# klindsay28/Newton-Krylov_OOC

Hardware: AMD Instinct MI355X
Metric: GMRES JVPs/sec, py_driver_2d iage (value = value_frozen: products on frozen years, the default; value_reference_semantic: the reference's product, two free-running years, same solver, same run) (higher is better)
Workload: dtype f64

## Files before the change

### newton-krylov_ooc_amd/csrc/nk2d_api.hip

```cpp
#include "nk2d_common.h"
#include "nk2d_build_id.h"

#include <algorithm>
#include <cmath>
#include <cstring>
#include <new>

namespace {

template <typename T>
int dev_alloc(nk2d_ctx* c, T** p, size_t n) {
    NK2D_CHECK(c, hipMalloc((void**)p, sizeof(T) * std::max<size_t>(n, 1)));
    NK2D_CHECK(c, hipMemsetAsync(*p, 0, sizeof(T) * std::max<size_t>(n, 1), nk2d_s(c)));
    return 0;
}

int ensure_stage(nk2d_ctx* c, size_t n) {
    if (n <= c->stage_elems) return 0;
    NK2D_CHECK(c, hipStreamSynchronize(nk2d_s(c)));
    if (c->STAGE) NK2D_CHECK(c, hipFree(c->STAGE));
    if (c->hSTAGE) NK2D_CHECK(c, hipHostFree(c->hSTAGE));
    c->STAGE = c->hSTAGE = nullptr;
    c->stage_elems = 0;
    NK2D_CHECK(c, hipMalloc((void**)&c->STAGE, sizeof(double) * n));
    NK2D_CHECK(c, hipHostMalloc((void**)&c->hSTAGE, sizeof(double) * n));
    c->stage_elems = n;
    return 0;
}

int stage_in(nk2d_ctx* c, const double* host, size_t n) {
    NK2D_TRY(ensure_stage(c, n));
    NK2D_CHECK(c, hipStreamSynchronize(nk2d_s(c)));
    std::memcpy(c->hSTAGE, host, sizeof(double) * n);
    NK2D_CHECK(c, hipMemcpyAsync(c->STAGE, c->hSTAGE, sizeof(double) * n, hipMemcpyHostToDevice, nk2d_s(c)));
    return 0;
}

int stage_out(nk2d_ctx* c, double* host, size_t n) {
    NK2D_CHECK(c, hipMemcpyAsync(c->hSTAGE, c->STAGE, sizeof(double) * n, hipMemcpyDeviceToHost, nk2d_s(c)));
    NK2D_CHECK(c, hipStreamSynchronize(nk2d_s(c)));
    std::memcpy(host, c->hSTAGE, sizeof(double) * n);
    return 0;
}

}

struct nk2d_download {
    double* dev = nullptr;
    double* host = nullptr;
    hipEvent_t done = nullptr;
    size_t n = 0;
};
struct nk2d_download_pool {
    std::mutex m;
    std::vector<nk2d_download*> all, idle;
};

namespace {

void download_pool_free(nk2d_ctx* c) {
    if (!c->dl_pool) return;
    for (nk2d_download* t : c->dl_pool->all) {
        (void)hipEventSynchronize(t->done);
        (void)hipEventDestroy(t->done);
        (void)hipFree(t->dev);
        (void)hipHostFree(t->host);
        delete t;
    }
    delete c->dl_pool;
    c->dl_pool = nullptr;
}

int upload_plane(nk2d_ctx* c, const double* host, int nrows, int ncols, double* dst, double fill = 0.0) {
    const size_t n = (size_t)nrows * ncols;
    NK2D_TRY(stage_in(c, host, n));
    NK2D_TRY(nk2d_k_pack_plane(c, c->STAGE, nrows, ncols, dst, fill));
    NK2D_CHECK(c, hipStreamSynchronize(nk2d_s(c)));
    return 0;
}

void build_front(nk2d_ctx* c, const std::vector<double>& dzr, const std::vector<double>& dyr) {
    const int nz = c->nz, ny = c->ny;
    const double* v = c->d.vvel;
    const double* w = c->d.wvel;
    const double* kh = c->d.hmix_coeff;
    std::vector<std::pair<double, double>> pts;
    pts.reserve((size_t)nz * ny);
    for (int k = 0; k < nz; ++k)
        for (int j = 0; j < ny; ++j) {
            const double a_up = (k > 0) ? (-0.5 * w[(size_t)k * ny + j]) * dzr[k] : 0.0;
            const double a_dn = (k < nz - 1) ? (0.5 * w[(size_t)(k + 1) * ny + j]) * dzr[k] : 0.0;
            const double a_s = (j > 0) ? (0.5 * v[(size_t)k * (ny + 1) + j]) * dyr[j] : 0.0;
            const double a_n = (j < ny - 1) ? (-0.5 * v[(size_t)k * (ny + 1) + j + 1]) * dyr[j] : 0.0;
            const double h_s = (j > 0) ? kh[(size_t)k * (ny - 1) + j - 1] * dyr[j] : 0.0;
            const double h_n = (j < ny - 1) ? kh[(size_t)k * (ny - 1) + j] * dyr[j] : 0.0;
            const double s = std::fabs(a_s + h_s) + std::fabs(a_n + h_n);
            const double q = (h_s + h_n) - (a_s + a_n) - 2.0 * (a_up + a_dn);
            if (c->kind == 1) {
                const double* ph = c->d.phos_params;
                const double upr_max = ph[1] * c->d.light_lim[(size_t)k * ny + j] / ph[0];
                const double sink_out = (k < nz - 1) ? ph[5] * dzr[k] : 0.0, sink_in = (k > 0) ? ph[5] * dzr[k] : 0.0;
                pts.emplace_back(q, s + ph[3] + ph[4]);
                pts.emplace_back(q + ph[3], s + ph[2] * upr_max);
                pts.emplace_back(q + ph[4] + sink_out - sink_in, s + (1.0 - ph[2]) * upr_max);
            } else if (s > 0.0) {
                pts.emplace_back(q, s);
            }
        }
    c->rho_c0 = 1.0e-10;
    c->rho_dlog = 1.0 / 64.0;
    const int ntab = 64 * 15;
    c->rho_tab.assign(ntab, 0.0);
    for (int k = 0; k < ntab; ++k) {
        const double shift = c->rho_c0 * std::pow(10.0, k * c->rho_dlog);
        double rho = 0.0;
        for (const auto& p : pts) {
            const double den = shift + p.first;
            const double r = (den > 0.0) ? p.second / den : 1.0e30;
            if (r > rho) rho = r;
        }
        c->rho_tab[k] = rho;
    }
}

}

extern "C" const char* nk2d_version(void) { return "nk2d 0.1 (gfx950)"; }

extern "C" const char* nk2d_last_error(const nk2d_ctx* ctx) { return ctx ? ctx->err.c_str() : "null context"; }

extern "C" void* nk2d_stream(nk2d_ctx* ctx) { return ctx ? (void*)nk2d_s(ctx) : nullptr; }

extern "C" int nk2d_set_option(nk2d_ctx* c, const char* name, double value) {
    const std::string key(name ? name : "");
    if (key == "device_ctl") {
        if ((int)value != 0) return nk2d_fail(c, "nk2d_set_option: device_ctl 1, 2 and 3 no longer exist (the controller is the host's; see option stream_years)");
        return 0;
    }
    if (key == "jac_fresh") { c->jac_fresh = value != 0.0; return 0; }
    if (key == "growth_cap") {
        if (!(value >= 0.0)) return nk2d_fail(c, "nk2d_set_option: growth_cap must be >= 0");
        c->growth_cap = value;
        return 0;
    }
    if (key == "speculate") { c->speculate = value != 0.0; return 0; }
    if (key == "hook_spec_depth") {
        if (!(value == 1.0 || value == 2.0)) return nk2d_fail(c, "nk2d_set_option: hook_spec_depth is 1 or 2");
        c->hook_spec_depth = (int)value;
        return 0;
    }
    if (key == "pc_valu") { c->pc_valu = value != 0.0; return 0; }
    if (key == "pc_fused") { c->pc_fused = (int)value; return 0; }
    if (key == "pc_fp32") { c->pc_fp32 = value != 0.0; return 0; }
    if (key == "pc_refine") {
        if (!(value >= 0.0 && value <= 4.0)) return nk2d_fail(c, "nk2d_set_option: pc_refine must be 0 .. 4");
        c->pc_refine = (int)value;
        return 0;
    }
    if (key == "pc_two_ended") {
        if (value != 0.0 && value != 1.0) return nk2d_fail(c, "nk2d_set_option: pc_two_ended is 0 or 1");
        c->pc_two_ended = (int)value;
        return 0;
    }
    if (key == "pc_pivot_wave") {
        if (value != 0.0 && value != 1.0) return nk2d_fail(c, "nk2d_set_option: pc_pivot_wave is 0 or 1");
        c->pc_pivot_wave = (int)value;
        return 0;
    }
    if (key == "final_fuse") { c->final_fuse = value != 0.0; return 0; }
    if (key == "year_fences") { c->year_fences = value != 0.0; return 0; }
    if (key == "frozen_persistent") { c->frozen_persistent = value != 0.0; return 0; }
    if (key == "frozen_team") { c->frozen_team = value != 0.0; return 0; }
    if (key == "frozen_coef_lds") { c->frozen_coef_lds = (int)value & 63; return 0; }
    if (key == "frozen_sums_poison") { c->frozen_sums_poison = (int)value != 0 ? 1 : 0; return 0; }
    if (key == "frozen_early") { c->frozen_early = (int)value != 0 ? 1 : 0; return 0; }
    if (key == "frozen_by_column") { c->frozen_by_column = (int)value; return 0; }
    if (key == "frozen_cache_after") { c->frozen_cache_after = (int)value; return 0; }
    if (key == "spec_bias") { c->spec_bias = value > 0.0 ? value : 1.0; return 0; }
    if (key == "stream_years") { c->stream_years = (int)value; c->stream_lost = 0; return 0; }
    if (key == "frozen_tape") {
        if (value != 0.0 && value != 1.0) return nk2d_fail(c, "nk2d_set_option: frozen_tape is 0 or 1");
        c->frozen_tape = (int)value;
        return 0;
    }
    if (key == "stream_hist") {
        if (value != 0.0 && value != 1.0) return nk2d_fail(c, "nk2d_set_option: stream_hist is 0 or 1");
        c->stream_hist = (int)value;
        return 0;
    }
    if (key == "stream_hist_mb") {
        if (!(value >= 0.0) || !std::isfinite(value)) return nk2d_fail(c, "nk2d_set_option: stream_hist_mb must be >= 0");
        c->stream_hist_mb = value;
        return 0;
    }
    if (key == "stream_two_waves") {
        if (c->strm) return nk2d_fail(c, "nk2d_set_option: stream_two_waves must be set before the first year of the context");
        c->stream_two_waves = (int)value;
        return 0;
    }
    if (key == "frozen_wpb") { c->frozen_wpb = (int)value; return 0; }
    if (key == "frozen_alloc_async") { c->frozen_alloc_async = value != 0.0; return 0; }
    if (key == "frozen_persistent_max_e") { c->frozen_persistent_max_e = (int)value; return 0; }
    if (key == "frozen_cache_gb") { c->frozen_cache_max_gb = value; return 0; }
    if (key == "frozen_cache_pieces") {
        if (value != 0.0 && value != 1.0) return nk2d_fail(c, "nk2d_set_option: frozen_cache_pieces is 0 or 1");
        c->frozen_cache_pieces = (int)value;
        return 0;
    }
    if (key == "frozen_cache_lean") {
        if (value != 0.0 && value != 1.0 && value != 2.0) return nk2d_fail(c, "nk2d_set_option: frozen_cache_lean is 0, 1 or 2");
        c->frozen_cache_lean = (int)value;
        return 0;
    }
    if (key == "frozen_forced") {
        if (value != 0.0 && value != 1.0 && value != 2.0 && value != 3.0) return nk2d_fail(c, "nk2d_set_option: frozen_forced is a bit mask 0 ... 3");
        c->frozen_forced = (int)value;
        return 0;
    }
    if (key == "frozen_phosphorus") {
        if (value != 0.0 && value != 1.0 && value != 2.0 && value != 3.0) return nk2d_fail(c, "nk2d_set_option: frozen_phosphorus is 0, 1, 2 or 3");
        c->frozen_phosphorus = (int)value;
        return 0;
    }
    if (key == "frozen_phosphorus_shallow") {
        if (value != 0.0 && value != 1.0) return nk2d_fail(c, "nk2d_set_option: frozen_phosphorus_shallow is 0 or 1");
        c->frozen_phosphorus_shallow = (int)value;
        return 0;
    }
    if (key == "frozen_cache_piece_mb") {
        if (!(value > 0.0) || !std::isfinite(value)) return nk2d_fail(c, "nk2d_set_option: frozen_cache_piece_mb must be > 0");
        c->frozen_cache_piece_mb = value;
        return 0;
    }
    if (key == "frozen_cache_piece_rows") {
        if (!(value >= 0.0) || value > 1.0e9) return nk2d_fail(c, "nk2d_set_option: frozen_cache_piece_rows must be 0 (from frozen_cache_piece_mb) or a row count");
        c->frozen_cache_piece_rows = (int64_t)value;
        return 0;
    }
    if (key == "frozen_cache_early") {
        if (value != 0.0 && value != 1.0) return nk2d_fail(c, "nk2d_set_option: frozen_cache_early is 0 or 1");
        c->frozen_cache_early = (int)value;
        return 0;
    }
    if (key == "barrier_timeout_ms") {
        if (!(value >= 0.0)) return nk2d_fail(c, "nk2d_set_option: barrier_timeout_ms must be >= 0");
        c->barrier_timeout_ms = value;
        return 0;
    }
    if (key == "frozen_err_check") {
        if (!(value >= 0.0) || value > 1.0e6) return nk2d_fail(c, "nk2d_set_option: frozen_err_check must be 0 (off) or a step stride");
        c->frozen_err_check = (int)value;
        return 0;
    }
    if (key == "jac_stage_state") { c->jac_stage_state = value != 0.0; return 0; }
    if (key == "jac_stage") {
        if (value != -1.0 && value != 0.0 && value != 1.0 && value != 2.0) return nk2d_fail(c, "nk2d_set_option: jac_stage must be -1, 0, 1 or 2");
        c->jac_stage = (int)value;
        return 0;
    }
    if (key == "team") {
        if (value != 0.0 && value != 1.0 && value != 2.0 && value != -1.0) return nk2d_fail(c, "nk2d_set_option: team must be -1, 0, 1 or 2");
        c->team = (value < 0.0) ? nk2d_team_auto(c) : (int)value;
        return 0;
    }
    if (key == "min_sweeps") {
        if (value != 1.0 && value != 2.0) return nk2d_fail(c, "nk2d_set_option: min_sweeps must be 1 or 2");
        c->min_sweeps = (int)value;
        c->yr_lin_tol = -1.0;
        return 0;
    }
    if (key == "factor_fp32") {
        c->factor_fp32 = value != 0.0;
        return 0;
    }
    if (key == "sweep_wpb") {
        const int w = (int)value;
        if (w != 1 && w != 2 && w != 4) return nk2d_fail(c, "nk2d_set_option: sweep_wpb must be 1, 2 or 4");
        c->sweep_wpb = w;
        return 0;
    }
    if (key == "lin_tol") {
        if (!(value > 0.0 && value < 1.0)) return nk2d_fail(c, "nk2d_set_option: lin_tol must be in (0, 1)");
        c->d.lin_tol = value;
        return 0;
    }
    return nk2d_fail(c, "nk2d_set_option: unknown option " + key);
}

extern "C" int nk2d_sync(nk2d_ctx* c) {
    NK2D_CHECK(c, hipSetDevice(c->dev));
    NK2D_CHECK(c, hipStreamSynchronize(nk2d_s(c)));
    return 0;
}

extern "C" int nk2d_profile_reset(nk2d_ctx* c, int32_t every_n) {
    NK2D_CHECK(c, hipSetDevice(c->dev));
    NK2D_CHECK(c, hipStreamSynchronize(nk2d_s(c)));
    const size_t want = every_n > 0 ? 2 * 8192 : 0;
    while (c->prof_ev.size() < want) {
        hipEvent_t e;
        NK2D_CHECK(c, hipEventCreate(&e));
        c->prof_ev.push_back(e);
    }
    c->prof_overhead_ms = 0.0;
    if (every_n > 0) {
        const int ncal = 64;
        for (int i = 0; i < ncal; ++i) {
            NK2D_CHECK(c, hipEventRecord(c->prof_ev[2 * i], nk2d_s(c)));
            NK2D_CHECK(c, hipEventRecord(c->prof_ev[2 * i + 1], nk2d_s(c)));
        }
        NK2D_CHECK(c, hipStreamSynchronize(nk2d_s(c)));
        double sum = 0.0;
        for (int i = 0; i < ncal; ++i) {
            float ms = 0.f;
            NK2D_CHECK(c, hipEventElapsedTime(&ms, c->prof_ev[2 * i], c->prof_ev[2 * i + 1]));
            sum += ms;
        }
        c->prof_overhead_ms = sum / ncal;
    }
    c->prof_every = every_n;
    c->prof_used = 0;
    c->prof_ms_sum = 0.0;
    c->prof_cnt = 0;
    c->prof_windows = 0;
    c->prof_win_launches.clear();
    c->win_open = 0;
    c->win_seq = 0;
    c->sweep_launches = 0;
// ... 121 lines not shown
        if (desc->restore_nrec == 0 && desc->sms_nrec == 0)
            return nk2d_fail(c, "nk2d_create: module_kind 2 without forcing records (use module_kind 0)");
        if ((desc->restore_nrec > 0 && (!desc->restore_times || !desc->restore_vals)) ||
            (desc->sms_nrec > 0 && (!desc->sms_times || !desc->sms_vals)))
            return nk2d_fail(c, "nk2d_create: forcing records missing");
        if (desc->sink_thres < 0.0) return nk2d_fail(c, "nk2d_create: sink_thres < 0");
        for (int i = 1; i < desc->restore_nrec; ++i)
            if (!(desc->restore_times[i] > desc->restore_times[i - 1])) return nk2d_fail(c, "nk2d_create: restore_times not increasing");
        for (int i = 1; i < desc->sms_nrec; ++i)
            if (!(desc->sms_times[i] > desc->sms_times[i - 1])) return nk2d_fail(c, "nk2d_create: sms_times not increasing");
    } else {
        c->d.restore_nrec = c->d.sms_nrec = 0;
        c->d.sink_thres = 0.0;
    }
    if (c->kind == 1 && (c->tc != 3 || desc->light_lim == nullptr))
        return nk2d_fail(c, "nk2d_create: the phosphorus module has 3 tracers and needs light_lim");
    if (c->nz < 2 || c->ny < 1 || c->tc < 1 || c->tc > NK2D_MAX_TRACERS) return nk2d_fail(c, "nk2d_create: bad grid / tracer count");
    c->E = (c->nz + 63) / 64;
    if (c->E > NK2D_MAX_E) return nk2d_fail(c, "nk2d_create: nz > 512 levels not supported by this build");
    c->nzp = c->E * 64;
    c->ncol = c->tc * c->ny;
    c->nv = (size_t)c->ncol * c->nzp;
    c->np = (size_t)c->ny * c->nzp;
    c->kv_len = (c->kind == 2) ? 2 * c->np + (size_t)c->ny : c->np;
    c->nreg = 0;
    c->dev = desc->device_id;
    NK2D_CHECK(c, hipSetDevice(c->dev));
    NK2D_CHECK(c, hipStreamCreateWithFlags(&c->stream_, hipStreamNonBlocking));
    const int nz = c->nz, ny = c->ny;
    {
        uint64_t h = 14695981039346656037ull;
        h = fnv_val(h, c->nz); h = fnv_val(h, c->ny); h = fnv_val(h, c->tc); h = fnv_val(h, c->kind);
        h = fnv1a(h, desc->depth_edges, sizeof(double) * (nz + 1));
        h = fnv1a(h, desc->ypos_edges, sizeof(double) * (ny + 1));
        h = fnv1a(h, desc->vvel, sizeof(double) * (size_t)nz * (ny + 1));
        h = fnv1a(h, desc->wvel, sizeof(double) * (size_t)(nz + 1) * ny);
        if (ny > 1) h = fnv1a(h, desc->hmix_coeff, sizeof(double) * (size_t)nz * (ny - 1));
        h = fnv1a(h, desc->bldepth_max, sizeof(double) * ny);
        h = fnv_val(h, desc->bldepth_min); h = fnv1a(h, desc->bld_tvals, sizeof(desc->bld_tvals));
        h = fnv1a(h, desc->bld_fvals, sizeof(desc->bld_fvals));
        h = fnv_val(h, desc->vmix_log_shallow); h = fnv_val(h, desc->vmix_log_deep); h = fnv_val(h, desc->vmix_half_width);
        h = fnv1a(h, desc->surf_rate, sizeof(desc->surf_rate)); h = fnv1a(h, desc->surf_target, sizeof(desc->surf_target));
        h = fnv1a(h, desc->decay_rate, sizeof(desc->decay_rate)); h = fnv_val(h, desc->const_src);
        if (c->kind == 1) {
            h = fnv1a(h, desc->phos_params, sizeof(desc->phos_params));
            h = fnv1a(h, desc->light_lim, sizeof(double) * (size_t)nz * ny);
        }
        if (c->kind == 2) {
            h = fnv_val(h, c->d.restore_nrec); h = fnv_val(h, c->d.sms_nrec); h = fnv_val(h, c->d.sink_thres);
            if (c->d.restore_nrec > 0) {
                h = fnv1a(h, desc->restore_times, sizeof(double) * c->d.restore_nrec);
                h = fnv1a(h, desc->restore_vals, sizeof(double) * (size_t)c->d.restore_nrec * ny);
            }
            if (c->d.sms_nrec > 0) {
                h = fnv1a(h, desc->sms_times, sizeof(double) * c->d.sms_nrec);
                h = fnv1a(h, desc->sms_vals, sizeof(double) * (size_t)c->d.sms_nrec * nz * ny);
            }
        }
        c->grid_hash = h;
    }
    NK2D_TRY(dev_alloc(c, &c->VV, (size_t)(ny + 1) * c->nzp));
    NK2D_TRY(dev_alloc(c, &c->KH, (size_t)(ny + 1) * c->nzp));
    NK2D_TRY(dev_alloc(c, &c->WT, c->np));
    NK2D_TRY(dev_alloc(c, &c->WB, c->np));
    NK2D_TRY(dev_alloc(c, &c->DZR, (size_t)c->nzp));
    NK2D_TRY(dev_alloc(c, &c->ZM0, (size_t)c->nzp));
    NK2D_TRY(dev_alloc(c, &c->ZM1, (size_t)c->nzp));
    NK2D_TRY(dev_alloc(c, &c->DM, (size_t)c->nzp));
    NK2D_TRY(dev_alloc(c, &c->DMR, (size_t)c->nzp));
    NK2D_TRY(dev_alloc(c, &c->DYR, (size_t)ny));
    NK2D_TRY(dev_alloc(c, &c->BLDMAX, (size_t)ny));
    NK2D_TRY(dev_alloc(c, &c->MASK, c->np));
    NK2D_TRY(dev_alloc(c, &c->WN, c->np));
    NK2D_TRY(dev_alloc(c, &c->JL, c->np));
    NK2D_TRY(dev_alloc(c, &c->JU, c->np));
    NK2D_TRY(dev_alloc(c, &c->JS, c->np));
    NK2D_TRY(dev_alloc(c, &c->JN, c->np));
    NK2D_TRY(dev_alloc(c, &c->JC, c->np));
    NK2D_TRY(dev_alloc(c, &c->LIGHT, c->np));
    NK2D_TRY(dev_alloc(c, &c->UPR, c->np));
    c->YLIN = nullptr;
    c->ylin_set = 0;
    for (int i = 0; i < 5; ++i) NK2D_TRY(dev_alloc(c, &c->KV[i], c->kv_len));
    for (int i = 0; i < 3; ++i) NK2D_TRY(dev_alloc(c, &c->KVN[i], c->kv_len));
    for (int i = 0; i < 5; ++i) NK2D_TRY(dev_alloc(c, &c->JB[i], c->np));
    NK2D_TRY(dev_alloc(c, &c->Y, c->nv));
    NK2D_TRY(dev_alloc(c, &c->YOLD, c->nv));
    NK2D_TRY(dev_alloc(c, &c->F, c->nv));
    NK2D_TRY(dev_alloc(c, &c->Z, 3 * c->nv));
    NK2D_TRY(dev_alloc(c, &c->ZP, 3 * c->nv));
    NK2D_TRY(dev_alloc(c, &c->ZN, 3 * c->nv));
    c->single_swap = 0;
    c->min_sweeps = 1;
    c->team = nk2d_team_auto(c);
    c->jac_stage = 1;
    c->final_fuse = 1;
    c->jac_stage_state = 1;
    c->part_cur = nullptr;
    NK2D_TRY(dev_alloc(c, &c->W, 3 * c->nv));
    NK2D_TRY(dev_alloc(c, &c->BR, c->nv));
    NK2D_TRY(dev_alloc(c, &c->BCR, c->nv));
    NK2D_TRY(dev_alloc(c, &c->BCI, c->nv));
    for (int i = 0; i < 2; ++i) {
        NK2D_TRY(dev_alloc(c, &c->XR[i], c->nv));
        NK2D_TRY(dev_alloc(c, &c->XCR[i], c->nv));
        NK2D_TRY(dev_alloc(c, &c->XCI[i], c->nv));
    }
    NK2D_TRY(dev_alloc(c, &c->FR_INV, c->nv));
    NK2D_TRY(dev_alloc(c, &c->FC_INVR, c->nv));
    NK2D_TRY(dev_alloc(c, &c->FC_INVI, c->nv));
    NK2D_TRY(dev_alloc(c, &c->FR_TAB, (size_t)c->ncol * 14 * 64));
    NK2D_TRY(dev_alloc(c, &c->FC_TABR, (size_t)c->ncol * 14 * 64));
    NK2D_TRY(dev_alloc(c, &c->FC_TABI, (size_t)c->ncol * 14 * 64));
    NK2D_TRY(dev_alloc(c, &c->FR32_INV, c->nv));
    NK2D_TRY(dev_alloc(c, &c->FC32_INVR, c->nv));
    NK2D_TRY(dev_alloc(c, &c->FC32_INVI, c->nv));
    NK2D_TRY(dev_alloc(c, &c->FR32_TAB, (size_t)c->ncol * 14 * 64));
    NK2D_TRY(dev_alloc(c, &c->FC32_TABR, (size_t)c->ncol * 14 * 64));
    NK2D_TRY(dev_alloc(c, &c->FC32_TABI, (size_t)c->ncol * 14 * 64));
    c->factor_fp32 = 0;
    NK2D_TRY(dev_alloc(c, &c->TMP, c->nv));
    NK2D_TRY(dev_alloc(c, &c->TMP2, c->nv));
    NK2D_TRY(dev_alloc(c, &c->PART, (size_t)c->ncol));
    NK2D_TRY(dev_alloc(c, &c->PART2, (size_t)c->ncol));
    NK2D_TRY(dev_alloc(c, &c->STEP_NORM, (size_t)3 * NK2D_OWN_REC_CAP));
    c->frozen_fallbacks = 0;
    c->frozen_resumes = 0;
    c->frozen_cache = nullptr;
    c->frozen_persistent = 1;
    c->frozen_persistent_max_e = 8;
    c->frozen_cache_max_gb = 128.0;
    c->frozen_cache_builds = c->frozen_persistent_years = 0;
    c->frozen_team = 1;
    c->frozen_cache_after = 0;
    c->frozen_cache_pieces = 0;
    c->frozen_cache_piece_mb = 1024.0;
    c->frozen_cache_piece_rows = 0;
    c->frozen_cache_early = 0;
    c->frozen_cache_lean = 0;
    c->frozen_lean_years = 0;
    c->frozen_lean_mem_key = 0;
    c->frozen_forced = 0;
    c->frozen_forced_years = 0;
    c->frozen_phosphorus = 0;
    c->frozen_phosphorus_shallow = 0;
    c->frozen_phosphorus_shallow_years = 0;
    c->frozen_two_waves_last = 0;
    c->frozen_phosphorus_years = c->frozen_two_waves_years = 0;
    c->frozen_cache_piece_allocs = c->frozen_cache_early_requests = 0;
    c->frozen_coef_lds = 63;
    c->frozen_lds_bits = 0;
    c->frozen_early = NK2D_FROZEN_EARLY_DEFAULT;
    c->frozen_early_bits = 0;
    c->frozen_by_column = 1;
    c->strm = nullptr;
    c->spec_bias = 1.0;
    c->stream_two_waves = std::getenv("NK2D_STREAM_TWO_WAVES") ? std::atoi(std::getenv("NK2D_STREAM_TWO_WAVES")) : 1;
    c->stream_years = 1;
    c->stream_on = 0;
    c->stream_lost = 0;
    c->stream_cmds = c->stream_launches = c->stream_timeouts = c->stream_years_run = 0;
    c->frozen_tape = 0;
    c->tape = nullptr;
    c->tape_rec = c->tape_foreign = 0;
    c->tape_years_run = c->tape_builds = c->tape_timeouts = c->tape_fallbacks = 0;
    c->frozen_wpb = 2;
    c->frozen_alloc_async = 1;
    c->barrier_timeout_ms = 2000.0;
    c->year_fences = 0;
    c->frozen_err_check = NK2D_CKPT_EVERY;
    c->STEP_PART = nullptr;
    c->step_part_rows = 0;
    NK2D_TRY(dev_alloc(c, &c->RED, (size_t)4096));
    for (int i = 0; i < 8; ++i) NK2D_CHECK(c, hipEventCreateWithFlags(&c->snap_ev[i], hipEventDisableTiming));
    c->snap_ready = 1;
    c->jac_fresh = 1;
    c->growth_cap = 0.0;
    c->hist_n = 0;
    c->hist_next = 0;
    c->hist_t = nullptr;
    c->hist_host = nullptr;
    c->stream_hist = 0;
    c->stream_hist_mb = 256.0;
    c->HISTBUF = nullptr;
    c->hist_slots = c->hist_buf_elems = 0;
    c->hist_year_samples = c->hist_year_drains = 0;
    c->stream_hist_samples = c->stream_hist_drains = 0;
    c->sweep_wpb = 4;
    NK2D_CHECK(c, hipHostMalloc((void**)&c->hRED, sizeof(double) * 4096));
    NK2D_CHECK(c, hipHostMalloc((void**)&c->hPART, sizeof(double) * c->ncol));
    NK2D_CHECK(c, hipHostMalloc((void**)&c->hPART2, sizeof(double) * c->ncol));
    NK2D_CHECK(c, hipHostMalloc((void**)&c->hPARTB, sizeof(double) * c->ncol));
    NK2D_CHECK(c, hipHostMalloc((void**)&c->hPARTC, sizeof(double) * c->ncol));
    c->part_on_host = 0;
    c->speculate = 1;
    c->hook_spec_depth = 2;
    c->factor_pending = 0;
    c->lu_cre = c->lu_ccr = c->lu_cci = 0.0;
    c->rcoef_elems = 0;
    c->RCOEF = nullptr;
    c->hRCOEF = nullptr;

    std::vector<double> zmid(nz), dz(nz), dzr(nz), dzm(nz), dzmr(nz), zm1(nz), dy(ny), dyr(ny);
    for (int k = 0; k < nz; ++k) {
        zmid[k] = 0.5 * (desc->depth_edges[k] + desc->depth_edges[k + 1]);
        dz[k] = desc->depth_edges[k + 1] - desc->depth_edges[k];
        dzr[k] = 1.0 / dz[k];
    }
    for (int k = 0; k < nz; ++k) {
        zm1[k] = (k < nz - 1) ? zmid[k + 1] : 0.0;
        dzm[k] = (k < nz - 1) ? zmid[k + 1] - zmid[k] : 0.0;
        dzmr[k] = (k < nz - 1) ? 1.0 / dzm[k] : 0.0;
    }
    for (int j = 0; j < ny; ++j) {
        dy[j] = desc->ypos_edges[j + 1] - desc->ypos_edges[j];
        dyr[j] = 1.0 / dy[j];
    }
    NK2D_TRY(upload_plane(c, desc->vvel, nz, ny + 1, c->VV));
    {
        std::vector<double> khf((size_t)nz * (ny + 1), 0.0);
        for (int k = 0; k < nz; ++k)
            for (int jf = 1; jf < ny; ++jf) khf[(size_t)k * (ny + 1) + jf] = desc->hmix_coeff[(size_t)k * (ny - 1) + jf - 1];
        NK2D_TRY(upload_plane(c, khf.data(), nz, ny + 1, c->KH));
    }
    NK2D_TRY(upload_plane(c, desc->wvel, nz, ny, c->WT));
    NK2D_TRY(upload_plane(c, desc->wvel + ny, nz, ny, c->WB));
    NK2D_TRY(upload_plane(c, dzr.data(), nz, 1, c->DZR));
    NK2D_TRY(upload_plane(c, zmid.data(), nz, 1, c->ZM0));
    NK2D_TRY(upload_plane(c, zm1.data(), nz, 1, c->ZM1));
    NK2D_TRY(upload_plane(c, dzm.data(), nz, 1, c->DM));
    NK2D_TRY(upload_plane(c, dzmr.data(), nz, 1, c->DMR));
    NK2D_CHECK(c, hipMemcpy(c->DYR, dyr.data(), sizeof(double) * ny, hipMemcpyHostToDevice));
    NK2D_CHECK(c, hipMemcpy(c->BLDMAX, desc->bldepth_max, sizeof(double) * ny, hipMemcpyHostToDevice));
    if (c->kind == 1) NK2D_TRY(upload_plane(c, desc->light_lim, nz, ny, c->LIGHT));
    if (c->kind == 2) {
        if (desc->sms_nrec > 0) {
            NK2D_TRY(dev_alloc(c, &c->SMSREC, (size_t)desc->sms_nrec * c->np));
            for (int r = 0; r < desc->sms_nrec; ++r)
                NK2D_TRY(upload_plane(c, desc->sms_vals + (size_t)r * nz * ny, nz, ny, c->SMSREC + (size_t)r * c->np));
            c->sms_t = new double[desc->sms_nrec];
            std::memcpy(c->sms_t, desc->sms_times, sizeof(double) * desc->sms_nrec);
        }
        if (desc->restore_nrec > 0) {
            NK2D_TRY(dev_alloc(c, &c->RESTREC, (size_t)desc->restore_nrec * ny));
            NK2D_CHECK(c, hipMemcpy(c->RESTREC, desc->restore_vals, sizeof(double) * desc->restore_nrec * ny, hipMemcpyHostToDevice));
            c->rest_t = new double[desc->restore_nrec];
            std::memcpy(c->rest_t, desc->restore_times, sizeof(double) * desc->restore_nrec);
        }
    }
    build_front(c, dzr, dyr);
    c->d.depth_edges = c->d.ypos_edges = c->d.vvel = c->d.wvel = c->d.hmix_coeff = c->d.bldepth_max = nullptr;
    c->d.light_lim = nullptr;
    c->d.restore_times = c->d.restore_vals = c->d.sms_times = c->d.sms_vals = nullptr;
    {
        std::vector<int32_t> m((size_t)nz * ny, 1);
        std::vector<double> w((size_t)nz * ny, 1.0);
        NK2D_TRY(nk2d_set_region(c, m.data(), w.data(), 1));
    }
    return 0;
}

extern "C" int nk2d_create(const nk2d_desc* desc, nk2d_ctx** out) {
    if (!desc || !out) return -2;
    nk2d_ctx* c = new (std::nothrow) nk2d_ctx();
    if (!c) return -2;
    c->stream_ = nullptr;
    c->STAGE = nullptr;
    c->hSTAGE = nullptr;
    c->stage_elems = 0;
    c->dl_pool = nullptr;
    c->precond = nullptr;
    c->pc_valu = 0;
    c->pc_fused = 1;
    c->pc_fp32 = 0;
    c->pc_refine = 1;
    c->pc_two_ended = 0;
    c->pc_setup_rounds = c->pc_sub_launches = 0;
    c->pc_pivot_wave = 0;
    c->pc_pivot_wave_steps = 0;
    c->st = nk2d_stats();
    c->prof_every = 0;
    c->snap_ready = 0;
    c->prof_used = 0;
    c->prof_ms_sum = 0.0;
    c->prof_overhead_ms = 0.0;
    c->prof_cnt = 0;
    c->prof_windows = 0;
    c->win_open = 0;
    c->win_seq = 0;
    c->sweep_launches = 0;
    c->sweep_bytes = 0.0;
    c->fused_bytes_all = 0.0;
    c->norm_hook = nullptr;
    c->norm_hook_user = nullptr;
    c->norm_hook_vec = nullptr;
    c->norm_hook_vec_user = nullptr;
    c->global_n = 0.0;
    c->timer_ready = 0;
    c->YR_PART = c->YR_OUT = c->hYR_OUT = c->YR_REC = nullptr;
    c->YR_SYNC = nullptr;
    c->YR_MTAB = nullptr;
    *out = c;
    return create_impl(c, desc);
}

extern "C" void nk2d_destroy(nk2d_ctx* c) {
// ... 206 lines not shown
}

extern "C" int nk2d_vmix_coeff(nk2d_ctx* c, double t, double* host_out) {
    NK2D_CHECK(c, hipSetDevice(c->dev));
    double* out[1] = {c->KV[4]};
    NK2D_TRY(nk2d_k_vmix(c, 1, &t, out));
    const size_t n = (size_t)(c->nz - 1) * c->ny;
    NK2D_TRY(ensure_stage(c, n));
    NK2D_TRY(nk2d_k_unpack_plane(c, c->KV[4], c->nz - 1, c->ny, c->STAGE));
    return stage_out(c, host_out, n);
}

static const double* lin_state(nk2d_ctx* c) { return (c->kind != 0 && c->ylin_set) ? c->YLIN : nullptr; }

extern "C" int nk2d_set_lin_state(nk2d_ctx* c, nk2d_vec y) {
    NK2D_CHECK(c, hipSetDevice(c->dev));
    if (!c->YLIN) NK2D_TRY(dev_alloc(c, &c->YLIN, c->nv));
    NK2D_CHECK(c, hipMemcpyAsync(c->YLIN, y, sizeof(double) * c->nv, hipMemcpyDeviceToDevice, nk2d_s(c)));
    c->ylin_set = 1;
    return 0;
}

extern "C" int nk2d_jacobian_apply(nk2d_ctx* c, double t, nk2d_vec v, nk2d_vec out) {
    NK2D_CHECK(c, hipSetDevice(c->dev));
    double* kv[1] = {c->KV[4]};
    NK2D_TRY(nk2d_k_vmix(c, 1, &t, kv));
    NK2D_TRY(nk2d_k_jac(c, c->KV[4], lin_state(c)));
    NK2D_TRY(nk2d_k_jac_apply(c, (const double*)v, (double*)out));
    return 0;
}

extern "C" int nk2d_jacobian_diags(nk2d_ctx* c, double t, double* host_out) {
    NK2D_CHECK(c, hipSetDevice(c->dev));
    if (c->kind == 1) return nk2d_fail(c, "nk2d_jacobian_diags: the phosphorus Jacobian is not five diagonals; use nk2d_jacobian_apply");
    double* out[1] = {c->KV[4]};
    NK2D_TRY(nk2d_k_vmix(c, 1, &t, out));
    NK2D_TRY(nk2d_k_jac(c, c->KV[4], lin_state(c)));
    const size_t P = (size_t)c->nz * c->ny;
    NK2D_TRY(ensure_stage(c, P));
    const double* planes[5] = {c->JL, c->JS, c->JC, c->JN, c->JU};
    std::vector<double> tmp(P), extra;
    if (c->kind == 2) {
        extra.resize(P);
        NK2D_TRY(nk2d_k_unpack_plane(c, c->UPR, c->nz, c->ny, c->STAGE));
        NK2D_TRY(stage_out(c, extra.data(), P));
    }
    for (int d = 0; d < 5; ++d) {
        NK2D_TRY(nk2d_k_unpack_plane(c, planes[d], c->nz, c->ny, c->STAGE));
        NK2D_TRY(stage_out(c, tmp.data(), P));
        for (int tr = 0; tr < c->tc; ++tr) {
            double* dst = host_out + ((size_t)d * c->tc + tr) * P;
            std::memcpy(dst, tmp.data(), sizeof(double) * P);
            if (d == 2) {
                for (int j = 0; j < c->ny; ++j) dst[j] = dst[j] + (-c->d.surf_rate[tr]);
                if (c->d.decay_rate[tr] != 0.0)
                    for (size_t i = 0; i < P; ++i) dst[i] = dst[i] + (-c->d.decay_rate[tr]);
                if (!extra.empty())
                    for (size_t i = 0; i < P; ++i) dst[i] = dst[i] - extra[i];
            }
        }
    }
    return 0;
}

extern "C" int nk2d_shifted_solve(nk2d_ctx* c, double t_jac, double h, double mu_re, double mu_im, nk2d_vec b_re,
                                  nk2d_vec b_im, nk2d_vec x_re, nk2d_vec x_im, int32_t* sweeps_out) {
    NK2D_CHECK(c, hipSetDevice(c->dev));
    double* out[1] = {c->KV[4]};
    NK2D_TRY(nk2d_k_vmix(c, 1, &t_jac, out));
    NK2D_TRY(nk2d_k_jac(c, c->KV[4], lin_state(c)));
    const bool cplxsys = mu_im != 0.0;
    const int m = nk2d_sweeps_for(c, mu_re / h);
    NK2D_TRY(nk2d_k_factor(c, !cplxsys, cplxsys, mu_re / h, mu_re / h, mu_im / h));
    int src = 0;
    for (int it = 0; it < m; ++it) {
        NK2D_TRY(nk2d_k_sweep(c, !cplxsys, cplxsys, it == 0, mu_re / h, mu_re / h, mu_im / h, (const double*)b_re,
                              (const double*)b_re, (const double*)b_im, src));
        src = 1 - src;
    }
    if (!cplxsys) {
        NK2D_CHECK(c, hipMemcpyAsync(x_re, c->XR[src], sizeof(double) * c->nv, hipMemcpyDeviceToDevice, nk2d_s(c)));
    } else {
        NK2D_CHECK(c, hipMemcpyAsync(x_re, c->XCR[src], sizeof(double) * c->nv, hipMemcpyDeviceToDevice, nk2d_s(c)));
        NK2D_CHECK(c, hipMemcpyAsync(x_im, c->XCI[src], sizeof(double) * c->nv, hipMemcpyDeviceToDevice, nk2d_s(c)));
    }
    NK2D_CHECK(c, hipStreamSynchronize(nk2d_s(c)));
    if (sweeps_out) *sweeps_out = m;
    return 0;
}

extern "C" int nk2d_comp_fcn(nk2d_ctx* c, nk2d_vec x, nk2d_vec fx, nk2d_stats* stats, const double* replay,
                             int64_t replay_n, double* record, int64_t record_cap, int64_t* record_n) {
    NK2D_CHECK(c, hipSetDevice(c->dev));
    if (record_n) *record_n = 0;
    const int rc = nk2d_radau_year(c, x, fx, stats, replay, replay_n, record, record_cap, record_n);
    if (rc == 0 && record && record_n && *record_n > 0 && c->frozen_cache_pieces && c->frozen_cache_early)
        NK2D_TRY(nk2d_frozen_cache_early(c, record, *record_n));
    return rc;
}

extern "C" int nk2d_comp_fcn_frozen(nk2d_ctx* c, nk2d_vec x, nk2d_vec fx, nk2d_stats* stats, const double* sched,
                                    int64_t sched_n) {
    NK2D_CHECK(c, hipSetDevice(c->dev));
    if (!sched || sched_n < 1) return nk2d_fail(c, "nk2d_comp_fcn_frozen: empty schedule");
    return nk2d_radau_year(c, x, fx, stats, sched, sched_n, nullptr, 0, nullptr, true);
}

extern "C" int nk2d_frozen_fallbacks(nk2d_ctx* c, int64_t* n) {
    if (n) *n = c->frozen_fallbacks;
    return 0;
}

extern "C" int nk2d_frozen_resumes(nk2d_ctx* c, int64_t* n) {
    if (n) *n = c->frozen_resumes;
    return 0;
}

extern "C" int nk2d_get_counter(nk2d_ctx* c, const char* name, int64_t* out) {
    const std::string key(name ? name : "");
    int64_t v = 0;
    if (key == "frozen_persistent_years") v = c->frozen_persistent_years;
    else if (key == "frozen_cache_builds") v = c->frozen_cache_builds;
    else if (key == "frozen_team_years") v = c->frozen_team_years;
    else if (key == "stream_years_run") v = c->stream_years_run;
    else if (key == "stream_commands") v = c->stream_cmds;
    else if (key == "stream_launches") v = c->stream_launches;
    else if (key == "stream_timeouts") v = c->stream_timeouts;
    else if (key == "stream_columns_per_workgroup") v = nk2d_stream_columns_per_workgroup(c);
    else if (key == "stream_two_waves_kernel") v = nk2d_stream_two_waves(c);
    else if (key == "stream_hist_samples") v = c->stream_hist_samples;
    else if (key == "stream_hist_drains") v = c->stream_hist_drains;
    else if (key == "pc_setup_rounds") v = c->pc_setup_rounds;
    else if (key == "pc_sub_launches") v = c->pc_sub_launches;
    else if (key == "pc_pivot_wave_steps") v = c->pc_pivot_wave_steps;
    else if (key == "tape_years_run") v = c->tape_years_run;
    else if (key == "tape_builds") v = c->tape_builds;
    else if (key == "tape_timeouts") v = c->tape_timeouts;
    else if (key == "tape_fallbacks") v = c->tape_fallbacks;
    else if (key == "tape_bytes") v = nk2d_tape_size(c, 0);
    else if (key == "tape_commands") v = nk2d_tape_size(c, 1);
    else if (key.rfind("stream_prof_", 0) == 0) {
        double pr[12];
        NK2D_TRY(nk2d_stream_profile(c, pr));
        const int i = std::atoi(key.c_str() + 12);
        v = (i >= 0 && i < 12) ? (int64_t)pr[i] : 0;
    }
    else if (key == "frozen_launch_us") v = c->frozen_launch_us;
    else if (key == "frozen_cache_pending") v = nk2d_frozen_cache_pending(c);
    else if (key == "frozen_cache_bytes") v = nk2d_frozen_cache_bytes(c);
    else if (key == "frozen_cache_pieces") v = nk2d_frozen_cache_npieces(c);
    else if (key == "frozen_cache_lean") v = nk2d_frozen_cache_is_lean(c);
    else if (key == "frozen_lds_bits") v = c->frozen_lds_bits;
    else if (key == "frozen_early_bits") v = c->frozen_early_bits;
    else if (key == "frozen_step_sums_hash") v = c->frozen_step_sums_hash;
    else if (key == "frozen_lean_years") v = c->frozen_lean_years;
    else if (key == "frozen_forced_years") v = c->frozen_forced_years;
    else if (key == "frozen_phosphorus_years") v = c->frozen_phosphorus_years;
    else if (key == "frozen_phosphorus_shallow_years") v = c->frozen_phosphorus_shallow_years;
    else if (key == "frozen_two_waves_years") v = c->frozen_two_waves_years;
    else if (key == "frozen_cache_piece_allocs") v = nk2d_frozen_cache_piece_allocs(c);
    else if (key == "frozen_cache_early_requests") v = c->frozen_cache_early_requests;
    else if (key == "frozen_fallbacks") v = c->frozen_fallbacks;
    else if (key == "frozen_resumes") v = c->frozen_resumes;
    else if (key == "spec_launches_dropped") v = c->cnt_spec_dropped;
    else if (key == "spec_front_launches_dropped") v = c->cnt_front_dropped;
    else if (key == "err_estimates_queued") v = c->cnt_err_queued;
    else if (key == "err_estimates_dropped") v = c->cnt_err_void;
    else return nk2d_fail(c, "nk2d_get_counter: unknown counter " + key);
    if (out) *out = v;
    return 0;
}

extern "C" int nk2d_schedule_fingerprint(nk2d_ctx* c, double* out) {
    if (out) *out = nk2d_fingerprint(c);
    return 0;
}

extern "C" int nk2d_last_schedule(nk2d_ctx* c, double* out, int64_t cap, int64_t* n) {
    const int64_t rows = (int64_t)(c->last_sched.size() / NK2D_SCHED_WIDTH);
    if (n) *n = rows;
    if (out) {
        if (cap < rows) return nk2d_fail(c, "nk2d_last_schedule: buffer too small", -4);
        std::memcpy(out, c->last_sched.data(), sizeof(double) * c->last_sched.size());
    }
    return 0;
}

extern "C" int nk2d_set_frozen_schedule(nk2d_ctx* c, const double* sched, int64_t sched_n) {
    if (sched_n < 0 || (sched_n > 0 && !sched)) return nk2d_fail(c, "nk2d_set_frozen_schedule: bad arguments");
    c->frozen_sched.assign(sched, sched + (size_t)sched_n * NK2D_SCHED_WIDTH);
    return 0;
}

int nk2d_hist_sample(nk2d_ctx* c, double t_old, double t_new, bool first) {
    const size_t n = (size_t)c->tc * c->nz * c->ny;
    double x = 0.0;
    while (nk2d_hist_due(c, t_old, t_new, &x)) {
        NK2D_TRY(nk2d_r_dense(c, x, c->TMP));
        NK2D_TRY(ensure_stage(c, n));
        NK2D_TRY(nk2d_k_unpack_state(c, c->TMP, c->STAGE));
        NK2D_TRY(stage_out(c, c->hist_host + (size_t)c->hist_next * n, n));
        c->hist_next++;
    }
    (void)first;
    return 0;
}

int nk2d_hist_buf_ready(nk2d_ctx* c) {
    nk2d_hist_buf_reset(c);
    const double bytes = c->stream_hist_mb * 1048576.0;
    const double fit = std::floor(bytes / (8.0 * (double)c->nv));
    c->hist_slots = (size_t)std::min((double)c->hist_n, std::max(1.0, fit));
    const size_t need = c->hist_slots * c->nv;
    if (c->hist_buf_elems < need) {
        NK2D_CHECK(c, hipStreamSynchronize(nk2d_s(c)));
        if (c->HISTBUF) NK2D_CHECK(c, hipFree(c->HISTBUF));
        c->HISTBUF = nullptr;
        c->hist_buf_elems = 0;
        NK2D_CHECK(c, hipMalloc((void**)&c->HISTBUF, sizeof(double) * need));
        c->hist_buf_elems = need;
    }
    return ensure_stage(c, (size_t)c->tc * c->nz * c->ny);
}

void nk2d_hist_buf_reset(nk2d_ctx* c) {
    c->hist_slot_k.clear();
    c->hist_year_samples = c->hist_year_drains = 0;
}
void nk2d_hist_year_done(nk2d_ctx* c) {
    c->stream_hist_samples += c->hist_year_samples;
    c->stream_hist_drains += c->hist_year_drains;
    c->hist_year_samples = c->hist_year_drains = 0;
}

int nk2d_hist_drain(nk2d_ctx* c) {
    if (c->hist_slot_k.empty()) return 0;
    const size_t n = (size_t)c->tc * c->nz * c->ny;
    NK2D_TRY(ensure_stage(c, n));
    for (size_t slot = 0; slot < c->hist_slot_k.size(); ++slot) {
        NK2D_TRY(nk2d_k_unpack_state(c, c->HISTBUF + slot * c->nv, c->STAGE));
        NK2D_TRY(stage_out(c, c->hist_host + (size_t)c->hist_slot_k[slot] * n, n));
    }
    c->hist_year_samples += (int64_t)c->hist_slot_k.size();
    c->hist_year_drains++;
    c->hist_slot_k.clear();
    return 0;
}

int nk2d_hist_push(nk2d_ctx* c, double t_old, double t_new) {
    double x = 0.0;
    while (nk2d_hist_due(c, t_old, t_new, &x)) {
        if (c->hist_slot_k.size() >= c->hist_slots) NK2D_TRY(nk2d_hist_drain(c));
        NK2D_TRY(nk2d_r_dense_push(c, x, c->HISTBUF + c->hist_slot_k.size() * c->nv));
        c->hist_slot_k.push_back(c->hist_next);
        c->hist_next++;
    }
    return 0;
}

extern "C" int nk2d_comp_fcn_hist(nk2d_ctx* c, nk2d_vec x, nk2d_vec fx, nk2d_stats* stats, int32_t n_eval,
                                  const double* t_eval, double* host_hist) {
    NK2D_CHECK(c, hipSetDevice(c->dev));
    for (int i = 1; i < n_eval; ++i)
        if (!(t_eval[i] > t_eval[i - 1])) return nk2d_fail(c, "nk2d_comp_fcn_hist: t_eval must be increasing");
    if (n_eval > 0 && (t_eval[0] < c->d.t0 || t_eval[n_eval - 1] > c->d.t1))
        return nk2d_fail(c, "nk2d_comp_fcn_hist: t_eval outside the time range");
    c->hist_n = n_eval;
    c->hist_next = 0;
    c->hist_t = t_eval;
    c->hist_host = host_hist;
    nk2d_hist_buf_reset(c);
    const int rc = nk2d_radau_year(c, x, fx, stats, nullptr, 0, nullptr, 0, nullptr);
    const bool complete = c->hist_next == n_eval && c->hist_slot_k.empty();
    nk2d_hist_buf_reset(c);
    c->hist_n = 0;
    c->hist_t = nullptr;
    c->hist_host = nullptr;
    if (rc != 0) return rc;
    if (!complete) return nk2d_fail(c, "nk2d_comp_fcn_hist: not every t_eval sample was produced");
    return 0;
}

__device__ __forceinline__ double bcast(const double* __restrict__ coef, int m) { return (m > 0) ? coef[m - 1] : 1.0; }

template <int E>
__global__ void k_dot(int ncol, int ny, int nreg, const double* __restrict__ a, const double* __restrict__ b,
                      const double* __restrict__ wn, const int32_t* __restrict__ mask, double* __restrict__ part) {
    const int lane = threadIdx.x & 63;
    const int task = blockIdx.x * NK2D_WAVES_PER_BLOCK + (threadIdx.x >> 6);
    if (task >= ncol) return;
    const int j = task % ny;
    double aa[E], bb[E], ww[E];
    int mm[E];
    load_col<E>(a, task, lane, aa);
    load_col<E>(b, task, lane, bb);
    load_col<E>(wn, j, lane, ww);
#pragma unroll
    for (int e = 0; e < E; ++e) {
        mm[e] = mask[(size_t)j * (E * 64) + e * 64 + lane];
        aa[e] = ww[e] * (aa[e] * bb[e]);
    }
    for (int r = 1; r <= nreg; ++r) {
        double acc = 0.0;
        bool any = false;
#pragma unroll
        for (int e = 0; e < E; ++e)
// ... 192 lines not shown
```

### newton-krylov_ooc_amd/csrc/nk2d_bodies.h

```cpp
#pragma once
#include <atomic>
#include <chrono>
#include <cmath>
#include <cstdio>
#include <cstdlib>
#include <cstring>
#include <mutex>
#include <thread>

#include "nk2d_common.h"
#include "nk2d_hostmath.h"


struct DevP {
    int nz, ny, tc, ncol;
    const double *VV, *KH, *WT, *WB, *DZR, *ZM0, *ZM1, *DM, *DMR, *DYR, *BLDMAX;
    double surf[NK2D_MAX_TRACERS], starget[NK2D_MAX_TRACERS], decay[NK2D_MAX_TRACERS], csrc;
    double atol, rtol;
    double ph_hs, ph_mu, ph_sig, ph_rd, ph_rp, ph_vs;
    const double *LIGHT, *UPR;
    const double *SMSREC, *RESTREC;
    int f_sms, f_restore;
    double f_thres_r;
    size_t np;
// ... 609 lines not shown
            for (int e = 0; e < E; ++e) rr[e] = __builtin_fma(jn[e], xn[e], __builtin_fma(js[e], xs[e], rr[e]));
            load_col<E, MP>(A.xci_old, cs_col, lane, xs);
            load_col<E, MP>(A.xci_old, cn_col, lane, xn);
#pragma unroll
            for (int e = 0; e < E; ++e) ri[e] = __builtin_fma(jn[e], xn[e], __builtin_fma(js[e], xs[e], ri[e]));
            if constexpr (KIND == 1) {
                phos_couple<E>(P, tr, j, lane, A.xcr_old, upr, rr);
                phos_couple<E>(P, tr, j, lane, A.xci_old, upr, ri);
            }
        }
#pragma unroll
        for (int e = 0; e < E; ++e) {
            const bool valid = (lane * E + e) < P.nz;
            r[e] = c_make(valid ? rr[e] : 0.0, valid ? ri[e] : 0.0);
        }
        tridiag_apply<E, cplx>(a, cc, inv, tab, r, lane);
#pragma unroll
        for (int e = 0; e < E; ++e) { rr[e] = r[e].re; ri[e] = r[e].im; }
        store_col<E, MP>(A.xcr_new, col, lane, rr);
        store_col<E, MP>(A.xci_new, col, lane, ri);
    }
}

static inline void fill_factor_args(const nk2d_ctx* c, SweepArgs& A) {
    A.JL = c->JL; A.JU = c->JU; A.JS = c->JS; A.JN = c->JN; A.JC = c->JC;
    A.fr_inv = c->FR_INV; A.fc_invr = c->FC_INVR; A.fc_invi = c->FC_INVI;
    A.fr_tab = c->FR_TAB; A.fc_tabr = c->FC_TABR; A.fc_tabi = c->FC_TABI;
    A.fr_inv32 = c->FR32_INV; A.fc_invr32 = c->FC32_INVR; A.fc_invi32 = c->FC32_INVI;
    A.fr_tab32 = c->FR32_TAB; A.fc_tabr32 = c->FC32_TABR; A.fc_tabi32 = c->FC32_TABI;
    A.f32 = c->factor_fp32;
}

__device__ double block_sum(const double* __restrict__ part, int ntasks, double* sh) {
    double s = 0.0;
    for (int i = threadIdx.x; i < ntasks; i += NK2D_BLOCK) s += part[i];
    sh[threadIdx.x] = s;
    __syncthreads();
    for (int o = NK2D_BLOCK / 2; o > 0; o >>= 1) {
        if ((int)threadIdx.x < o) sh[threadIdx.x] += sh[threadIdx.x + o];
        __syncthreads();
    }
    return sh[0];
}

struct PredictArgs {
    const double *y, *yold, *zp;
    double *z, *w;
    size_t nv;
    double x0, x1, x2;
};

template <int E, int MP = 0>
__device__ __forceinline__ void predict_body(const PredictArgs& A, int task, int lane) {
    const double* __restrict__ y = A.y;
    const double* __restrict__ yold = A.yold;
    const double* __restrict__ zp = A.zp;
    double* __restrict__ z = A.z;
    double* __restrict__ w = A.w;
    const size_t nv = A.nv;
    const double x0 = A.x0, x1 = A.x1, x2 = A.x2;
    double yy[E], yo[E], z0[E], z1[E], z2[E];
    load_col<E, MP>(y, task, lane, yy);
    load_col<E, MP>(yold, task, lane, yo);
    load_col<E, MP>(zp, task, lane, z0);
    load_col<E, MP>(zp + nv, task, lane, z1);
    load_col<E, MP>(zp + 2 * nv, task, lane, z2);
    const double xs[3] = {x0, x1, x2};
    double o[3][E];
#pragma unroll
    for (int e = 0; e < E; ++e) {
        double q[3];
#pragma unroll
        for (int cidx = 0; cidx < 3; ++cidx) q[cidx] = (z0[e] * cP[0][cidx] + z1[e] * cP[1][cidx]) + z2[e] * cP[2][cidx];
#pragma unroll
        for (int i = 0; i < 3; ++i) {
            const double p1 = xs[i], p2 = p1 * xs[i], p3 = p2 * xs[i];
            double v = (q[0] * p1 + q[1] * p2) + q[2] * p3;
            v = v + yo[e];
            o[i][e] = v - yy[e];
        }
    }
    double wv[E];
#pragma unroll
    for (int i = 0; i < 3; ++i) store_col<E, MP>(z + i * nv, task, lane, o[i]);
#pragma unroll
    for (int r = 0; r < 3; ++r) {
#pragma unroll
        for (int e = 0; e < E; ++e) wv[e] = (cTI[r][0] * o[0][e] + cTI[r][1] * o[1][e]) + cTI[r][2] * o[2][e];
        store_col<E>(w + r * nv, task, lane, wv);
    }
}

struct JacOut {
    double *JL, *JU, *JS, *JN, *JC;
    int stage;
};

struct StageArgs {
    const double *y, *z, *w;
    double* zout;
    const double* kv[3];
    double *br, *bcr, *bci;
    size_t nv;
    double mreal, mcr, mci;
};

struct FinalArgs {
    double* ynew;
    double* znext;
    double x0, x1, x2;
    int nblk_cols;
};

struct FusedArgs {
    StageArgs st;
    SweepArgs sw;
    double* part;
    int do_stage, do_update;
    int delta;
};

template <int E>
__device__ __forceinline__ void w_lds_get(const double* s, int r, int lane, double (&v)[E]) {
#pragma unroll
    for (int e = 0; e < E; ++e) v[e] = s[(r * E + e) * 64 + lane];
}
template <int E>
__device__ __forceinline__ void w_lds_put(double* s, int r, int lane, const double (&v)[E]) {
#pragma unroll
    for (int e = 0; e < E; ++e) s[(r * E + e) * 64 + lane] = v[e];
}

struct LdsSrc {
    const double* coef;
    double* w;
    const double* step;
    const double* piv;
    double* y;
};
template <int E>
struct OwnState {
    double z[3][E];
    int valid;
};
template <int E>
__device__ __forceinline__ void col_lds_get(const double* s, int r, int lane, double (&v)[E]) {
#pragma unroll
    for (int e = 0; e < E; ++e) v[e] = s[(r * E + e) * 64 + lane];
}
struct LateNorm {
    double acc;
    double* part;
    int defer, pending;
};
template <int E>
__device__ __forceinline__ double norm_partial_sum(const DevP& P, const double (&yy)[E], const double (&d0v)[E],
                                                   const double (&d1v)[E], const double (&d2v)[E]) {
    double acc = 0.0;
#pragma unroll
    for (int e = 0; e < E; ++e) {
        const double sc = P.atol + fabs(yy[e]) * P.rtol;
        const double d0 = d0v[e] / sc, d1 = d1v[e] / sc, d2 = d2v[e] / sc;
        acc += (d0 * d0 + d1 * d1) + d2 * d2;
    }
    return wave_sum(acc);
}

template <int E, int KIND, int FACTOR, int STAGE, int MP = 0, int FINAL = 0, int CL = 0>
__device__ __forceinline__ void newton_fused_body(const DevP& P, const FusedArgs& A, int task, int lane,
                                                  const FinalArgs* fin = nullptr, const LdsSrc* lds = nullptr,
                                                  OwnState<E>* own = nullptr, LateNorm* late = nullptr) {
    const double* coef_lds = (CL & 1) ? lds->coef : nullptr;
    double* w_lds = (CL & 2) ? lds->w : nullptr;
    (void)coef_lds; (void)w_lds;
    const int tr = task / P.ny, j = task - tr * P.ny;
    const int cs_col = (j > 0) ? task - 1 : task, cn_col = (j < P.ny - 1) ? task + 1 : task;
    double fr[E], fcr[E], fci[E];
    if (STAGE && A.do_stage) {
        ColCoef<E> cf;
        if constexpr (CL & 1) load_coef_lds<E>(coef_lds, lane, cf);
        else load_coef<E>(P, j, lane, cf);
        double y0[E], ys[E], yn[E];
        if constexpr (CL & 16) {
            if (!own->valid) {
                load_col<E, MP>(A.st.y, task, lane, y0);
                w_lds_put<E>(lds->y, 0, lane, y0);
            } else {
                col_lds_get<E>(lds->y, 0, lane, y0);
            }
        } else {
            load_col<E, MP>(A.st.y, task, lane, y0);
        }
        load_col<E, MP>(A.st.y, cs_col, lane, ys);
        load_col<E, MP>(A.st.y, cn_col, lane, yn);
#pragma unroll
        for (int e = 0; e < E; ++e) { fr[e] = 0.0; fcr[e] = 0.0; fci[e] = 0.0; }
#pragma unroll
        for (int i = 0; i < 3; ++i) {
            double c[E], cs[E], cn[E], kv[E], f[E];
            if constexpr (CL & 32) {
                if (own->valid) {
#pragma unroll
                    for (int e = 0; e < E; ++e) c[e] = own->z[i][e];
                } else {
                    load_col<E, MP>(A.st.z + i * A.st.nv, task, lane, c);
                }
            } else {
                load_col<E, MP>(A.st.z + i * A.st.nv, task, lane, c);
            }
            load_col<E, MP>(A.st.z + i * A.st.nv, cs_col, lane, cs);
            load_col<E, MP>(A.st.z + i * A.st.nv, cn_col, lane, cn);
            if constexpr (CL & 4) col_lds_get<E>(lds->step, i, lane, kv);
            else load_col<E, MP>(A.st.kv[i], j, lane, kv);
#pragma unroll
            for (int e = 0; e < E; ++e) { c[e] = y0[e] + c[e]; cs[e] = ys[e] + cs[e]; cn[e] = yn[e] + cn[e]; }
            tend_col<E, KIND>(P, cf, c, cs, cn, kv, tr, lane, f);
            if constexpr (KIND == 2) forced_sources<E>(P, A.st.kv[i], j, lane, c, f);
            if constexpr (KIND == 1) {
                double u1[E], u2[E], v1[E], v2[E];
                phos_load_others<E>(P, tr, j, lane, A.st.y, u1, u2);
                phos_load_others<E>(P, tr, j, lane, A.st.z + i * A.st.nv, v1, v2);
                phos_add<E>(u1, u2, v1, v2);
                phos_sources<E>(P, tr, j, lane, c, u1, u2, cf.dzr, f);
            }
#pragma unroll
            for (int e = 0; e < E; ++e) {
                fr[e] = fr[e] + f[e] * cTI[0][i];
                fcr[e] = fcr[e] + f[e] * cTI[1][i];
                fci[e] = fci[e] + f[e] * cTI[2][i];
            }
        }
        double w0[E], w1[E], w2[E];
        if constexpr (CL & 2) {
            w_lds_get<E>(w_lds, 0, lane, w0); w_lds_get<E>(w_lds, 1, lane, w1); w_lds_get<E>(w_lds, 2, lane, w2);
        } else {
            load_col<E>(A.st.w, task, lane, w0);
            load_col<E>(A.st.w + A.st.nv, task, lane, w1);
            load_col<E>(A.st.w + 2 * A.st.nv, task, lane, w2);
        }
#pragma unroll
        for (int e = 0; e < E; ++e) {
            fr[e] = fr[e] - A.st.mreal * w0[e];
            fcr[e] = fcr[e] - (A.st.mcr * w1[e] - A.st.mci * w2[e]);
            fci[e] = fci[e] - (A.st.mcr * w2[e] + A.st.mci * w1[e]);
        }
        if (!A.do_update && !A.delta) {
            store_col<E>(A.st.br, task, lane, fr);
            store_col<E>(A.st.bcr, task, lane, fcr);
            store_col<E>(A.st.bci, task, lane, fci);
        }
    } else if (A.delta) {
#pragma unroll
        for (int e = 0; e < E; ++e) { fr[e] = 0.0; fcr[e] = 0.0; fci[e] = 0.0; }
    } else {
        load_col<E>(A.sw.br, task, lane, fr);
        load_col<E>(A.sw.bcr, task, lane, fcr);
        load_col<E>(A.sw.bci, task, lane, fci);
    }
    double a[E], cc[E];
    {
        double jl[E], ju[E];
        if constexpr (CL & 4) {
            col_lds_get<E>(lds->step, 3, lane, jl);
            col_lds_get<E>(lds->step, 4, lane, ju);
        } else {
            load_col<E, MP>(A.sw.JL, j, lane, jl);
            load_col<E, MP>(A.sw.JU, j, lane, ju);
        }
        line_offdiag<E, KIND>(P, tr, lane, jl, ju, a, cc);
    }
    if (!A.sw.first) {
        double js[E], jn[E], xs[E], xn[E];
        load_col<E, MP>(A.sw.JS, j, lane, js);
        load_col<E, MP>(A.sw.JN, j, lane, jn);
        load_col<E, MP>(A.sw.xr_old, cs_col, lane, xs);
        load_col<E, MP>(A.sw.xr_old, cn_col, lane, xn);
#pragma unroll
        for (int e = 0; e < E; ++e) fr[e] = __builtin_fma(jn[e], xn[e], __builtin_fma(js[e], xs[e], fr[e]));
        load_col<E, MP>(A.sw.xcr_old, cs_col, lane, xs);
        load_col<E, MP>(A.sw.xcr_old, cn_col, lane, xn);
#pragma unroll
        for (int e = 0; e < E; ++e) fcr[e] = __builtin_fma(jn[e], xn[e], __builtin_fma(js[e], xs[e], fcr[e]));
        load_col<E, MP>(A.sw.xci_old, cs_col, lane, xs);
        load_col<E, MP>(A.sw.xci_old, cn_col, lane, xn);
#pragma unroll
        for (int e = 0; e < E; ++e) fci[e] = __builtin_fma(jn[e], xn[e], __builtin_fma(js[e], xs[e], fci[e]));
        if constexpr (KIND == 1) {
            double upr[E];
            load_col<E>(P.UPR, j, lane, upr);
            phos_couple<E>(P, tr, j, lane, A.sw.xr_old, upr, fr);
            phos_couple<E>(P, tr, j, lane, A.sw.xcr_old, upr, fcr);
            phos_couple<E>(P, tr, j, lane, A.sw.xci_old, upr, fci);
        }
    }
    {
        double inv[E], tab[NK2D_TAB];
        if constexpr (FACTOR) {
            double dre[E];
            line_diag<E, KIND, MP>(P, A.sw.JC, tr, j, lane, A.sw.cre, dre);
            tridiag_factor<E, double>(a, cc, dre, inv, tab, lane);
            store_col<E>(A.sw.fr_inv, task, lane, inv);
            double* p = A.sw.fr_tab + (size_t)task * (NK2D_TAB * 64) + lane;
#pragma unroll
            for (int i = 0; i < NK2D_TAB; ++i) p[i * 64] = tab[i];
            if (A.sw.f32) {
                store_col32<E>(A.sw.fr_inv32, task, lane, inv);
                store_tab32(A.sw.fr_tab32, task, lane, tab);
            }
        } else if (A.sw.f32) {
            load_col32<E>(A.sw.fr_inv32, task, lane, inv);
            load_tab32(A.sw.fr_tab32, task, lane, tab);
        } else {
            if constexpr (CL & 8) col_lds_get<E>(lds->piv, 0, lane, inv);
            else load_col<E>(A.sw.fr_inv, task, lane, inv);
            load_tab<E>(A.sw.fr_tab, task, lane, tab);
        }
#pragma unroll
        for (int e = 0; e < E; ++e) fr[e] = ((lane * E + e) < P.nz) ? fr[e] : 0.0;
        tridiag_apply<E, double>(a, cc, inv, tab, fr, lane);
    }
    {
        cplx r[E], inv[E], tab[NK2D_TAB];
        if constexpr (FACTOR) {
            double dre[E];
            cplx d[E];
            line_diag<E, KIND, MP>(P, A.sw.JC, tr, j, lane, A.sw.ccr, dre);
#pragma unroll
            for (int e = 0; e < E; ++e) d[e] = c_make(dre[e], ((lane * E + e) < P.nz) ? A.sw.cci : 0.0);
            tridiag_factor<E, cplx>(a, cc, d, inv, tab, lane);
            double re[E], im[E];
#pragma unroll
            for (int e = 0; e < E; ++e) { re[e] = inv[e].re; im[e] = inv[e].im; }
            store_col<E>(A.sw.fc_invr, task, lane, re);
            store_col<E>(A.sw.fc_invi, task, lane, im);
            double* pr = A.sw.fc_tabr + (size_t)task * (NK2D_TAB * 64) + lane;
            double* pi = A.sw.fc_tabi + (size_t)task * (NK2D_TAB * 64) + lane;
            double tre[NK2D_TAB], tim[NK2D_TAB];
#pragma unroll
            for (int i = 0; i < NK2D_TAB; ++i) { pr[i * 64] = tab[i].re; pi[i * 64] = tab[i].im; tre[i] = tab[i].re; tim[i] = tab[i].im; }
            if (A.sw.f32) {
                store_col32<E>(A.sw.fc_invr32, task, lane, re);
                store_col32<E>(A.sw.fc_invi32, task, lane, im);
                store_tab32(A.sw.fc_tabr32, task, lane, tre);
                store_tab32(A.sw.fc_tabi32, task, lane, tim);
            }
        } else {
            double t0[E], t1[E], tr0[NK2D_TAB], ti0[NK2D_TAB];
            if (A.sw.f32) {
                load_col32<E>(A.sw.fc_invr32, task, lane, t0);
                load_col32<E>(A.sw.fc_invi32, task, lane, t1);
                load_tab32(A.sw.fc_tabr32, task, lane, tr0);
                load_tab32(A.sw.fc_tabi32, task, lane, ti0);
            } else {
                load_col<E>(A.sw.fc_invr, task, lane, t0);
                load_col<E>(A.sw.fc_invi, task, lane, t1);
                load_tab<E>(A.sw.fc_tabr, task, lane, tr0);
                load_tab<E>(A.sw.fc_tabi, task, lane, ti0);
            }
#pragma unroll
            for (int e = 0; e < E; ++e) inv[e] = c_make(t0[e], t1[e]);
#pragma unroll
            for (int i = 0; i < NK2D_TAB; ++i) tab[i] = c_make(tr0[i], ti0[i]);
        }
#pragma unroll
        for (int e = 0; e < E; ++e) {
            const bool valid = (lane * E + e) < P.nz;
            r[e] = c_make(valid ? fcr[e] : 0.0, valid ? fci[e] : 0.0);
        }
        tridiag_apply<E, cplx>(a, cc, inv, tab, r, lane);
#pragma unroll
        for (int e = 0; e < E; ++e) { fcr[e] = r[e].re; fci[e] = r[e].im; }
    }
    if (!A.do_stage && A.delta) {
        double x1[E];
        load_col<E, MP>(A.sw.xr_old, task, lane, x1);
#pragma unroll
        for (int e = 0; e < E; ++e) fr[e] = x1[e] + fr[e];
        load_col<E, MP>(A.sw.xcr_old, task, lane, x1);
#pragma unroll
        for (int e = 0; e < E; ++e) fcr[e] = x1[e] + fcr[e];
        load_col<E, MP>(A.sw.xci_old, task, lane, x1);
#pragma unroll
        for (int e = 0; e < E; ++e) fci[e] = x1[e] + fci[e];
    }
    if (!A.do_update) {
        store_col<E, MP>(A.sw.xr_new, task, lane, fr);
        store_col<E, MP>(A.sw.xcr_new, task, lane, fcr);
        store_col<E, MP>(A.sw.xci_new, task, lane, fci);
        if constexpr (CL & 32) {
#pragma unroll
            for (int i = 0; i < 3; ++i) {
#pragma unroll
                for (int e = 0; e < E; ++e) own->z[i][e] = 0.0;
            }
            own->valid = 0;
        }
        return;
    }
    const bool norm = A.part != nullptr;
    double yy[E], w0[E], w1[E], w2[E];
    if (FINAL || norm) {
        if constexpr (CL & 16) col_lds_get<E>(lds->y, 0, lane, yy);
        else load_col<E, MP>(A.st.y, task, lane, yy);
    }
    if constexpr (CL & 2) {
        w_lds_get<E>(w_lds, 0, lane, w0); w_lds_get<E>(w_lds, 1, lane, w1); w_lds_get<E>(w_lds, 2, lane, w2);
    } else {
        load_col<E>(A.st.w, task, lane, w0);
        load_col<E>(A.st.w + A.st.nv, task, lane, w1);
        load_col<E>(A.st.w + 2 * A.st.nv, task, lane, w2);
    }
    bool norm_late = false;
    if constexpr (CL & 128) norm_late = norm && late->defer != 0;
    if (norm && !norm_late) {
        double acc = 0.0;
#pragma unroll
        for (int e = 0; e < E; ++e) {
            const double sc = P.atol + fabs(yy[e]) * P.rtol;
            const double d0 = fr[e] / sc, d1 = fcr[e] / sc, d2 = fci[e] / sc;
            acc += (d0 * d0 + d1 * d1) + d2 * d2;
        }
        acc = wave_sum(acc);
        if (lane == 0) st_mp<MP>(A.part + task, acc);
    }
#pragma unroll
    for (int e = 0; e < E; ++e) {
        w0[e] = w0[e] + fr[e];
        w1[e] = w1[e] + fcr[e];
        w2[e] = w2[e] + fci[e];
    }
    double* wout = const_cast<double*>(A.st.w);
    if constexpr (FINAL) {
        double z0[E], z1[E], z2[E], yn[E];
#pragma unroll
        for (int e = 0; e < E; ++e) {
            z0[e] = (cT[0][0] * w0[e] + cT[0][1] * w1[e]) + cT[0][2] * w2[e];
            z1[e] = (cT[1][0] * w0[e] + cT[1][1] * w1[e]) + cT[1][2] * w2[e];
            z2[e] = (cT[2][0] * w0[e] + cT[2][1] * w1[e]) + cT[2][2] * w2[e];
            yn[e] = yy[e] + z2[e];
        }
        store_col<E, MP>(fin->ynew, task, lane, yn);
        if constexpr (CL & 16) w_lds_put<E>(lds->y, 0, lane, yn);
        const double xs[3] = {fin->x0, fin->x1, fin->x2};
        double o[3][E];
#pragma unroll
        for (int e = 0; e < E; ++e) {
            double q[3];
#pragma unroll
            for (int cidx = 0; cidx < 3; ++cidx) q[cidx] = (z0[e] * cP[0][cidx] + z1[e] * cP[1][cidx]) + z2[e] * cP[2][cidx];
#pragma unroll
            for (int i = 0; i < 3; ++i) {
                const double p1 = xs[i], p2 = p1 * xs[i], p3 = p2 * xs[i];
                double v = (q[0] * p1 + q[1] * p2) + q[2] * p3;
                v = v + yy[e];
                o[i][e] = v - yn[e];
            }
        }
#pragma unroll
        for (int i = 0; i < 3; ++i) store_col<E, MP>(fin->znext + i * A.st.nv, task, lane, o[i]);
        double wv[E];
#pragma unroll
        for (int r = 0; r < 3; ++r) {
#pragma unroll
            for (int e = 0; e < E; ++e) wv[e] = (cTI[r][0] * o[0][e] + cTI[r][1] * o[1][e]) + cTI[r][2] * o[2][e];
            if constexpr (CL & 2) w_lds_put<E>(w_lds, r, lane, wv);
            else store_col<E>(wout + r * A.st.nv, task, lane, wv);
        }
        if constexpr (CL & 32) {
#pragma unroll
            for (int i = 0; i < 3; ++i) {
#pragma unroll
                for (int e = 0; e < E; ++e) own->z[i][e] = o[i][e];
            }
        }
        if constexpr ((CL & 48) != 0) own->valid = 1;
        if constexpr (CL & 128) {
            if (norm_late) { late->acc = norm_partial_sum<E>(P, yy, fr, fcr, fci); late->part = A.part + task; late->pending = 1; }
        }
        return;
    }
    double* zout = A.st.zout;
    if constexpr (CL & 2) {
        w_lds_put<E>(w_lds, 0, lane, w0); w_lds_put<E>(w_lds, 1, lane, w1); w_lds_put<E>(w_lds, 2, lane, w2);
    } else {
        store_col<E>(wout, task, lane, w0);
        store_col<E>(wout + A.st.nv, task, lane, w1);
        store_col<E>(wout + 2 * A.st.nv, task, lane, w2);
    }
    double zz[E];
#pragma unroll
    for (int r = 0; r < 3; ++r) {
#pragma unroll
        for (int e = 0; e < E; ++e) zz[e] = (cT[r][0] * w0[e] + cT[r][1] * w1[e]) + cT[r][2] * w2[e];
        store_col<E, MP>(zout + r * A.st.nv, task, lane, zz);
        if constexpr (CL & 32) {
#pragma unroll
            for (int e = 0; e < E; ++e) own->z[r][e] = zz[e];
        }
    }
    if constexpr ((CL & 48) != 0) own->valid = 1;
    if constexpr (CL & 128) {
        if (norm_late) { late->acc = norm_partial_sum<E>(P, yy, fr, fcr, fci); late->part = A.part + task; late->pending = 1; }
    }
}


template <int E>
__device__ __forceinline__ void plane_task(const DevP& P, const VmixArgs& V, const JacOut& J, int ptask, int lane) {
    int ti = ptask / P.ny;
    const int j = ptask - ti * P.ny;
    if (J.stage > 0) ti = (ti == 0) ? J.stage : ((ti <= J.stage) ? ti - 1 : ti);
    double kv[E];
    vmix_body_kv<E>(P, V, ti * P.ny + j, lane, kv);
    if (ti == J.stage) jac_core<E, 0>(P, kv, V.out[ti], J.JL, J.JU, J.JS, J.JN, J.JC, nullptr, nullptr, j, lane);
}

template <int E, int WR>
struct TeamLds {
    double F[3][E * 64];
    double D[3][E * 64];
    double W[WR > 0 ? WR : 1][WR > 0 ? E * 64 : 1];
    double a[E * 64], c[E * 64], inv[E * 64];
    double tab[NK2D_TAB * 64];
};

template <int E>
__device__ __forceinline__ void lds_put(double* s, int lane, const double (&v)[E]) {
#pragma unroll
    for (int e = 0; e < E; ++e) s[e * 64 + lane] = v[e];
}
template <int E>
__device__ __forceinline__ void lds_get(const double* s, int lane, double (&v)[E]) {
#pragma unroll
    for (int e = 0; e < E; ++e) v[e] = s[e * 64 + lane];
}

template <int E, int KIND, int FACTOR, int STAGE, int NW, int FIN, int MP = 0>
__device__ __forceinline__ void newton_team_body(const DevP& P, const FusedArgs& A, TeamLds<E, (NW == 4 ? 3 : 0)>& S, int task, int w, int lane,
                                                 const FinalArgs* fin) {
    constexpr int CW = NW - 1;
    constexpr int NS = NW - 1;
    const int tr = task / P.ny, j = task - tr * P.ny;
    const int cs_col = (j > 0) ? task - 1 : task, cn_col = (j < P.ny - 1) ? task + 1 : task;
    const bool stage = STAGE && A.do_stage;

    if (w == CW) {
        double a[E], cc[E];
        {
            double jl[E], ju[E];
            load_col<E>(A.sw.JL, j, lane, jl);
            load_col<E>(A.sw.JU, j, lane, ju);
            line_offdiag<E, KIND>(P, tr, lane, jl, ju, a, cc);
        }
        cplx cinv[E], ctab[NK2D_TAB];
        double dre[E];
        if (stage) {
            double rinv[E], rtab[NK2D_TAB], w0[E];
            if constexpr (FACTOR) {
                double drr[E];
                line_diag<E, KIND, 0>(P, A.sw.JC, tr, j, lane, A.sw.cre, drr);
#pragma unroll
                for (int e = 0; e < E; ++e) rinv[e] = drr[e];
            } else if (A.sw.f32) {
                load_col32<E>(A.sw.fr_inv32, task, lane, rinv);
                load_tab32(A.sw.fr_tab32, task, lane, rtab);
            } else {
                load_col<E>(A.sw.fr_inv, task, lane, rinv);
                load_tab<E>(A.sw.fr_tab, task, lane, rtab);
            }
            if constexpr (NW == 4) load_col<E, MP>(A.st.w, task, lane, w0);
            lds_put<E>(S.a, lane, a);
            lds_put<E>(S.c, lane, cc);
            lds_put<E>(S.inv, lane, rinv);
            if constexpr (!FACTOR) {
#pragma unroll
                for (int i = 0; i < NK2D_TAB; ++i) S.tab[i * 64 + lane] = rtab[i];
            }
            if constexpr (NW == 4) lds_put<E>(S.W[0], lane, w0);
        }
        if constexpr (FACTOR) {
            line_diag<E, KIND, 0>(P, A.sw.JC, tr, j, lane, A.sw.ccr, dre);
        } else {
            double t0[E], t1[E], tr0[NK2D_TAB], ti0[NK2D_TAB];
            if (A.sw.f32) {
                load_col32<E>(A.sw.fc_invr32, task, lane, t0);
                load_col32<E>(A.sw.fc_invi32, task, lane, t1);
                load_tab32(A.sw.fc_tabr32, task, lane, tr0);
                load_tab32(A.sw.fc_tabi32, task, lane, ti0);
            } else {
                load_col<E>(A.sw.fc_invr, task, lane, t0);
                load_col<E>(A.sw.fc_invi, task, lane, t1);
                load_tab<E>(A.sw.fc_tabr, task, lane, tr0);
                load_tab<E>(A.sw.fc_tabi, task, lane, ti0);
            }
#pragma unroll
            for (int e = 0; e < E; ++e) cinv[e] = c_make(t0[e], t1[e]);
#pragma unroll
            for (int i = 0; i < NK2D_TAB; ++i) ctab[i] = c_make(tr0[i], ti0[i]);
        }
        double fcr[E], fci[E];
        if (stage) {
            double w1[E], w2[E];
            load_col<E, MP>(A.st.w + A.st.nv, task, lane, w1);
            load_col<E, MP>(A.st.w + 2 * A.st.nv, task, lane, w2);
            if constexpr (NW == 4) {
                lds_put<E>(S.W[1], lane, w1);
                lds_put<E>(S.W[2], lane, w2);
            }
            __syncthreads();
#pragma unroll
            for (int e = 0; e < E; ++e) {
                const double f0 = S.F[0][e * 64 + lane], f1 = S.F[1][e * 64 + lane], f2 = S.F[2][e * 64 + lane];
                double sr = 0.0, si = 0.0;
                sr = sr + f0 * cTI[1][0];
                si = si + f0 * cTI[2][0];
                sr = sr + f1 * cTI[1][1];
                si = si + f1 * cTI[2][1];
                sr = sr + f2 * cTI[1][2];
                si = si + f2 * cTI[2][2];
                fcr[e] = sr - (A.st.mcr * w1[e] - A.st.mci * w2[e]);
                fci[e] = si - (A.st.mcr * w2[e] + A.st.mci * w1[e]);
            }
            if (!A.do_update && !A.delta) {
                store_col<E, MP>(A.st.bcr, task, lane, fcr);
                store_col<E, MP>(A.st.bci, task, lane, fci);
            }
        } else if (A.delta) {
#pragma unroll
            for (int e = 0; e < E; ++e) { fcr[e] = 0.0; fci[e] = 0.0; }
        } else {
            load_col<E, MP>(A.sw.bcr, task, lane, fcr);
            load_col<E, MP>(A.sw.bci, task, lane, fci);
        }
        if (!A.sw.first) {
            double js[E], jn[E], xs[E], xn[E];
            load_col<E>(A.sw.JS, j, lane, js);
            load_col<E>(A.sw.JN, j, lane, jn);
            load_col<E, MP>(A.sw.xcr_old, cs_col, lane, xs);
            load_col<E, MP>(A.sw.xcr_old, cn_col, lane, xn);
#pragma unroll
            for (int e = 0; e < E; ++e) fcr[e] = __builtin_fma(jn[e], xn[e], __builtin_fma(js[e], xs[e], fcr[e]));
            load_col<E, MP>(A.sw.xci_old, cs_col, lane, xs);
            load_col<E, MP>(A.sw.xci_old, cn_col, lane, xn);
#pragma unroll
            for (int e = 0; e < E; ++e) fci[e] = __builtin_fma(jn[e], xn[e], __builtin_fma(js[e], xs[e], fci[e]));
            if constexpr (KIND == 1) {
                double upr[E];
                load_col<E>(P.UPR, j, lane, upr);
// ... 382 lines not shown
    if (lane == 0) st_mp<MP>(A.part + task, acc);
}

template <int E, int KIND, int MP = 0>
__device__ __forceinline__ void err_rhs2_body(const DevP& P, const double* __restrict__ y, const double* __restrict__ err,
                                              const double* __restrict__ kvp, const double* __restrict__ z, size_t nv,
                                              double h, double* __restrict__ out, int task, int lane) {
    const int tr = task / P.ny, j = task - tr * P.ny;
    const int cs_col = (j > 0) ? task - 1 : task, cn_col = (j < P.ny - 1) ? task + 1 : task;
    ColCoef<E> cf;
    load_coef<E>(P, j, lane, cf);
    double c[E], cs[E], cn[E], t0[E], kv[E], ff[E];
    load_col<E, MP>(y, task, lane, c);
    load_col<E, MP>(err, task, lane, t0);
#pragma unroll
    for (int e = 0; e < E; ++e) c[e] = c[e] + t0[e];
    load_col<E, MP>(y, cs_col, lane, cs);
    load_col<E, MP>(err, cs_col, lane, t0);
#pragma unroll
    for (int e = 0; e < E; ++e) cs[e] = cs[e] + t0[e];
    load_col<E, MP>(y, cn_col, lane, cn);
    load_col<E, MP>(err, cn_col, lane, t0);
#pragma unroll
    for (int e = 0; e < E; ++e) cn[e] = cn[e] + t0[e];
    load_col<E, MP>(kvp, j, lane, kv);
    tend_col<E, KIND>(P, cf, c, cs, cn, kv, tr, lane, ff);
    if constexpr (KIND == 2) forced_sources<E>(P, kvp, j, lane, c, ff);
    if constexpr (KIND == 1) {
        double u1[E], u2[E], v1[E], v2[E];
        phos_load_others<E>(P, tr, j, lane, y, u1, u2);
        phos_load_others<E>(P, tr, j, lane, err, v1, v2);
        phos_add<E>(u1, u2, v1, v2);
        phos_sources<E>(P, tr, j, lane, c, u1, u2, cf.dzr, ff);
    }
    double z0[E], z1[E], z2[E];
    load_col<E, MP>(z, task, lane, z0);
    load_col<E, MP>(z + nv, task, lane, z1);
    load_col<E, MP>(z + 2 * nv, task, lane, z2);
#pragma unroll
    for (int e = 0; e < E; ++e) {
        const double ze = ((z0[e] * cE[0] + z1[e] * cE[1]) + z2[e] * cE[2]) / h;
        ff[e] = ff[e] + ze;
    }
    store_col<E>(out, task, lane, ff);
}

template <int E, int KIND, int MP = 0>
__device__ __forceinline__ void commit_tend_body(const DevP& P, const double* __restrict__ y, const double* __restrict__ z2,
                                                 const double* __restrict__ kvp, double* __restrict__ ynew,
                                                 double* __restrict__ f, int task, int lane) {
    const int tr = task / P.ny, j = task - tr * P.ny;
    const int cs_col = (j > 0) ? task - 1 : task, cn_col = (j < P.ny - 1) ? task + 1 : task;
    ColCoef<E> cf;
    load_coef<E>(P, j, lane, cf);
    double c[E], cs[E], cn[E], t0[E], kv[E], ff[E];
    load_col<E, MP>(y, task, lane, c);
    load_col<E, MP>(z2, task, lane, t0);
#pragma unroll
    for (int e = 0; e < E; ++e) c[e] = c[e] + t0[e];
    store_col<E, MP>(ynew, task, lane, c);
    load_col<E, MP>(y, cs_col, lane, cs);
    load_col<E, MP>(z2, cs_col, lane, t0);
#pragma unroll
    for (int e = 0; e < E; ++e) cs[e] = cs[e] + t0[e];
    load_col<E, MP>(y, cn_col, lane, cn);
    load_col<E, MP>(z2, cn_col, lane, t0);
#pragma unroll
    for (int e = 0; e < E; ++e) cn[e] = cn[e] + t0[e];
    load_col<E, MP>(kvp, j, lane, kv);
    tend_col<E, KIND>(P, cf, c, cs, cn, kv, tr, lane, ff);
    if constexpr (KIND == 2) forced_sources<E>(P, kvp, j, lane, c, ff);
    if constexpr (KIND == 1) {
        double u1[E], u2[E], v1[E], v2[E];
        phos_load_others<E>(P, tr, j, lane, y, u1, u2);
        phos_load_others<E>(P, tr, j, lane, z2, v1, v2);
        phos_add<E>(u1, u2, v1, v2);
        phos_sources<E>(P, tr, j, lane, c, u1, u2, cf.dzr, ff);
    }
    store_col<E>(f, task, lane, ff);
}

struct BoundaryArgs {
    const double *y, *z2, *kv_new;
    double *ynew, *f;
    double *JL, *JU, *JS, *JN, *JC;
    int do_jac, nblk_vmix, nblk_jac;
    int jac_stage;
    int with_tend;
};

template <int E, int MP = 0>
__device__ __forceinline__ void err_norm_body(const DevP& P, const double* __restrict__ y, const double* __restrict__ z2p,
                                              const double* __restrict__ err, double* __restrict__ part, int task, int lane) {
    double yy[E], z2[E], er[E];
    load_col<E, MP>(y, task, lane, yy);
    load_col<E, MP>(z2p, task, lane, z2);
    load_col<E, MP>(err, task, lane, er);
    double acc = 0.0;
#pragma unroll
    for (int e = 0; e < E; ++e) {
        const double yn = yy[e] + z2[e];
        const double sc = P.atol + fmax(fabs(yy[e]), fabs(yn)) * P.rtol;
        const double a = er[e] / sc;
        acc += a * a;
    }
    acc = wave_sum(acc);
    if (lane == 0) st_mp<MP>(part + task, acc);
}

static inline PredictArgs predict_args(nk2d_ctx* c, double x0, double x1, double x2) {
    PredictArgs A;
    A.y = c->Y; A.yold = c->YOLD; A.zp = c->ZP; A.z = c->Z; A.w = c->W;
    A.nv = c->nv;
    A.x0 = x0; A.x1 = x1; A.x2 = x2;
    return A;
}
static inline double fused_words(const nk2d_ctx* c, bool do_stage, bool first, bool do_update, bool delta, bool do_factor) {
    const double Pc = (double)c->nz * c->ny, N = Pc * c->tc;
    double words = 0.0;
    if (do_stage) words += 7.0 * N + 7.0 * Pc + ((do_update || delta) ? 0.0 : 3.0 * N);
    const double fw = (c->factor_fp32 && !do_factor) ? 0.5 : 1.0;
    words += (first ? 2.0 : 4.0) * Pc + fw * (3.0 * N + 3.0 * 14.0 / c->E * N);
    if (do_factor) words += Pc;
    if (!do_stage && !delta) words += 3.0 * N;
    if (!first) words += 3.0 * N;
    if (!do_update) words += 3.0 * N;
    if (do_update) words += (do_stage ? 0.0 : N) + 9.0 * N;
    return words;
}

static inline void fill_fused_args(nk2d_ctx* c, FusedArgs& A, bool do_stage, bool first, bool do_update, double mreal,
                            double mcr, double mci, int src, bool delta) {
    A = {};
    A.st.y = c->Y; A.st.z = c->Z; A.st.w = c->W;
    A.st.zout = c->Z;
    A.st.kv[0] = c->KV[0]; A.st.kv[1] = c->KV[1]; A.st.kv[2] = c->KV[2];
    A.st.br = c->BR; A.st.bcr = c->BCR; A.st.bci = c->BCI;
    A.st.nv = c->nv; A.st.mreal = mreal; A.st.mcr = mcr; A.st.mci = mci;
    fill_factor_args(c, A.sw);
    A.sw.br = c->BR; A.sw.bcr = c->BCR; A.sw.bci = c->BCI;
    A.sw.xr_old = c->XR[src]; A.sw.xcr_old = c->XCR[src]; A.sw.xci_old = c->XCI[src];
    A.sw.xr_new = c->XR[1 - src]; A.sw.xcr_new = c->XCR[1 - src]; A.sw.xci_new = c->XCI[1 - src];
    A.sw.first = first ? 1 : 0;
    A.sw.cre = c->lu_cre; A.sw.ccr = c->lu_ccr; A.sw.cci = c->lu_cci;
    A.part = c->PART;
    A.do_stage = do_stage ? 1 : 0;
    A.do_update = do_update ? 1 : 0;
    A.delta = delta ? 1 : 0;
}

#define NK2D_SPIN_LIMIT 4000000

static inline size_t yr_sync_bytes(const nk2d_ctx* c) { return 8192 + (size_t)c->ncol * 128; }

struct NeighbourSync {
    unsigned* flags;
    int* abort_flag;
    int me, left, right;
    unsigned phase;
    int* lds_ok;
    long long spin_ticks;
    int fences;
#ifdef NK2D_FROZEN_CLOCKS
    long long ck_drain = 0, ck_wait = 0, ck_flag = 0;
#endif
    __device__ __forceinline__ void publish() {
#ifdef NK2D_FROZEN_CLOCKS
        const long long ck0 = (long long)__builtin_amdgcn_s_memrealtime();
        asm volatile("s_waitcnt vmcnt(0)" ::: "memory");
        ck_drain += (long long)__builtin_amdgcn_s_memrealtime() - ck0;
#else
        asm volatile("s_waitcnt vmcnt(0)" ::: "memory");
#endif
        if (fences) __builtin_amdgcn_fence(__ATOMIC_RELEASE, "agent");
        __syncthreads();
        ++phase;
        if (threadIdx.x == 0) __hip_atomic_store(flags + (size_t)me * 32, phase, __ATOMIC_RELAXED, __HIP_MEMORY_SCOPE_AGENT);
#ifdef NK2D_FROZEN_CLOCKS
        ck_flag = (long long)__builtin_amdgcn_s_memrealtime();
#endif
    }
    __device__ __forceinline__ bool wait() {
        if (threadIdx.x < 64) {
            const int lane = threadIdx.x;
            const int other = (lane == 0) ? left : ((lane == 1) ? right : -1);
            int good = 1;
            long long spins = 0;
            const long long t_begin = (long long)__builtin_amdgcn_s_memrealtime();
            for (;;) {
                unsigned v = phase;
                if (other >= 0) v = __hip_atomic_load(flags + (size_t)other * 32, __ATOMIC_RELAXED, __HIP_MEMORY_SCOPE_AGENT);
                if (__all((int)(v >= phase))) break;
                const int ab = __builtin_amdgcn_readfirstlane(
                    (lane == 0) ? __hip_atomic_load(abort_flag, __ATOMIC_RELAXED, __HIP_MEMORY_SCOPE_AGENT) : 0);
                const bool late = ((++spins & 63) == 0 || spin_ticks == 0) &&
                                  (long long)__builtin_amdgcn_s_memrealtime() - t_begin > spin_ticks;
                if (late || spins > 4000LL * NK2D_SPIN_LIMIT || ab != 0) {
                    if (lane == 0) __hip_atomic_store(abort_flag, 1, __ATOMIC_RELAXED, __HIP_MEMORY_SCOPE_AGENT);
                    good = 0;
                    break;
                }
                __builtin_amdgcn_s_sleep(1);
            }
            if (lane == 0) *lds_ok = good;
#ifdef NK2D_FROZEN_CLOCKS
            ck_wait += (long long)__builtin_amdgcn_s_memrealtime() - ck_flag;
#endif
        }
        __syncthreads();
        if (fences) __builtin_amdgcn_fence(__ATOMIC_ACQUIRE, "agent");
        return *lds_ok != 0;
    }
    __device__ __forceinline__ bool sync() {
        asm volatile("s_waitcnt vmcnt(0)" ::: "memory");
        if (fences) __builtin_amdgcn_fence(__ATOMIC_RELEASE, "agent");
        __syncthreads();
        ++phase;
        if (threadIdx.x < 64) {
            const int lane = threadIdx.x;
            if (lane == 0) __hip_atomic_store(flags + (size_t)me * 32, phase, __ATOMIC_RELAXED, __HIP_MEMORY_SCOPE_AGENT);
            const int other = (lane == 0) ? left : ((lane == 1) ? right : -1);
            int good = 1;
            long long spins = 0;
            const long long t_begin = (long long)__builtin_amdgcn_s_memrealtime();
            for (;;) {
                unsigned v = phase;
                if (other >= 0) v = __hip_atomic_load(flags + (size_t)other * 32, __ATOMIC_RELAXED, __HIP_MEMORY_SCOPE_AGENT);
                if (__all((int)(v >= phase))) break;
                const int ab = __builtin_amdgcn_readfirstlane(
                    (lane == 0) ? __hip_atomic_load(abort_flag, __ATOMIC_RELAXED, __HIP_MEMORY_SCOPE_AGENT) : 0);
                const bool late = ((++spins & 63) == 0 || spin_ticks == 0) &&
                                  (long long)__builtin_amdgcn_s_memrealtime() - t_begin > spin_ticks;
                if (late || spins > 4000LL * NK2D_SPIN_LIMIT || ab != 0) {
                    if (lane == 0) __hip_atomic_store(abort_flag, 1, __ATOMIC_RELAXED, __HIP_MEMORY_SCOPE_AGENT);
                    good = 0;
                    break;
                }
                __builtin_amdgcn_s_sleep(1);
            }
            if (lane == 0) *lds_ok = good;
        }
        __syncthreads();
        if (fences) __builtin_amdgcn_fence(__ATOMIC_ACQUIRE, "agent");
        return *lds_ok != 0;
    }
};

__device__ __forceinline__ int uni_i(int v) { return __builtin_amdgcn_readfirstlane(v); }
__device__ __forceinline__ bool uni_b(bool v) { return __builtin_amdgcn_readfirstlane((int)v) != 0; }
__device__ __forceinline__ double uni_d(double v) {
    const int lo = __builtin_amdgcn_readfirstlane(__double2loint(v));
    const int hi = __builtin_amdgcn_readfirstlane(__double2hiint(v));
    return __hiloint2double(hi, lo);
}



struct CacheRow {
    VmixArgs v;
    double cre, ccr, cci;
};

struct CachePtrs {
    double *KV, *J;
    double *fr_inv, *fc_invr, *fc_invi;
    double *fr_tab, *fc_tabr, *fc_tabi;
    size_t kv_len, np, nv, ntab;
};

struct PieceTab {
    double* const* base;
    int rows;
    size_t oJ, ofr, ofcr, ofci, otr, otcr, otci;
    size_t oS;
};

struct RowTabs {
    double *KV, *J, *fr_inv, *fc_invr, *fc_invi, *fr_tab, *fc_tabr, *fc_tabi;
    double* SRC;
};

__device__ __forceinline__ double* uni_p(double* p) {
    const unsigned long long v = (unsigned long long)p;
    const unsigned lo = (unsigned)__builtin_amdgcn_readfirstlane((int)(unsigned)v);
    const unsigned hi = (unsigned)__builtin_amdgcn_readfirstlane((int)(unsigned)(v >> 32));
    return (double*)(((unsigned long long)hi << 32) | lo);
}

__device__ __forceinline__ RowTabs piece_row_tabs(const CachePtrs& C, const PieceTab& T, double* b, int r) {
    RowTabs t;
    t.KV = b + (size_t)r * 3 * C.kv_len;
    t.J = b + T.oJ + (size_t)r * 5 * C.np;
    t.fr_inv = b + T.ofr + (size_t)r * C.nv;
    t.fc_invr = b + T.ofcr + (size_t)r * C.nv;
    t.fc_invi = b + T.ofci + (size_t)r * C.nv;
    t.fr_tab = b + T.otr + (size_t)r * C.ntab;
    t.fc_tabr = b + T.otcr + (size_t)r * C.ntab;
    t.fc_tabi = b + T.otci + (size_t)r * C.ntab;
    t.SRC = b + T.oS + (size_t)r * C.np;
    return t;
}

struct CachePiecePtrs {
    CachePtrs C;
    PieceTab T;
};
template <int PIECES> struct CacheArgOf { typedef CachePtrs type; };
template <> struct CacheArgOf<1> { typedef CachePiecePtrs type; };

template <int E, int MP, int FINAL>
__device__ __forceinline__ void newton_single_body(const DevP& P, const FusedArgs& A, int task, int lane, const FinalArgs* fin = nullptr) {
    const int tr = task / P.ny, j = task - tr * P.ny;
    const int cs_col = (j > 0) ? task - 1 : task, cn_col = (j < P.ny - 1) ? task + 1 : task;
    ColCoef<E> cf;
    load_coef<E>(P, j, lane, cf);
    double y0[E], ys[E], yn[E], zc[3][E], zs[3][E], zn[3][E], kvs[3][E], w0[E], w1[E], w2[E], jl[E], ju[E];
    load_col<E, MP>(A.st.y, task, lane, y0);
    load_col<E, MP>(A.st.y, cs_col, lane, ys);
    load_col<E, MP>(A.st.y, cn_col, lane, yn);
#pragma unroll
    for (int i = 0; i < 3; ++i) {
        load_col<E, MP>(A.st.z + i * A.st.nv, task, lane, zc[i]);
        load_col<E, MP>(A.st.z + i * A.st.nv, cs_col, lane, zs[i]);
        load_col<E, MP>(A.st.z + i * A.st.nv, cn_col, lane, zn[i]);
        load_col<E>(A.st.kv[i], j, lane, kvs[i]);
    }
    load_col<E>(A.st.w, task, lane, w0);
    load_col<E>(A.st.w + A.st.nv, task, lane, w1);
    load_col<E>(A.st.w + 2 * A.st.nv, task, lane, w2);
    load_col<E>(A.sw.JL, j, lane, jl);
    load_col<E>(A.sw.JU, j, lane, ju);
    double inv_r[E], tab_r[NK2D_TAB], t0[E], t1[E], tr0[NK2D_TAB], ti0[NK2D_TAB];
    load_col<E>(A.sw.fr_inv, task, lane, inv_r);
    load_tab<E>(A.sw.fr_tab, task, lane, tab_r);
    load_col<E>(A.sw.fc_invr, task, lane, t0);
    load_col<E>(A.sw.fc_invi, task, lane, t1);
    load_tab<E>(A.sw.fc_tabr, task, lane, tr0);
    load_tab<E>(A.sw.fc_tabi, task, lane, ti0);
    double fr[E], fcr[E], fci[E];
#pragma unroll
    for (int e = 0; e < E; ++e) { fr[e] = 0.0; fcr[e] = 0.0; fci[e] = 0.0; }
#pragma unroll
    for (int i = 0; i < 3; ++i) {
        double c[E], cs[E], cn[E], f[E];
#pragma unroll
        for (int e = 0; e < E; ++e) { c[e] = y0[e] + zc[i][e]; cs[e] = ys[e] + zs[i][e]; cn[e] = yn[e] + zn[i][e]; }
        tend_col<E, 0>(P, cf, c, cs, cn, kvs[i], tr, lane, f);
#pragma unroll
        for (int e = 0; e < E; ++e) {
            fr[e] = fr[e] + f[e] * cTI[0][i];
            fcr[e] = fcr[e] + f[e] * cTI[1][i];
            fci[e] = fci[e] + f[e] * cTI[2][i];
        }
    }
#pragma unroll
    for (int e = 0; e < E; ++e) {
        fr[e] = fr[e] - A.st.mreal * w0[e];
        fcr[e] = fcr[e] - (A.st.mcr * w1[e] - A.st.mci * w2[e]);
        fci[e] = fci[e] - (A.st.mcr * w2[e] + A.st.mci * w1[e]);
    }
    double a[E], cc[E];
    line_offdiag<E, 0>(P, tr, lane, jl, ju, a, cc);
#pragma unroll
    for (int e = 0; e < E; ++e) fr[e] = ((lane * E + e) < P.nz) ? fr[e] : 0.0;
    tridiag_apply<E, double>(a, cc, inv_r, tab_r, fr, lane);
    {
        cplx r[E], inv[E], tab[NK2D_TAB];
#pragma unroll
        for (int e = 0; e < E; ++e) inv[e] = c_make(t0[e], t1[e]);
#pragma unroll
        for (int i = 0; i < NK2D_TAB; ++i) tab[i] = c_make(tr0[i], ti0[i]);
#pragma unroll
        for (int e = 0; e < E; ++e) {
            const bool valid = (lane * E + e) < P.nz;
            r[e] = c_make(valid ? fcr[e] : 0.0, valid ? fci[e] : 0.0);
        }
        tridiag_apply<E, cplx>(a, cc, inv, tab, r, lane);
#pragma unroll
        for (int e = 0; e < E; ++e) { fcr[e] = r[e].re; fci[e] = r[e].im; }
    }
    double acc = 0.0;
#pragma unroll
    for (int e = 0; e < E; ++e) {
        const double sc = P.atol + fabs(y0[e]) * P.rtol;
        const double d0 = fr[e] / sc, d1 = fcr[e] / sc, d2 = fci[e] / sc;
        acc += (d0 * d0 + d1 * d1) + d2 * d2;
        w0[e] = w0[e] + fr[e];
        w1[e] = w1[e] + fcr[e];
        w2[e] = w2[e] + fci[e];
    }
    acc = wave_sum(acc);
    if (lane == 0) st_mp<0>(A.part + task, acc);
    double* wout = const_cast<double*>(A.st.w);
    if constexpr (FINAL) {
        double z0[E], z1[E], z2[E], ynw[E];
#pragma unroll
        for (int e = 0; e < E; ++e) {
            z0[e] = (cT[0][0] * w0[e] + cT[0][1] * w1[e]) + cT[0][2] * w2[e];
            z1[e] = (cT[1][0] * w0[e] + cT[1][1] * w1[e]) + cT[1][2] * w2[e];
            z2[e] = (cT[2][0] * w0[e] + cT[2][1] * w1[e]) + cT[2][2] * w2[e];
            ynw[e] = y0[e] + z2[e];
        }
        store_col<E, MP>(fin->ynew, task, lane, ynw);
        const double xs[3] = {fin->x0, fin->x1, fin->x2};
        double o[3][E];
#pragma unroll
        for (int e = 0; e < E; ++e) {
            double q[3];
#pragma unroll
            for (int cidx = 0; cidx < 3; ++cidx) q[cidx] = (z0[e] * cP[0][cidx] + z1[e] * cP[1][cidx]) + z2[e] * cP[2][cidx];
#pragma unroll
            for (int i = 0; i < 3; ++i) {
                const double p1 = xs[i], p2 = p1 * xs[i], p3 = p2 * xs[i];
                double v = (q[0] * p1 + q[1] * p2) + q[2] * p3;
                v = v + y0[e];
                o[i][e] = v - ynw[e];
            }
        }
#pragma unroll
        for (int i = 0; i < 3; ++i) store_col<E, MP>(fin->znext + i * A.st.nv, task, lane, o[i]);
        double wv[E];
#pragma unroll
        for (int r = 0; r < 3; ++r) {
#pragma unroll
            for (int e = 0; e < E; ++e) wv[e] = (cTI[r][0] * o[0][e] + cTI[r][1] * o[1][e]) + cTI[r][2] * o[2][e];
            store_col<E>(wout + r * A.st.nv, task, lane, wv);
        }
        return;
    }
    store_col<E>(wout, task, lane, w0);
    store_col<E>(wout + A.st.nv, task, lane, w1);
    store_col<E>(wout + 2 * A.st.nv, task, lane, w2);
    double zz[E];
#pragma unroll
    for (int r = 0; r < 3; ++r) {
#pragma unroll
        for (int e = 0; e < E; ++e) zz[e] = (cT[r][0] * w0[e] + cT[r][1] * w1[e]) + cT[r][2] * w2[e];
        store_col<E, MP>(A.st.zout + r * A.st.nv, task, lane, zz);
    }
}

struct FrozenRow {
    double mreal, mcr, mci;
    double x0, x1, x2;
    int n_iter, m;
    double h;
    int err;
    int upr;
    double cre, ccr, cci;
};

struct FrozenArgs {
    double *Y, *YOLD, *Z, *ZN, *W, *F;
    double *BR, *BCR, *BCI, *XR[2], *XCR[2], *XCI[2];
    double* PART;
    double* STEP_PART;
    const FrozenRow* rows;
    CachePtrs C;
    int n;
    unsigned* arrive;
    int* abort_flag;
    double* out;
    long long spin_ticks;
    int fences;
    int coef_lds;
#define NK2D_FROZEN_EARLY_OF(coef_lds) (((coef_lds) >> 8) & 1)
    int by_column;
    const double* SRC;
    int upr_on;
};

struct FrozenPieceArgs : FrozenArgs {
    PieceTab T;
};
template <int PIECES> struct FrozenArgOf { typedef FrozenArgs type; };
template <> struct FrozenArgOf<1> { typedef FrozenPieceArgs type; };

template <int E, int KIND, int MP>
__device__ __forceinline__ void tend_at_body(const DevP& P, const double* __restrict__ y, const double* __restrict__ kvp,
                                             double* __restrict__ f, int task, int lane) {
    const int tr = task / P.ny, j = task - tr * P.ny;
    const int cs_col = (j > 0) ? task - 1 : task, cn_col = (j < P.ny - 1) ? task + 1 : task;
    ColCoef<E> cf;
    load_coef<E>(P, j, lane, cf);
    double c[E], cs[E], cn[E], kv[E], ff[E];
    load_col<E, MP>(y, task, lane, c);
    load_col<E, MP>(y, cs_col, lane, cs);
    load_col<E, MP>(y, cn_col, lane, cn);
    load_col<E, MP>(kvp, j, lane, kv);
    tend_col<E, KIND>(P, cf, c, cs, cn, kv, tr, lane, ff);
    if constexpr (KIND == 2) forced_sources<E>(P, kvp, j, lane, c, ff);
    if constexpr (KIND == 1) {
        double u1[E], u2[E];
        phos_load_others<E>(P, tr, j, lane, y, u1, u2);
        phos_sources<E>(P, tr, j, lane, c, u1, u2, cf.dzr, ff);
    }
    store_col<E, MP>(f, task, lane, ff);
}

template <int E, int MP>
__device__ __forceinline__ void step_tail_body(const double* __restrict__ y, const double* __restrict__ z, size_t nv,
                                               const FinalArgs& fin, double* __restrict__ wout, int task, int lane) {
    double yy[E], z0[E], z1[E], z2[E], yn[E];
    load_col<E, MP>(y, task, lane, yy);
    load_col<E, MP>(z, task, lane, z0);
    load_col<E, MP>(z + nv, task, lane, z1);
    load_col<E, MP>(z + 2 * nv, task, lane, z2);
#pragma unroll
    for (int e = 0; e < E; ++e) yn[e] = yy[e] + z2[e];
    store_col<E, MP>(fin.ynew, task, lane, yn);
    const double xs[3] = {fin.x0, fin.x1, fin.x2};
    double o[3][E];
#pragma unroll
    for (int e = 0; e < E; ++e) {
        double q[3];
#pragma unroll
        for (int cidx = 0; cidx < 3; ++cidx) q[cidx] = (z0[e] * cP[0][cidx] + z1[e] * cP[1][cidx]) + z2[e] * cP[2][cidx];
#pragma unroll
        for (int i = 0; i < 3; ++i) {
            const double p1 = xs[i], p2 = p1 * xs[i], p3 = p2 * xs[i];
            double v = (q[0] * p1 + q[1] * p2) + q[2] * p3;
            v = v + yy[e];
            o[i][e] = v - yn[e];
        }
    }
#pragma unroll
    for (int i = 0; i < 3; ++i) store_col<E, MP>(fin.znext + i * nv, task, lane, o[i]);
    double wv[E];
#pragma unroll
    for (int r = 0; r < 3; ++r) {
#pragma unroll
        for (int e = 0; e < E; ++e) wv[e] = (cTI[r][0] * o[0][e] + cTI[r][1] * o[1][e]) + cTI[r][2] * o[2][e];
        store_col<E, MP>(wout + r * nv, task, lane, wv);
    }
}
```

### newton-krylov_ooc_amd/csrc/nk2d_common.h

```cpp
#pragma once

#include <hip/hip_runtime.h>
#include <stdint.h>
#include <string>
#include <mutex>
#include <vector>

#include "../../include/nk2d.h"

#define NK2D_WAVE 64
#define NK2D_WAVES_PER_BLOCK 4
#define NK2D_BLOCK (NK2D_WAVE * NK2D_WAVES_PER_BLOCK)
#define NK2D_MAX_E 8
#define NK2D_OWN_REC_CAP 65536
#define NK2D_CKPT_EVERY 128


#define NK2D_FROZEN_EARLY_DEFAULT 1
struct nk2d_ctx {
    nk2d_desc d;
    int nz, ny, tc, E, nzp, ncol, nreg;
    int kind;
    size_t nv;
    size_t np;
    int dev;
    hipStream_t stream_;
    std::string err;
    struct nk2d_stream_state* strm;
    int stream_years;
    int stream_two_waves;
    int stream_on;
    int stream_lost;
    int64_t stream_cmds, stream_launches, stream_timeouts, stream_years_run;
    int frozen_tape;
    struct nk2d_tape* tape;
    int tape_rec, tape_foreign;
    int64_t tape_years_run, tape_builds, tape_timeouts;
    int64_t tape_fallbacks;

    double* VV;
    double* KH;
    double* WT;
    double* WB;
    double* DZR;
    double* ZM0;
    double* ZM1;
    double* DM;
    double* DMR;
    double* DYR;
    double* BLDMAX;
    int32_t* MASK;
    double* WN;
    double *JL, *JU, *JS, *JN, *JC;
    double *LIGHT, *UPR, *YLIN;
    double *SMSREC, *RESTREC;
    double *sms_t, *rest_t;
    size_t kv_len;
    int ylin_set;
    double* KV[5];
    double* KVN[3];
    double* JB[5];
    double *Y, *YOLD, *F, *Z , *ZP , *W ;
    double* ZN ;
    int min_sweeps;
    std::vector<double> last_sched;
    std::vector<double> own_rec;
    std::vector<double> frozen_sched;
    int jac_stage_state;
    int final_fuse;
    int jac_stage;
    int team;
    int single_swap;
    int swap_updates;
    double *BR, *BCR, *BCI, *XR[2], *XCR[2], *XCI[2], *TMP, *TMP2;
    double *FR_INV, *FC_INVR, *FC_INVI;
    double *FR_TAB, *FC_TABR, *FC_TABI;
    float *FR32_INV, *FC32_INVR, *FC32_INVI, *FR32_TAB, *FC32_TABR, *FC32_TABI;
    int factor_fp32;
    hipEvent_t snap_ev[8];
    int snap_ready;
    int sweep_wpb;
    int jac_fresh;
    double growth_cap;
    double* PART;
    double* PART2;
    double* STEP_PART;
    size_t step_part_rows;
    double* STEP_NORM;
    int64_t frozen_fallbacks;
    void* frozen_cache;
    int frozen_persistent;
    int frozen_persistent_max_e;
    double frozen_cache_max_gb;
    int64_t frozen_cache_builds, frozen_persistent_years;
    int frozen_team;
    int frozen_wpb;
    int frozen_coef_lds;
    int frozen_lds_bits;
    int frozen_early;
    int frozen_early_bits;
    int frozen_by_column;
    int frozen_alloc_async;
    int frozen_cache_after;
    int frozen_cache_pieces;
    double frozen_cache_piece_mb;
    int64_t frozen_cache_piece_rows;
    int frozen_cache_lean;
    int64_t frozen_lean_years;
    uint64_t frozen_lean_mem_key;
    int frozen_forced;
    int64_t frozen_forced_years;
    int frozen_phosphorus;
    int frozen_phosphorus_shallow;
    int64_t frozen_phosphorus_shallow_years;
    int frozen_two_waves_last;
    int64_t frozen_phosphorus_years;
    int64_t frozen_two_waves_years;
    int frozen_cache_early;
    int64_t frozen_cache_piece_allocs, frozen_cache_early_requests;
    uint64_t frozen_seen_key; int frozen_seen_years;
    int64_t frozen_team_years;
    int64_t frozen_launch_us;
    double barrier_timeout_ms;
    int year_fences;
    int64_t frozen_resumes;
    int frozen_err_check;
    uint64_t grid_hash;
    std::vector<double*> ckpt;
    double* RED;
    double* hRED;
    double* hPART;
    double* hPART2;
    double* hPARTB;
    double* hPARTC;
    double* ZS ;
    int hook_spec_depth;
    int64_t cnt_spec_dropped, cnt_front_dropped, cnt_err_void, cnt_err_queued;
    double* part_cur;
    int part_on_host;
    int factor_pending;
    double lu_cre, lu_ccr, lu_cci;
    int speculate;
    double spec_bias;
    std::vector<double*> vec_pool;
    std::mutex pool_mutex;
    double* STAGE;
    double* hSTAGE;
    size_t stage_elems;
    struct nk2d_download_pool* dl_pool;
    double* RCOEF;
    double* hRCOEF;
    size_t rcoef_elems;

    std::vector<double> rho_tab;
    double rho_c0, rho_dlog;
    void* precond;
    int pc_fused;
    int pc_valu;
    int pc_fp32;
    int pc_refine;
    int pc_two_ended;
    int64_t pc_setup_rounds, pc_sub_launches;
    int pc_pivot_wave;
    int64_t pc_pivot_wave_steps;

    int hist_n, hist_next;
    const double* hist_t;
    double* hist_host;
    int stream_hist;
    double stream_hist_mb;
    double* HISTBUF;
    size_t hist_slots, hist_buf_elems;
    std::vector<int> hist_slot_k;
    int64_t hist_year_samples, hist_year_drains;
    int64_t stream_hist_samples, stream_hist_drains;

    nk2d_stats st;

    nk2d_norm_hook_fn norm_hook;
    void* norm_hook_user;
    nk2d_norm_hook_vec_fn norm_hook_vec;
    void* norm_hook_vec_user;
    double global_n;
    double *YR_PART, *YR_OUT, *hYR_OUT, *YR_REC;
    void* YR_SYNC;
    int* YR_MTAB;
    double yr_lin_tol;
    int64_t yr_rec_cap;
    hipEvent_t yr_ev[2];
    hipEvent_t timer_ev[2];
    int timer_ready;

    int prof_every;
    std::vector<hipEvent_t> prof_ev;
    size_t prof_used;
    double prof_ms_sum;
    double prof_overhead_ms;
    int64_t prof_cnt;
    int64_t sweep_launches;
    double fused_bytes_all;
    int64_t shape_cnt[4];
    double shape_bytes[4];
    double sweep_bytes;
    int64_t prof_windows;
    std::vector<int> prof_win_launches;
    int win_open, win_launches;
    int64_t win_seq;
    double win_bytes;
    int frozen_sums_poison = 0;
    int64_t frozen_step_sums_hash = 0;
};

#define NK2D_CHECK(ctx, call)                                                        \
    do {                                                                             \
        hipError_t e_ = (call);                                                      \
        if (e_ != hipSuccess) {                                                      \
            (ctx)->err = std::string(#call) + ": " + hipGetErrorString(e_) + " at " + \
                         __FILE__ + ":" + std::to_string(__LINE__);                  \
            return -1;                                                               \
        }                                                                            \
    } while (0)

#define NK2D_TRY(expr)            \
    do {                          \
        int rc_ = (expr);         \
        if (rc_ != 0) return rc_; \
    } while (0)

void nk2d_turn_take(int waves);
void nk2d_turn_give(int waves);
#define NK2D_RC_STREAM_LOST 17
int nk2d_stream_pause(nk2d_ctx* c);
bool nk2d_stream_running(const nk2d_ctx* c);
int nk2d_stream_columns_per_workgroup(const nk2d_ctx* c);
int nk2d_stream_two_waves(const nk2d_ctx* c);
int nk2d_stream_eligible(const nk2d_ctx* c);
int nk2d_stream_ready(nk2d_ctx* c);
int nk2d_stream_end(nk2d_ctx* c);
void nk2d_stream_free(nk2d_ctx* c);
int64_t nk2d_tape_size(const nk2d_ctx* c, int what);
void nk2d_tape_forget(nk2d_ctx* c);
int nk2d_stream_profile(nk2d_ctx* c, double* out12);
double* nk2d_stream_part_take(nk2d_ctx* c, const double* name);
const double* nk2d_stream_part_named(const nk2d_ctx* c, const double* name);
void nk2d_stream_part_forget(nk2d_ctx* c, const double* name);
int nk2d_stream_wait_part(nk2d_ctx* c, const double* part, int n);
static inline hipStream_t nk2d_s(nk2d_ctx* c) {
    if (c->tape_rec) c->tape_foreign++;
    if (c->strm && nk2d_stream_running(c)) (void)nk2d_stream_pause(c);
    return c->stream_;
}

static inline int nk2d_fail(nk2d_ctx* c, const std::string& msg, int code = -2) {
// ... 328 lines not shown
```

### newton-krylov_ooc_amd/csrc/nk2d_frozen.hip

```cpp
#include "nk2d_bodies.h"
#include "nk2d_frozen_plan.h"

#include <algorithm>
#ifdef NK2D_FROZEN_CLOCKS
#include <cstdio>
#endif
#include <vector>

__device__ __forceinline__ RowTabs cache_row_tabs(const CachePiecePtrs& C, int i) {
    const int p = i / C.T.rows;
    return piece_row_tabs(C.C, C.T, C.T.base[p], i - p * C.T.rows);
}

template <int E, int PIECES = 0>
__global__ void __launch_bounds__(NK2D_BLOCK) k_cache_planes(DevP P, const CacheRow* __restrict__ rows, typename CacheArgOf<PIECES>::type C, int n) {
    const int lane = threadIdx.x & 63;
    const long long task = (long long)blockIdx.x * (blockDim.x >> 6) + (threadIdx.x >> 6);
    const long long per_row = 4LL * P.ny;
    if (task >= per_row * n) return;
    const int i = (int)(task / per_row), rem = (int)(task - (long long)i * per_row);
    const int slot = rem / P.ny, j = rem - slot * P.ny;
    const CacheRow& R = rows[i];
    if (slot < 3) {
        double kv[E];
// ... 405 lines not shown
    fc->key = 0; fc->n = 0;
    std::vector<double*> give_back;
    if (g.replace) { give_back.swap(fc->blocks); fc->block_rows = 0; }
    if (g.in_thread) {
        frozen_request(fc, c->dev, pl, g, give_back);
        return 1;
    }
    for (double* p : give_back) (void)hipFree(p);
    std::vector<double*> got;
    NK2D_CHECK(c, frozen_alloc_blocks(g.count, g.block_bytes, &got));
    frozen_take_blocks(c, fc, pl, g, &got);
    return 0;
}

static int frozen_ensure_storage(nk2d_ctx* c, nk2d_frozen_cache* fc, const FrozenPlanIn& in, const FrozenPlan& pl, int64_t n) {
    if (pl.lean) NK2D_TRY(frozen_grow(c, (void**)&fc->lean_tab, &fc->lean_tab_doubles, 3 * in.nv + 3 * frozen_ntab(in), sizeof(double)));
    if (pl.src || pl.phos) NK2D_TRY(frozen_grow(c, (void**)&fc->upr, &fc->upr_doubles, pl.phos ? in.np : in.nv, sizeof(double)));
    NK2D_TRY(frozen_ensure_blocks(c, fc, in, pl, n));
    const size_t rows_want = pl.pieces ? (size_t)n : fc->block_rows;
    if (fc->rows_cap < rows_want) {
        size_t cap_r = fc->rows_cap, cap_f = fc->rows_cap;
        fc->rows_cap = 0;
        NK2D_TRY(frozen_grow(c, (void**)&fc->rows_dev, &cap_r, rows_want, sizeof(CacheRow)));
        NK2D_TRY(frozen_grow(c, (void**)&fc->frows_dev, &cap_f, rows_want, sizeof(FrozenRow)));
        fc->rows_cap = rows_want;
    }
    if (pl.pieces) {
        NK2D_TRY(frozen_grow(c, (void**)&fc->blocks_dev, &fc->blocks_dev_cap, fc->blocks.size(), sizeof(double*)));
        NK2D_CHECK(c, hipMemcpy(fc->blocks_dev, fc->blocks.data(), sizeof(double*) * fc->blocks.size(), hipMemcpyHostToDevice));
    }
    return 0;
}

static CachePtrs frozen_cache_ptrs(const nk2d_frozen_cache* fc, const FrozenLayout& L) {
    CachePtrs C = {};
    C.kv_len = L.kv_len; C.np = L.np; C.nv = L.nv; C.ntab = L.ntab;
    double* b = fc->pieces ? nullptr : fc->blocks[0];
    if (b) { C.KV = b; C.J = b + L.oJ; }
    if (L.lean) {
        double* p = fc->lean_tab;
        C.fr_inv = p; C.fc_invr = p + L.nv; C.fc_invi = p + 2 * L.nv;
        p += 3 * L.nv;
        C.fr_tab = p; C.fc_tabr = p + L.ntab; C.fc_tabi = p + 2 * L.ntab;
    } else if (b) {
        C.fr_inv = b + L.ofr; C.fc_invr = b + L.ofcr; C.fc_invi = b + L.ofci;
        C.fr_tab = b + L.otr; C.fc_tabr = b + L.otcr; C.fc_tabi = b + L.otci;
    }
    return C;
}
static PieceTab frozen_piece_tab(const nk2d_frozen_cache* fc, const FrozenLayout& L) {
    PieceTab T;
    T.base = fc->blocks_dev;
    T.rows = (int)L.B;
    T.oJ = L.oJ; T.ofr = L.ofr; T.ofcr = L.ofcr; T.ofci = L.ofci; T.otr = L.otr; T.otcr = L.otcr; T.otci = L.otci;
    T.oS = L.oS;
    return T;
}

static void frozen_fill_rows(nk2d_ctx* c, nk2d_frozen_cache* fc, const FrozenLayout& L, const double* sched, int64_t n, std::vector<CacheRow>* rows) {
    const double RCs[3] = {0.15505102572168222, 0.6449489742783178, 1.0};
    const double MU_REAL = 3.637834252744496, MU_CR = 2.6810828736277523, MU_CI = -3.050430199247411;
    auto at = [&](int64_t i, int slot) {
        const FrozenPlace p = frozen_place(L, (size_t)i, slot);
        return fc->blocks[p.block] + p.offset;
    };
    rows->assign((size_t)n, CacheRow());
    fc->frows.assign((size_t)n, FrozenRow());
    for (int64_t i = 0; i < n; ++i) {
        const double* r = sched + i * NK2D_SCHED_WIDTH;
        const double t = r[0], t_new = r[1], h = r[2], t_jac = r[4], h_lu = r[5];
        CacheRow& R = (*rows)[(size_t)i];
        double times[4];
        for (int k = 0; k < 3; ++k) times[k] = t + (h * RCs[k]);
        times[3] = t_jac;
        for (int k = 0; k < 4; ++k) {
            nk2d_host_interp(4, c->d.bld_tvals, c->d.bld_fvals, times[k], &R.v.frac[k]);
            R.v.out[k] = (k < 3) ? at(i, FROZEN_KV0 + k) : nullptr;
        }
        if (L.src) R.v.out[3] = at(i, FROZEN_SRC);
        vmix_forcing_args(c, L.src ? 4 : 3, times, R.v);
        R.v.bldmin = c->d.bldepth_min; R.v.y0 = c->d.vmix_log_shallow; R.v.y1 = c->d.vmix_log_deep; R.v.hw = c->d.vmix_half_width;
        R.cre = MU_REAL / h_lu; R.ccr = MU_CR / h_lu; R.cci = MU_CI / h_lu;
        FrozenRow& F = fc->frows[(size_t)i];
        F.mreal = MU_REAL / h; F.mcr = MU_CR / h; F.mci = MU_CI / h;
        F.n_iter = (int)r[3];
        int m_real = nk2d_sweeps_for(c, MU_REAL / h_lu), m_cplx = nk2d_sweeps_for(c, MU_CR / h_lu);
        if (c->min_sweeps > 1 && nk2d_has_lateral(c)) { m_real = std::max(m_real, 2); m_cplx = std::max(m_cplx, 2); }
        F.m = std::max(m_real, m_cplx);
        F.h = h;
        F.cre = R.cre; F.ccr = R.ccr; F.cci = R.cci;
        F.err = (c->frozen_err_check > 0 && i > 0 && i + 1 < n && (i % c->frozen_err_check) == 0 && F.m == 1 && F.n_iter >= 1) ? 1 : 0;
        F.upr = (i == 0 || t_jac != sched[(i - 1) * NK2D_SCHED_WIDTH + 4]) ? 1 : 0;
        F.x0 = F.x1 = F.x2 = 1.0;
        if (i + 1 < n) {
            const double h2 = r[NK2D_SCHED_WIDTH + 2];
            F.x0 = ((t_new + h2 * RCs[0]) - t) / (t_new - t);
            F.x1 = ((t_new + h2 * RCs[1]) - t) / (t_new - t);
            F.x2 = ((t_new + h2 * RCs[2]) - t) / (t_new - t);
        }
    }
}

template <int PIECES>
static int frozen_build_tables(nk2d_ctx* c, const CacheRow* rows_dev, typename CacheArgOf<PIECES>::type C, int64_t n, bool lean) {
    DevP P = make_devp(c);
    const long long tasks = 4LL * c->ny * n;
    NK2D_DISPATCH_E(c->E, hipLaunchKernelGGL((k_cache_planes<EE, PIECES>), dim3((unsigned)((tasks + 3) / 4)), dim3(NK2D_BLOCK), 0, nk2d_s(c),
                                              P, rows_dev, C, (int)n));
    NK2D_CHECK(c, hipGetLastError());
    c->st.nlaunch += 1;
    if (lean) return 0;
    const long long ftasks = 2LL * c->ncol * n;
    NK2D_DISPATCH_EK(c->E, c->kind, hipLaunchKernelGGL((k_cache_factor<EE, KK, PIECES>), dim3((unsigned)((ftasks + 3) / 4)), dim3(NK2D_BLOCK), 0,
                                                       nk2d_s(c), P, rows_dev, C, (int)n));
    NK2D_CHECK(c, hipGetLastError());
    c->st.nlaunch += 1;
    return 0;
}

static int frozen_build(nk2d_ctx* c, nk2d_frozen_cache* fc, const FrozenPlanIn& in, const FrozenPlan& pl, const double* sched, int64_t n) {
    const FrozenLayout L = frozen_layout(in, fc->block_rows, fc->lean, fc->src);
    std::vector<CacheRow> rows;
    frozen_fill_rows(c, fc, L, sched, n, &rows);
    NK2D_CHECK(c, hipMemcpyAsync(fc->rows_dev, rows.data(), sizeof(CacheRow) * (size_t)n, hipMemcpyHostToDevice, nk2d_s(c)));
    NK2D_CHECK(c, hipMemcpyAsync(fc->frows_dev, fc->frows.data(), sizeof(FrozenRow) * (size_t)n, hipMemcpyHostToDevice, nk2d_s(c)));
    NK2D_CHECK(c, hipStreamSynchronize(nk2d_s(c)));
    if (pl.pieces) {
        CachePiecePtrs CP;
        CP.C = frozen_cache_ptrs(fc, L);
        CP.T = frozen_piece_tab(fc, L);
        NK2D_TRY(frozen_build_tables<1>(c, fc->rows_dev, CP, n, pl.lean));
    } else {
        NK2D_TRY(frozen_build_tables<0>(c, fc->rows_dev, frozen_cache_ptrs(fc, L), n, pl.lean));
    }
    fc->key = pl.key;
    fc->n = n;
    c->frozen_cache_builds++;
    return 0;
}

static bool frozen_holds(const nk2d_frozen_cache* fc, const FrozenPlan& pl) {
    if (fc->pieces != pl.pieces || fc->lean != pl.lean || fc->src != pl.src || fc->blocks.empty()) return false;
    if (!pl.pieces) return true;
    if (fc->block_rows != pl.B || fc->blocks.size() < pl.need || !fc->blocks_dev || fc->blocks_dev_cap < pl.need) return false;
    for (size_t p = 0; p < pl.need; ++p)
        if (!fc->blocks[p]) return false;
    return true;
}

static int frozen_year_buffers(nk2d_ctx* c) {
    if (c->YR_OUT) return 0;
    NK2D_CHECK(c, hipMalloc((void**)&c->YR_PART, sizeof(double) * 2 * c->ncol));
    NK2D_CHECK(c, hipMalloc((void**)&c->YR_OUT, sizeof(double) * 32));
    NK2D_CHECK(c, hipMalloc((void**)&c->YR_SYNC, yr_sync_bytes(c)));
    NK2D_CHECK(c, hipMalloc((void**)&c->YR_MTAB, sizeof(int) * std::max<size_t>(c->rho_tab.size(), 1)));
    NK2D_CHECK(c, hipHostMalloc((void**)&c->hYR_OUT, sizeof(double) * 32));
    NK2D_CHECK(c, hipEventCreate(&c->yr_ev[0]));
    NK2D_CHECK(c, hipEventCreate(&c->yr_ev[1]));
    c->yr_lin_tol = -1.0;
    c->yr_rec_cap = 0;
    c->YR_REC = nullptr;
    return 0;
}

static int frozen_year_args(nk2d_ctx* c, const nk2d_frozen_cache* fc, const FrozenPlanIn& in, const FrozenPlan& pl, int64_t n, DevP* P, FrozenPieceArgs* Ap) {
    const FrozenLayout L = frozen_layout(in, fc->block_rows, fc->lean, fc->src);
    FrozenPieceArgs& A = *Ap;
    A = {};
    if (pl.pieces) A.T = frozen_piece_tab(fc, L);
    A.Y = c->Y; A.YOLD = c->YOLD; A.Z = c->Z; A.ZN = c->ZN; A.W = c->W; A.F = c->F;
    A.BR = c->BR; A.BCR = c->BCR; A.BCI = c->BCI;
    for (int i = 0; i < 2; ++i) { A.XR[i] = c->XR[i]; A.XCR[i] = c->XCR[i]; A.XCI[i] = c->XCI[i]; }
    A.PART = c->YR_PART;
    A.STEP_PART = c->STEP_PART;
    A.rows = fc->frows_dev;
    A.C = frozen_cache_ptrs(fc, L);
    A.n = (int)n;
    A.arrive = (unsigned*)c->YR_SYNC; A.abort_flag = (int*)((char*)c->YR_SYNC + 4096);
    A.out = c->YR_OUT;
    A.spin_ticks = (long long)(c->barrier_timeout_ms * 1.0e5);
    A.fences = c->year_fences;
    A.upr_on = (pl.src || pl.phos) ? 1 : 0;
    A.SRC = (pl.src && !pl.pieces) ? fc->blocks[0] + L.oS : nullptr;
    *P = make_devp(c);
    if (pl.src || pl.phos) P->UPR = fc->upr;
    NK2D_TRY(frozen_fit_lds(c, in, pl, &A.coef_lds, &A.by_column));
    c->frozen_lds_bits = A.coef_lds;
    c->frozen_early_bits = (A.coef_lds & 48) == 48 ? c->frozen_early : 0;
    A.coef_lds |= c->frozen_early_bits << 8;
    return 0;
}

static int frozen_launch_year(nk2d_ctx* c, const FrozenPlan& pl, int64_t n, DevP& P, FrozenPieceArgs& A) {
    const bool team = c->frozen_team && c->E <= 2 && !pl.phos;
    const dim3 grid((unsigned)(team ? c->ncol : nk2d_grid(c->ncol)));
    NK2D_CHECK(c, hipMemsetAsync(c->YR_SYNC, 0, yr_sync_bytes(c), nk2d_s(c)));
    NK2D_CHECK(c, hipMemsetAsync(c->YR_OUT, 0, sizeof(double) * 32, nk2d_s(c)));
    NK2D_CHECK(c, hipEventRecord(c->yr_ev[0], nk2d_s(c)));
    {
        struct Turn {
            int waves;
            explicit Turn(int w) : waves(w) { nk2d_turn_take(waves); }
            ~Turn() { nk2d_turn_give(waves); }
        } turn(team ? 4 * c->ncol : c->ncol);
        hipError_t rc = hipErrorInvalidValue;
        bool two = false;
        if (pl.phos) rc = launch_frozen_phos_flavour(c, pl.pieces, P, A, false, &two);
        else if (pl.lean) rc = pl.pieces ? launch_frozen<1, 1>(c, team, grid, P, A) : launch_frozen<0, 1>(c, team, grid, P, static_cast<FrozenArgs&>(A));
        else rc = pl.pieces ? launch_frozen<1, 0>(c, team, grid, P, A) : launch_frozen<0, 0>(c, team, grid, P, static_cast<FrozenArgs&>(A));
        c->frozen_two_waves_last = two ? 1 : 0;
        if (rc == hipErrorCooperativeLaunchTooLarge) { (void)hipGetLastError(); return 1; }
        NK2D_CHECK(c, rc);
        NK2D_CHECK(c, hipEventRecord(c->yr_ev[1], nk2d_s(c)));
        NK2D_CHECK(c, hipMemcpyAsync(c->hYR_OUT, c->YR_OUT, sizeof(double) * 32, hipMemcpyDeviceToHost, nk2d_s(c)));
        NK2D_CHECK(c, hipStreamSynchronize(nk2d_s(c)));
    }
    const double* o = c->hYR_OUT;
    if ((int)o[0] != 0 || (int64_t)o[1] != n) return 2;
#ifdef NK2D_FROZEN_CLOCKS
    std::fprintf(stderr, "frozen clocks (early %d): %.0f phases, per phase drain %.3f us, flag store to poll match %.3f us, rest %.3f us; kernel %.3f ms\n",
                 c->frozen_early_bits, o[11], 0.01 * o[8] / o[11], 0.01 * o[9] / o[11], 0.01 * (o[10] - o[8] - o[9]) / o[11], 1.0e-5 * o[10]);
#endif
    if (team) c->frozen_team_years++;
    float ms = 0.f;
    NK2D_CHECK(c, hipEventElapsedTime(&ms, c->yr_ev[0], c->yr_ev[1]));
    c->frozen_launch_us += (int64_t)(1000.0 * (double)ms);
    if ((int)o[2]) std::swap(c->Y, c->YOLD);
    if ((int)o[3]) std::swap(c->Z, c->ZN);
    return 0;
}

static void frozen_book_year(nk2d_ctx* c, const nk2d_frozen_cache* fc, int64_t n, std::vector<char>* err_rows) {
    for (int64_t i = 0; i < n; ++i) {
        const FrozenRow& F = fc->frows[(size_t)i];
        c->st.nnewton += F.n_iter; c->st.nfev += 3 * (int64_t)F.n_iter; c->st.nsolve += 2 * (int64_t)F.n_iter;
        c->st.nsweeps += (int64_t)F.n_iter * F.m;
        double words = 0.0;
        for (int it = 0; it < F.m; ++it) words += fused_words(c, it == 0, it == 0, it == F.m - 1, F.m == 2, false);
        c->fused_bytes_all += 8.0 * words * F.n_iter;
    }
    if (err_rows) {
        err_rows->assign((size_t)n, 0);
        for (int64_t i = 0; i < n; ++i)
            if (fc->frows[(size_t)i].err) { (*err_rows)[(size_t)i] = 1; c->st.nerr_checked++; c->st.nfev++; c->st.nsolve++; }
    }
    c->sweep_launches += 1;
    c->st.nsteps += n - 1;
    c->st.njev += n; c->st.nlu += 2 * n;
    c->st.nlaunch += 1;
}

int nk2d_frozen_persistent(nk2d_ctx* c, const double* sched, int64_t n, std::vector<char>* err_rows) {
    const FrozenPlanIn in = frozen_plan_in(c);
    if (!frozen_eligible(in, sched, n)) return 1;
    FrozenPlan pl;
    NK2D_TRY(frozen_make_plan(c, in, sched, n, &pl));
    if (pl.phos) NK2D_TRY(frozen_phos_resident(c, in, pl));
    nk2d_frozen_cache* fc = frozen_store(c);
    NK2D_TRY(frozen_thread_done(c, fc));
    NK2D_TRY(frozen_drop_other_form(c, fc, pl));
    NK2D_TRY(frozen_admitted(c, in, pl, n));
    if (fc->key != pl.key || fc->n != n) {
        NK2D_TRY(frozen_deferred(c, in, pl));
        NK2D_TRY(frozen_ensure_storage(c, fc, in, pl, n));
        NK2D_TRY(frozen_build(c, fc, in, pl, sched, n));
    }
    if (!frozen_holds(fc, pl)) return 1;
    NK2D_TRY(frozen_year_buffers(c));
    DevP P;
    FrozenPieceArgs A;
    NK2D_TRY(frozen_year_args(c, fc, in, pl, n, &P, &A));
    NK2D_TRY(frozen_launch_year(c, pl, n, P, A));
    frozen_book_year(c, fc, n, err_rows);
    return 0;
}

int nk2d_frozen_cache_early(nk2d_ctx* c, const double* sched, int64_t n) {
    if (!c->frozen_cache_pieces || !c->frozen_cache_early || !sched) return 0;
    const FrozenPlanIn in = frozen_plan_in(c);
    if (!frozen_eligible(in, sched, n)) return 0;
    auto quiet = [](int rc) { return rc < 0 ? rc : 0; };
    FrozenPlan pl;
    int rc = frozen_make_plan(c, in, sched, n, &pl);
    if (rc) return quiet(rc);
    nk2d_frozen_cache* fc = frozen_store(c);
    if ((rc = frozen_thread_done(c, fc)) != 0) return quiet(rc);
    NK2D_TRY(frozen_drop_other_form(c, fc, pl));
    const FrozenHeld held = frozen_held(c);
    if (!frozen_must_grow(pl, held, n)) return 0;
    if ((rc = frozen_admitted(c, in, pl, n)) != 0) return quiet(rc);
    frozen_request(fc, c->dev, pl, frozen_growth(in, pl, held, n, 0.0), {});
    c->frozen_cache_early_requests++;
    return 0;
}
```

### newton-krylov_ooc_amd/csrc/nk2d_frozen_body.inc

```
    constexpr int XCD = 0, NB = 1;
    __shared__ int lds_ok;
    __shared__ double team_lds[TEAM ? sizeof(TeamLds<E, 3>) / sizeof(double) : 1];
    constexpr int MPX = XCD ? 2 : 1;
    const int lane = threadIdx.x & 63;
    int wg = (int)blockIdx.x;
    const int tw = uni_i((int)(threadIdx.x >> 6));
    const bool by_col = !TEAM && !XCD && NB != 0 && A.by_column != 0;
    const int wave = TEAM ? uni_i(wg) : (by_col ? uni_i(tw * P.ny + wg) : uni_i(wg * (int)(blockDim.x >> 6) + (int)(threadIdx.x >> 6)));
    const bool col_wave = wave < P.ncol && (!by_col || (tw < P.tc && wg < P.ny));
    int nb_left, nb_right;
    if constexpr (TEAM) {
        const int nb_j = wave % P.ny;
        nb_left = (nb_j > 0) ? wg - 1 : -1;
        nb_right = (nb_j < P.ny - 1) ? wg + 1 : -1;
    } else if (by_col) {
        nb_left = (wg > 0) ? wg - 1 : -1;
        nb_right = (wg < P.ny - 1) ? wg + 1 : -1;
    } else {
        const int wpb = (int)(blockDim.x >> 6);
        const int c0 = wg * wpb, cl = min(c0 + wpb - 1, P.ncol - 1);
        nb_left = (c0 % P.ny > 0) ? wg - 1 : -1;
        nb_right = (cl % P.ny < P.ny - 1) ? wg + 1 : -1;
    }
    NeighbourSync nbs{(unsigned*)((char*)A.arrive + 8192), A.abort_flag, wg, nb_left, nb_right, 0u, &lds_ok, A.spin_ticks, A.fences};
#ifdef NK2D_FROZEN_CLOCKS
    const long long ck_begin = (long long)__builtin_amdgcn_s_memrealtime();
#endif
    const size_t nv = A.C.nv;
    int swapY = 0, swapZ = 0, status = 0, done = 0;
    int pc_p = 0, pc_r = 0;
    (void)pc_p; (void)pc_r;
#define FZ_Y (swapY ? A.YOLD : A.Y)
#define FZ_YOLD (swapY ? A.Y : A.YOLD)
#define FZ_Z (swapZ ? A.ZN : A.Z)
#define FZ_ZN (swapZ ? A.Z : A.ZN)
#define FZ_SYNC() \
    if (!nbs.sync()) { status = 1; goto finish; }
#define FZ_OWN_DEAD() \
    if constexpr (OWN) { \
        _Pragma("unroll") for (int r_ = 0; r_ < 3; ++r_) { \
            _Pragma("unroll") for (int e_ = 0; e_ < E; ++e_) own.z[r_][e_] = 0.0; \
        } \
    }
    constexpr bool COEF_LDS = NB != 0 && !TEAM && !XCD && E >= 3;
    extern __shared__ double dyn_lds[];
    const bool w_in_lds = COEF_LDS && (A.coef_lds & 2) != 0;
    const bool step_in_lds = COEF_LDS && by_col && (A.coef_lds & 4) != 0;
    const bool piv_in_lds = COEF_LDS && by_col && (A.coef_lds & 8) != 0;
    constexpr bool OWN = COEF_LDS && NK2D_FROZEN_OWN(E, KIND, TEAM, LEAN);
    const int own_bits = OWN && by_col ? (A.coef_lds & 48) : 0;
    (void)own_bits;
    const int nwv = (int)(blockDim.x >> 6);
    double* my_coef;
    double* my_w;
    double* step_lds = nullptr;
    double* my_piv = nullptr;
    double* my_y = nullptr;
    if (by_col) {
        double* p = dyn_lds;
        my_coef = p; p += NK2D_COEF_LDS_DOUBLES(E);
        step_lds = p; p += step_in_lds ? 5 * E * 64 : 0;
        my_w = p + (size_t)tw * (3 * E * 64); p += w_in_lds ? (size_t)nwv * 3 * E * 64 : 0;
        my_piv = p + (size_t)tw * (E * 64); p += piv_in_lds ? (size_t)nwv * E * 64 : 0;
        my_y = p + (size_t)tw * (E * 64);
    } else {
        my_coef = dyn_lds + (size_t)(threadIdx.x >> 6) * (NK2D_COEF_LDS_DOUBLES(E) + (w_in_lds ? 3 * E * 64 : 0));
        my_w = my_coef + NK2D_COEF_LDS_DOUBLES(E);
    }
    const LdsSrc L = {my_coef, my_w, step_lds, my_piv, my_y};
    (void)L;
    OwnState<OWN ? E : 1> own;
    own.valid = 0;
    if constexpr (OWN) {
#pragma unroll
        for (int r = 0; r < 3; ++r) {
#pragma unroll
            for (int e = 0; e < E; ++e) own.z[r][e] = 0.0;
        }
    }
    if constexpr (COEF_LDS) {
        if (A.coef_lds && col_wave && (!by_col || tw == 0)) {
            ColCoef<E> cf;
            load_coef<E>(P, wave % P.ny, lane, cf);
            store_coef_lds<E>(my_coef, lane, cf);
        }
        if (by_col && A.coef_lds) __syncthreads();
    }
    int lds_step = -1;
    (void)lds_step;
    LateNorm late = {0.0, nullptr, (OWN && by_col && own_bits == 48) ? uni_i(NK2D_FROZEN_EARLY_OF(A.coef_lds)) : 0, 0};
    (void)late;
    if (col_wave && (!TEAM || tw == 0)) {
        double zero[E];
#pragma unroll
        for (int e = 0; e < E; ++e) zero[e] = 0.0;
#pragma unroll
        for (int i = 0; i < 3; ++i) {
            store_col<E, MPX>(FZ_Z + i * nv, wave, lane, zero);
            store_col<E, (TEAM ? MPX : 0)>(A.W + i * nv, wave, lane, zero);
            if constexpr (COEF_LDS) {
                if (w_in_lds) w_lds_put<E>(my_w, i, lane, zero);
            }
        }
    }
    FZ_SYNC()
    for (int i = 0; i < A.n; ++i) {
        const FrozenRow R = A.rows[i];
        const int n_iter = uni_i(R.n_iter), m = uni_i(R.m);
        const bool last_row = i == A.n - 1;
        RowTabs T = {};
        const double* kv_prev = nullptr;
        (void)T; (void)kv_prev;
        if constexpr (PIECES) {
            double* const base = uni_p(A.T.base[pc_p]);
            T = piece_row_tabs(A.C, A.T, base, pc_r);
            if (i > 0 && uni_i(R.err) != 0) {
                const double* pb = pc_r > 0 ? base : uni_p(A.T.base[pc_p - 1]);
                const int pr = pc_r > 0 ? pc_r - 1 : A.T.rows - 1;
                kv_prev = pb + ((size_t)pr * 3 + 2) * A.C.kv_len;
            }
            if (++pc_r == A.T.rows) { pc_r = 0; ++pc_p; }
        }
        const double* kvb = PIECES ? T.KV : A.C.KV + (size_t)i * 3 * A.C.kv_len;
        const double* J = PIECES ? T.J : A.C.J + (size_t)i * 5 * A.C.np;
        if constexpr (KIND == 1 && LEAN) {
            if (A.upr_on != 0 && uni_i(R.upr) != 0 && col_wave) {
                phos_upr_col<E, 0>(P, FZ_Y, const_cast<double*>(P.UPR), wave % P.ny, lane);
                asm volatile("s_waitcnt vmcnt(0)" ::: "memory");
            }
        }
        if constexpr (KIND == 2 && LEAN) {
            if (A.upr_on != 0 && uni_i(R.upr) != 0 && col_wave) {
                const double* sp = PIECES ? T.SRC : A.SRC + (size_t)i * A.C.np;
                forced_upr_col<E, MPX>(P, FZ_Y, sp, const_cast<double*>(P.UPR), wave % P.ny, lane);
                asm volatile("s_waitcnt vmcnt(0)" ::: "memory");
            }
        }
        const bool with_err = uni_i(R.err) != 0 && !last_row && i > 0;
        if (with_err) {
            if (col_wave && (!TEAM || tw == 0))
                tend_at_body<E, KIND, MPX>(P, FZ_Y, PIECES ? kv_prev : A.C.KV + ((size_t)(i - 1) * 3 + 2) * A.C.kv_len, A.F, wave, lane);
            FZ_SYNC()
        }
        for (int k = 0; k < n_iter; ++k) {
            int src = 0;
            for (int it = 0; it < m; ++it) {
                const bool do_stage = it == 0, first = it == 0, do_update = it == m - 1, delta = m == 2;
                const bool is_final = do_update && k == n_iter - 1 && !last_row && !with_err;
                FusedArgs FA = {};
                FA.st.y = FZ_Y; FA.st.z = FZ_Z; FA.st.w = A.W;
                FA.st.zout = (do_stage && do_update) ? FZ_ZN : FZ_Z;
                FA.st.kv[0] = kvb; FA.st.kv[1] = kvb + A.C.kv_len; FA.st.kv[2] = kvb + 2 * A.C.kv_len;
                FA.st.br = A.BR; FA.st.bcr = A.BCR; FA.st.bci = A.BCI;
                FA.st.nv = nv; FA.st.mreal = R.mreal; FA.st.mcr = R.mcr; FA.st.mci = R.mci;
                FA.sw.JL = J; FA.sw.JU = J + A.C.np; FA.sw.JS = J + 2 * A.C.np; FA.sw.JN = J + 3 * A.C.np; FA.sw.JC = J + 4 * A.C.np;
                const bool fac = LEAN != 0 && k == 0 && it == 0;
                const DevP& PK = *(const DevP*)__builtin_amdgcn_kernarg_segment_ptr();
                (void)PK;
                if constexpr (LEAN) {
                    FA.sw.fr_inv = A.C.fr_inv; FA.sw.fc_invr = A.C.fc_invr; FA.sw.fc_invi = A.C.fc_invi;
                    FA.sw.fr_tab = A.C.fr_tab; FA.sw.fc_tabr = A.C.fc_tabr; FA.sw.fc_tabi = A.C.fc_tabi;
                    FA.sw.cre = R.cre; FA.sw.ccr = R.ccr; FA.sw.cci = R.cci;
                } else if constexpr (PIECES) {
                    FA.sw.fr_inv = T.fr_inv; FA.sw.fc_invr = T.fc_invr; FA.sw.fc_invi = T.fc_invi;
                    FA.sw.fr_tab = T.fr_tab; FA.sw.fc_tabr = T.fc_tabr; FA.sw.fc_tabi = T.fc_tabi;
                } else {
                    FA.sw.fr_inv = A.C.fr_inv + (size_t)i * nv; FA.sw.fc_invr = A.C.fc_invr + (size_t)i * nv;
                    FA.sw.fc_invi = A.C.fc_invi + (size_t)i * nv;
                    FA.sw.fr_tab = A.C.fr_tab + (size_t)i * A.C.ntab; FA.sw.fc_tabr = A.C.fc_tabr + (size_t)i * A.C.ntab;
                    FA.sw.fc_tabi = A.C.fc_tabi + (size_t)i * A.C.ntab;
                }
                FA.sw.f32 = 0;
                FA.sw.br = A.BR; FA.sw.bcr = A.BCR; FA.sw.bci = A.BCI;
                FA.sw.xr_old = src ? A.XR[1] : A.XR[0]; FA.sw.xcr_old = src ? A.XCR[1] : A.XCR[0];
                FA.sw.xci_old = src ? A.XCI[1] : A.XCI[0];
                FA.sw.xr_new = src ? A.XR[0] : A.XR[1]; FA.sw.xcr_new = src ? A.XCR[0] : A.XCR[1];
                FA.sw.xci_new = src ? A.XCI[0] : A.XCI[1];
                FA.sw.first = first ? 1 : 0;
                FA.part = (k == n_iter - 1) ? A.STEP_PART + (size_t)(3 * i) * P.ncol
                                            : ((k == n_iter - 2) ? A.STEP_PART + (size_t)(3 * i + 1) * P.ncol
                                                                 : ((!TEAM && E >= 3) ? nullptr : A.PART));
                FA.do_stage = do_stage ? 1 : 0; FA.do_update = do_update ? 1 : 0; FA.delta = delta ? 1 : 0;
                if constexpr (COEF_LDS) {
                    if (step_in_lds && lds_step != i) {
                        for (int r = tw; r < 5; r += nwv) {
                            double v[E];
                            const double* src = (r == 0) ? FA.st.kv[0] : ((r == 1) ? FA.st.kv[1] : ((r == 2) ? FA.st.kv[2]
                                                : ((r == 3) ? FA.sw.JL : FA.sw.JU)));
                            load_col<E, MPX>(src, wave % P.ny, lane, v);
                            w_lds_put<E>(step_lds, r, lane, v);
                        }
                        if constexpr (!LEAN) {
                        if (piv_in_lds && col_wave) {
                            double v[E];
                            load_col<E>(FA.sw.fr_inv, wave, lane, v);
                            w_lds_put<E>(my_piv, 0, lane, v);
                        }
                        }
                        lds_step = i;
                        __syncthreads();
                    }
                }
                if (is_final) {
                    FinalArgs Fin;
                    Fin.ynew = FZ_YOLD;
                    Fin.znext = do_stage ? FZ_ZN : FZ_Z;
                    Fin.x0 = R.x0; Fin.x1 = R.x1; Fin.x2 = R.x2;
                    Fin.nblk_cols = 0;
                    if constexpr (TEAM) {
                        if constexpr (LEAN) {
                            if (col_wave && fac)
                                newton_team_body<E, KIND, 1, 1, 4, 1, MPX>(PK, FA, *reinterpret_cast<TeamLds<E, 3>*>(team_lds), wave, tw, lane, &Fin);
                        }
                        if (col_wave && !fac)
                            newton_team_body<E, KIND, 0, 1, 4, 1, MPX>(P, FA, *reinterpret_cast<TeamLds<E, 3>*>(team_lds), wave, tw, lane, &Fin);
                    } else if (col_wave && fac) {
                        if constexpr (LEAN && COEF_LDS) frozen_factor_phase<E, KIND, MPX, 1>(PK, FA, wave, lane, &Fin, &L, A.coef_lds, w_in_lds, piv_in_lds ? my_piv : nullptr);
                        else if constexpr (LEAN) newton_fused_body<E, KIND, 1, 1, MPX, 1>(PK, FA, wave, lane, &Fin);
                    } else if (col_wave) {
                        bool taken = false;
                        if constexpr (KIND == 0 && E <= 2) {
                            if (m == 1) { newton_single_body<E, MPX, 1>(P, FA, wave, lane, &Fin); taken = true; }
                        }
                        if constexpr (OWN) {
                            if (own_bits == 48) { newton_fused_body<E, KIND, 0, 1, MPX, 1, 191>(P, FA, wave, lane, &Fin, &L, &own, &late); taken = true; }
                            else if (!PIECES && own_bits == 32) { newton_fused_body<E, KIND, 0, 1, MPX, 1, 47>(P, FA, wave, lane, &Fin, &L, &own); taken = true; }
                            else if (own_bits == 16) { newton_fused_body<E, KIND, 0, 1, MPX, 1, 31>(P, FA, wave, lane, &Fin, &L, &own); FZ_OWN_DEAD() taken = true; }
                        }
                        if constexpr (COEF_LDS) {
                            if (taken) {}
                            else if (step_in_lds && piv_in_lds) { newton_fused_body<E, KIND, 0, 1, MPX, 1, 15>(P, FA, wave, lane, &Fin, &L); FZ_OWN_DEAD() taken = true; }
                            else if (step_in_lds) { newton_fused_body<E, KIND, 0, 1, MPX, 1, 7>(P, FA, wave, lane, &Fin, &L); FZ_OWN_DEAD() taken = true; }
                            else if (w_in_lds) { newton_fused_body<E, KIND, 0, 1, MPX, 1, 3>(P, FA, wave, lane, &Fin, &L); FZ_OWN_DEAD() taken = true; }
                            else if (A.coef_lds) { newton_fused_body<E, KIND, 0, 1, MPX, 1, 1>(P, FA, wave, lane, &Fin, &L); FZ_OWN_DEAD() taken = true; }
                        }
                        if (!taken) { newton_fused_body<E, KIND, 0, 1, MPX, 1>(P, FA, wave, lane, &Fin); FZ_OWN_DEAD() }
                    }
                    swapY ^= 1;
                    if (do_stage) swapZ ^= 1;
                } else {
                    if constexpr (TEAM) {
                        if constexpr (LEAN) {
                            if (col_wave && fac)
                                newton_team_body<E, KIND, 1, 1, 4, 0, MPX>(PK, FA, *reinterpret_cast<TeamLds<E, 3>*>(team_lds), wave, tw, lane, nullptr);
                        }
                        if (col_wave && !fac)
                            newton_team_body<E, KIND, 0, 1, 4, 0, MPX>(P, FA, *reinterpret_cast<TeamLds<E, 3>*>(team_lds), wave, tw, lane, nullptr);
                    } else if (col_wave && fac) {
                        if constexpr (LEAN && COEF_LDS) frozen_factor_phase<E, KIND, MPX, 0>(PK, FA, wave, lane, nullptr, &L, A.coef_lds, w_in_lds, piv_in_lds ? my_piv : nullptr);
                        else if constexpr (LEAN) newton_fused_body<E, KIND, 1, 1, MPX, 0>(PK, FA, wave, lane);
                    } else if (col_wave) {
                        bool taken = false;
                        if constexpr (KIND == 0 && E <= 2) {
                            if (m == 1) { newton_single_body<E, MPX, 0>(P, FA, wave, lane); taken = true; }
                        }
                        if constexpr (OWN) {
                            if (own_bits == 48) { newton_fused_body<E, KIND, 0, 1, MPX, 0, 191>(P, FA, wave, lane, nullptr, &L, &own, &late); taken = true; }
                            else if (!PIECES && own_bits == 32) { newton_fused_body<E, KIND, 0, 1, MPX, 0, 47>(P, FA, wave, lane, nullptr, &L, &own); taken = true; }
                            else if (own_bits == 16) { newton_fused_body<E, KIND, 0, 1, MPX, 0, 31>(P, FA, wave, lane, nullptr, &L, &own); FZ_OWN_DEAD() taken = true; }
                        }
                        if constexpr (COEF_LDS) {
                            if (taken) {}
                            else if (step_in_lds && piv_in_lds) { newton_fused_body<E, KIND, 0, 1, MPX, 0, 15>(P, FA, wave, lane, nullptr, &L); FZ_OWN_DEAD() taken = true; }
                            else if (step_in_lds) { newton_fused_body<E, KIND, 0, 1, MPX, 0, 7>(P, FA, wave, lane, nullptr, &L); FZ_OWN_DEAD() taken = true; }
                            else if (w_in_lds) { newton_fused_body<E, KIND, 0, 1, MPX, 0, 3>(P, FA, wave, lane, nullptr, &L); FZ_OWN_DEAD() taken = true; }
                            else if (A.coef_lds) { newton_fused_body<E, KIND, 0, 1, MPX, 0, 1>(P, FA, wave, lane, nullptr, &L); FZ_OWN_DEAD() taken = true; }
                        }
                        if (!taken) { newton_fused_body<E, KIND, 0, 1, MPX, 0>(P, FA, wave, lane); FZ_OWN_DEAD() }
                    }
                    if (do_stage && do_update) swapZ ^= 1;
                }
                src = 1 - src;
                if constexpr (OWN) {
                    nbs.publish();
                    if (late.pending) {
                        if (lane == 0) st_mp<MPX>(late.part, late.acc);
                        late.pending = 0;
                    }
                    if (!nbs.wait()) { status = 1; goto finish; }
                } else {
                    FZ_SYNC()
                }
            }
        }
        if (with_err) {
            if (col_wave && (!TEAM || tw == 0)) {
                ErrArgs EA = {};
                EA.sw.JL = J; EA.sw.JU = J + A.C.np; EA.sw.JS = J + 2 * A.C.np; EA.sw.JN = J + 3 * A.C.np; EA.sw.JC = J + 4 * A.C.np;
                EA.sw.fr_inv = LEAN ? A.C.fr_inv : (PIECES ? T.fr_inv : A.C.fr_inv + (size_t)i * nv);
                EA.sw.fr_tab = LEAN ? A.C.fr_tab : (PIECES ? T.fr_tab : A.C.fr_tab + (size_t)i * A.C.ntab);
                EA.sw.xr_old = A.XR[0]; EA.sw.xr_new = A.XR[1];
                EA.f = A.F; EA.z = FZ_Z; EA.y = FZ_Y; EA.nv = nv; EA.h = R.h;
                EA.part = A.STEP_PART + (size_t)(3 * i + 2) * P.ncol;
                EA.stage = 0; EA.last = 1;
                err_fused_body<E, KIND, MPX>(P, EA, wave, lane);
            }
            FZ_SYNC()
            if (col_wave && (!TEAM || tw == 0)) {
                FinalArgs Fin;
                Fin.ynew = FZ_YOLD;
                Fin.znext = FZ_ZN;
                Fin.x0 = R.x0; Fin.x1 = R.x1; Fin.x2 = R.x2;
                Fin.nblk_cols = 0;
                step_tail_body<E, MPX>(FZ_Y, FZ_Z, nv, Fin, A.W, wave, lane);
                own.valid = 0;
                if constexpr (COEF_LDS) {
                    if (w_in_lds) {
                        asm volatile("s_waitcnt vmcnt(0)" ::: "memory");
#pragma unroll
                        for (int r = 0; r < 3; ++r) {
                            double wv[E];
                            load_col<E, (TEAM ? MPX : 0)>(A.W + r * nv, wave, lane, wv);
                            w_lds_put<E>(my_w, r, lane, wv);
                        }
                    }
                }
            }
            swapY ^= 1;
            swapZ ^= 1;
            FZ_SYNC()
        }
        done = i + 1;
    }
finish:
    if constexpr (COEF_LDS) {
        if (w_in_lds && col_wave) {
#pragma unroll
            for (int r = 0; r < 3; ++r) {
                double wv[E];
                w_lds_get<E>(my_w, r, lane, wv);
                store_col<E>(A.W + r * nv, wave, lane, wv);
            }
        }
    }
    if (status != 0 && threadIdx.x == 0) A.out[0] = (double)status;
#ifdef NK2D_FROZEN_CLOCKS
    if (wg == (int)(gridDim.x / 2) && threadIdx.x == 0) {
        A.out[8] = (double)nbs.ck_drain; A.out[9] = (double)nbs.ck_wait;
        A.out[10] = (double)((long long)__builtin_amdgcn_s_memrealtime() - ck_begin); A.out[11] = (double)nbs.phase;
    }
#endif
    if (wg == 0 && threadIdx.x == 0) {
        A.out[1] = (double)done; A.out[2] = (double)swapY; A.out[3] = (double)swapZ; A.out[4] = (double)nbs.phase;
    }
#undef FZ_SYNC
#undef FZ_OWN_DEAD
#undef FZ_Y
#undef FZ_YOLD
#undef FZ_Z
#undef FZ_ZN
```

### newton-krylov_ooc_amd/csrc/nk2d_frozen_plan.h

```cpp
#pragma once

#include <algorithm>
#include <cmath>
#include <cstddef>
#include <cstdint>
#include <initializer_list>

#define NK2D_WAVES_PER_BLOCK 4
#define NK2D_TAB 14
#define NK2D_SCHED_WIDTH 8
#define NK2D_COEF_LDS_DOUBLES(E) ((7 * (E) + 1) * 64)

#define NK2D_FROZEN_OWN(E, KIND, TEAM, LEAN) ((E) >= 5 && (E) <= 7 && ((KIND) == 0 || (KIND) == 2) && !(TEAM) && !(LEAN))

struct FrozenPlanIn {
    int E, kind, tc, ny, ncol;
    size_t np, nv, kv_len;
    int sms_nrec;
    double sink_thres, t0;
    int frozen_persistent, frozen_persistent_max_e, frozen_forced, frozen_phosphorus;
    int frozen_phosphorus_shallow;
    int frozen_cache_lean, frozen_cache_pieces;
    double frozen_cache_piece_mb;
    int64_t frozen_cache_piece_rows;
    double frozen_cache_max_gb;
    int frozen_cache_after, frozen_alloc_async, frozen_err_check;
    int frozen_coef_lds, frozen_by_column, frozen_wpb, frozen_team;
    int factor_fp32, jac_stage_state, hist_n;
    bool norm_hook;
};

struct FrozenHeld {
    bool pieces = false, lean = false, src = false;
    size_t blocks = 0, block_rows = 0;
    int alloc_state = 0;
    bool alloc_lean = false;
    uint64_t key = 0;
    int64_t n = 0;
    size_t rows() const { return blocks * block_rows; }
};

static inline bool frozen_thres(const FrozenPlanIn& in) { return in.kind == 2 && in.sms_nrec > 0 && in.sink_thres > 0.0; }

static inline bool frozen_phos(const FrozenPlanIn& in) {
    const int e_min = in.frozen_phosphorus_shallow != 0 ? 1 : 3;
    return in.kind == 1 && in.frozen_phosphorus != 0 && in.frozen_cache_lean != 0 && in.E >= e_min && in.E <= 8 && in.tc <= NK2D_WAVES_PER_BLOCK;
}

static inline size_t frozen_ntab(const FrozenPlanIn& in) { return (size_t)in.ncol * NK2D_TAB * 64; }

static inline size_t frozen_row_doubles(const FrozenPlanIn& in, bool lean, bool src) {
    return 3 * in.kv_len + 5 * in.np + (lean ? 0 : 3 * in.nv + 3 * frozen_ntab(in)) + (src ? in.np : 0);
}

static inline size_t frozen_piece_rows(const FrozenPlanIn& in, bool lean, bool src) {
    if (in.frozen_cache_piece_rows > 0) return (size_t)in.frozen_cache_piece_rows;
    const double fit = std::floor(in.frozen_cache_piece_mb * 1048576.0 / (8.0 * (double)frozen_row_doubles(in, lean, src)));
    return fit >= 1.0 ? (size_t)std::min(fit, 1.0e9) : (size_t)1;
}

static inline double frozen_held_bytes(const FrozenPlanIn& in, const FrozenHeld& h) {
    return 8.0 * (double)h.rows() * (double)frozen_row_doubles(in, h.lean, h.src);
}

static inline bool frozen_admit(double bytes, double free_bytes, double held_bytes) { return !(1.02 * bytes > 0.85 * (free_bytes + held_bytes)); }

static inline bool frozen_eligible(const FrozenPlanIn& in, const double* sched, int64_t n) {
    const bool thres = frozen_thres(in);
    const bool phos = frozen_phos(in);
    const bool needs_state = (in.kind == 1 && !phos) || (thres && !((in.frozen_forced & 2) && in.frozen_cache_lean != 0));
    if (!in.frozen_persistent || needs_state || in.hist_n != 0 || in.norm_hook || n < 1) return false;
    if (in.factor_fp32) return false;
    if (in.E > in.frozen_persistent_max_e || in.E > 8) return false;
    if (in.E > 4 && in.kind != 0 && !phos && !(in.kind == 2 && (in.frozen_forced & (thres ? 2 : 1)))) return false;
    if (thres || phos) {
        const double RCs[3] = {0.15505102572168222, 0.6449489742783178, 1.0};
        double t_jac_prev = in.t0;
        for (int64_t i = 0; i < n; ++i) {
            const double* r = sched + i * NK2D_SCHED_WIDTH;
            const double t = r[0], h = r[2], t_jac = r[4];
            if (t_jac != t_jac_prev && t_jac != t) {
                bool at_stage = false;
                for (int k = 0; k < 3 && in.jac_stage_state; ++k) at_stage = at_stage || t_jac == t + (h * RCs[k]);
                if (!at_stage) return false;
            }
            t_jac_prev = t_jac;
        }
    }
    for (int64_t i = 0; i + 1 < n; ++i) {
        const double* r = sched + i * NK2D_SCHED_WIDTH;
        if (!(r[0] + r[2] == r[1] && r[NK2D_SCHED_WIDTH] == r[1] && r[NK2D_SCHED_WIDTH + 2] > 0.0 && (int)r[3] >= 1)) return false;
    }
    return (int)sched[(n - 1) * NK2D_SCHED_WIDTH + 3] >= 1;
}

static inline uint64_t frozen_sched_hash(const double* sched, int64_t n) {
    uint64_t h = 14695981039346656037ull;
    const unsigned char* p = (const unsigned char*)sched;
    const size_t nb = sizeof(double) * (size_t)n * NK2D_SCHED_WIDTH;
    for (size_t i = 0; i < nb; ++i) { h ^= p[i]; h *= 1099511628211ull; }
    return h ? h : 1;
}
static inline uint64_t frozen_key_full(const FrozenPlanIn& in, uint64_t sched_hash, uint64_t fingerprint) {
    return sched_hash ^ fingerprint ^ ((uint64_t)(in.frozen_err_check + 1) * 0x9E3779B97F4A7C15ull);
}
static const uint64_t FROZEN_LEAN_KEY = 0xC2B2AE3D27D4EB4Full;
static const uint64_t FROZEN_SRC_KEY = 0x165667B19E3779F9ull;
static const uint64_t FROZEN_PHOS_KEY = 0x27D4EB2F165667C5ull;
static inline uint64_t frozen_form_key(uint64_t key_full, bool lean, bool src, bool phos) {
    return key_full ^ (lean ? FROZEN_LEAN_KEY : 0) ^ (src ? FROZEN_SRC_KEY : 0) ^ (phos ? FROZEN_PHOS_KEY : 0);
}

static inline int frozen_form(const FrozenPlanIn& in, int64_t n, uint64_t key_full, const FrozenHeld& held, uint64_t lean_mem_key,
                              const double* free_bytes, bool* ruled) {
    *ruled = false;
    if (frozen_thres(in) || in.kind == 1) return 1;
    if (in.frozen_cache_lean != 2) return in.frozen_cache_lean == 1 ? 1 : 0;
    if (held.alloc_state != 0) return held.alloc_lean ? 1 : 0;
    const bool pieces = in.frozen_cache_pieces != 0;
    const size_t B = pieces ? frozen_piece_rows(in, false, false) : 1, rows = ((size_t)n + B - 1) / B * B;
    const double bytes = 8.0 * (double)rows * (double)frozen_row_doubles(in, false, false);
    if (bytes > in.frozen_cache_max_gb * 1.0e9) return 1;
    const bool holds = held.blocks != 0;
    if (holds && !held.lean && held.pieces == pieces) {
        if (pieces ? (held.block_rows == B && held.rows() >= rows) : held.rows() >= (size_t)n) return 0;
    }
    if (holds && held.lean && held.n == n && held.key == (key_full ^ FROZEN_LEAN_KEY) && lean_mem_key == key_full) return 1;
    if (!free_bytes) return -1;
    *ruled = true;
    return frozen_admit(bytes, *free_bytes, frozen_held_bytes(in, held)) ? 0 : 1;
}

struct FrozenPlan {
    bool pieces, lean, src, phos;
    size_t per_row;
    size_t B, need;
    double bytes;
    bool allowed;
    uint64_t key;
};
static inline FrozenPlan frozen_plan(const FrozenPlanIn& in, int64_t n, uint64_t key_full, bool lean) {
    FrozenPlan pl;
    pl.pieces = in.frozen_cache_pieces != 0;
    pl.lean = lean;
    pl.src = frozen_thres(in);
    pl.phos = in.kind == 1;
    pl.per_row = frozen_row_doubles(in, pl.lean, pl.src);
    pl.B = pl.pieces ? frozen_piece_rows(in, pl.lean, pl.src) : 0;
    pl.need = pl.pieces ? ((size_t)n + pl.B - 1) / pl.B : 0;
    pl.bytes = 8.0 * (double)(pl.pieces ? pl.need * pl.B : (size_t)n) * (double)pl.per_row;
    pl.allowed = !(pl.bytes > in.frozen_cache_max_gb * 1.0e9);
    pl.key = frozen_form_key(key_full, pl.lean, pl.src, pl.phos);
    return pl;
}

static inline bool frozen_other_form(const FrozenPlan& pl, const FrozenHeld& held) {
    if (held.blocks == 0) return false;
    return held.pieces != pl.pieces || held.lean != pl.lean || held.src != pl.src || (pl.pieces && held.block_rows != pl.B);
}

static inline bool frozen_must_grow(const FrozenPlan& pl, const FrozenHeld& held, int64_t n) {
    return pl.pieces ? held.blocks < pl.need : held.rows() < (size_t)n;
}

static inline int frozen_years_before_build(const FrozenPlanIn& in, double bytes) {
    return in.frozen_cache_after >= 0 ? in.frozen_cache_after : (bytes > 8.0e9 ? 3 : 0);
// ... 94 lines not shown
```

### newton-krylov_ooc_amd/engine.py

```python

import ctypes
import os

import numpy as np

from . import _lib
from .grid import BLDEPTH_MIN, YEAR, bldepth_time_knots


DEFAULT_LIN_TOL = 3.0e-2
DEFAULT_JAC_FRESH = 1
DEFAULT_JAC_STAGE = 1
DEFAULT_GROWTH_CAP = 0.0


class Nk2dError(RuntimeError):
    pass


class Nk2dFrozenMismatch(Nk2dError):
    """a frozen year (comp_fcn_frozen) whose recorded Newton iteration counts do not converge for the state given"""


class Nk2dScheduleMismatch(Nk2dError):
# ... 15 lines not shown
        raise ValueError(f"schedule rows must have 6 or {_lib.SCHED_WIDTH} columns")
    return np.ascontiguousarray(sched)


class DevVec:

    __slots__ = ("eng", "ptr")

    def __init__(self, eng, ptr):
        self.eng = eng
        self.ptr = ptr

    def __del__(self):
        eng, ptr = self.eng, self.ptr
        self.ptr = None
        if ptr is not None and eng is not None and eng._handle is not None:
            eng._lib.nk2d_vec_free(eng._handle, ptr)

    def to_host(self):
        return self.eng.download(self)

    def copy(self):
        res = self.eng.new_vec()
        self.eng._chk(self.eng._lib.nk2d_vec_copy(self.eng._ctx, res.ptr, self.ptr))
        return res


class PendingDownload:

    __slots__ = ("eng", "ticket")

    def __init__(self, eng, ticket):
        self.eng = eng
        self.ticket = ticket

    def result(self):
        eng, ticket = self.eng, self.ticket
        if ticket is None:
            raise RuntimeError("download already taken")
        self.ticket = None
        host = np.empty(eng.shape)
        if eng._handle is None:
            raise RuntimeError("download: the engine was closed before its values were taken")
        if eng._lib.nk2d_vec_download_end(eng._handle, ticket, _dp(host)) != 0:
            raise RuntimeError("nk2d_vec_download_end: the copy to the host failed")
        return host

    def __del__(self):
        eng, ticket = self.eng, self.ticket
        self.ticket = None
        if ticket is not None and eng is not None and eng._handle is not None:
            eng._lib.nk2d_vec_download_end(eng._handle, ticket, None)


class ModuleEngine:

    def __init__(self, grid, tc, surf_rate=(), decay_rate=(), const_src=0.0, surf_target=(),
                 device_id=0,
                 time_range=(0.0, YEAR), rtol=1.0e-6, atol=1.0e-6, max_step_frac=0.01,
                 lin_tol=None, module_kind=0, phos_params=None, light_lim=None,
                 restore_series=None, sms_series=None, sink_thres=None):
        self._lib = _lib.load()
        self._handle = None
        self.grid = grid
        self.nz = len(grid.depth)
        self.ny = len(grid.ypos)
        self.tc = int(tc)
        self._device_id = int(device_id)
        self.shape = (self.tc, self.nz, self.ny)
        self.nreg = 1
        desc = _lib.Desc()
        desc.nz, desc.ny, desc.tc, desc.device_id = self.nz, self.ny, self.tc, int(device_id)
        keep = [np.ascontiguousarray(a, dtype=np.float64) for a in (
            grid.depth.edges, grid.ypos.edges, grid.vvel, grid.wvel, grid.hmix_coeff,
            grid.bldepth_max)]
        (desc.depth_edges, desc.ypos_edges, desc.vvel, desc.wvel, desc.hmix_coeff,
         desc.bldepth_max) = [_dp(a) for a in keep]
        desc.bldepth_min = BLDEPTH_MIN
        tvals, fvals = bldepth_time_knots()
        desc.bld_tvals = (ctypes.c_double * 4)(*tvals)
        desc.bld_fvals = (ctypes.c_double * 4)(*fvals)
        desc.vmix_log_shallow = float(np.log(1.0e1))
        desc.vmix_log_deep = float(np.log(5.0e-4))
        desc.vmix_half_width = 20.0
        surf = list(surf_rate) + [0.0] * (_lib.MAX_TRACERS - len(surf_rate))
        decay = list(decay_rate) + [0.0] * (_lib.MAX_TRACERS - len(decay_rate))
        target = list(surf_target) + [0.0] * (_lib.MAX_TRACERS - len(surf_target))
        desc.surf_rate = (ctypes.c_double * _lib.MAX_TRACERS)(*surf)
        desc.surf_target = (ctypes.c_double * _lib.MAX_TRACERS)(*target)
        desc.decay_rate = (ctypes.c_double * _lib.MAX_TRACERS)(*decay)
        desc.const_src = float(const_src)
        desc.t0, desc.t1 = float(time_range[0]), float(time_range[1])
        desc.rtol, desc.atol = float(rtol), float(atol)
        desc.max_step_frac = float(max_step_frac)
        if lin_tol is None:
            lin_tol = float(os.environ.get("NK2D_LIN_TOL", DEFAULT_LIN_TOL))
        desc.lin_tol = float(lin_tol)
        desc.module_kind = int(module_kind)
        if module_kind == 1:
            keep.append(np.ascontiguousarray(light_lim, dtype=np.float64))
            assert keep[-1].shape == (self.nz, self.ny)
            desc.light_lim = _dp(keep[-1])
            desc.phos_params = (ctypes.c_double * 6)(*[float(v) for v in phos_params])
        if module_kind == 2:
            if restore_series is not None:
                times, vals = [np.ascontiguousarray(a, dtype=np.float64) for a in restore_series]
                assert vals.shape == (len(times), self.ny)
                keep += [times, vals]
                desc.restore_nrec, desc.restore_times, desc.restore_vals = len(times), _dp(times), _dp(vals)
            if sms_series is not None:
                times, vals = [np.ascontiguousarray(a, dtype=np.float64) for a in sms_series]
                assert vals.shape == (len(times), self.nz, self.ny)
                keep += [times, vals]
                desc.sms_nrec, desc.sms_times, desc.sms_vals = len(times), _dp(times), _dp(vals)
            desc.sink_thres = 0.0 if sink_thres is None else float(sink_thres)
        self.state_dependent_precond = module_kind == 2 and sms_series is not None and bool(sink_thres)
        self.module_kind = int(module_kind)
        self.light_lim = keep[-1] if module_kind == 1 else None
        self.phos = dict(zip(PHOSPHORUS_PARAM_NAMES, phos_params)) if module_kind == 1 else None
        ctx = ctypes.c_void_p()
        rc = self._lib.nk2d_create(ctypes.byref(desc), ctypes.byref(ctx))
        if rc != 0:
            msg = self._lib.nk2d_last_error(ctx).decode() if ctx else "allocation failed"
            if ctx:
                self._lib.nk2d_destroy(ctx)
            raise Nk2dError(f"nk2d_create failed ({rc}): {msg}")
        self._handle = ctx
        self.device_ctl = 0
        self._precond_ready = False
        if "NK2D_STREAM_YEARS" in os.environ:
            self.set_option("stream_years", float(os.environ["NK2D_STREAM_YEARS"]))
        if "NK2D_FROZEN_TAPE" in os.environ:
            self.set_option("frozen_tape", float(os.environ["NK2D_FROZEN_TAPE"]))
        if "NK2D_STREAM_HIST" in os.environ:
            self.set_option("stream_hist", float(os.environ["NK2D_STREAM_HIST"]))
        if "NK2D_STREAM_HIST_MB" in os.environ:
            self.set_option("stream_hist_mb", float(os.environ["NK2D_STREAM_HIST_MB"]))
        if "NK2D_FROZEN_CACHE_PIECES" in os.environ:
            self.set_option("frozen_cache_pieces", float(os.environ["NK2D_FROZEN_CACHE_PIECES"]))
        if "NK2D_FROZEN_CACHE_PIECE_MB" in os.environ:
            self.set_option("frozen_cache_piece_mb", float(os.environ["NK2D_FROZEN_CACHE_PIECE_MB"]))
        if "NK2D_FROZEN_CACHE_EARLY" in os.environ:
            self.set_option("frozen_cache_early", float(os.environ["NK2D_FROZEN_CACHE_EARLY"]))
        if "NK2D_FROZEN_CACHE_LEAN" in os.environ:
            self.set_option("frozen_cache_lean", float(os.environ["NK2D_FROZEN_CACHE_LEAN"]))
        if "NK2D_FROZEN_FORCED" in os.environ:
            self.set_option("frozen_forced", float(os.environ["NK2D_FROZEN_FORCED"]))
        if "NK2D_FROZEN_PHOSPHORUS" in os.environ:
            self.set_option("frozen_phosphorus", float(os.environ["NK2D_FROZEN_PHOSPHORUS"]))
        if "NK2D_FROZEN_PHOSPHORUS_SHALLOW" in os.environ:
            self.set_option("frozen_phosphorus_shallow", float(os.environ["NK2D_FROZEN_PHOSPHORUS_SHALLOW"]))
        if "NK2D_FROZEN_EARLY" in os.environ:
            self.set_option("frozen_early", float(os.environ["NK2D_FROZEN_EARLY"]))
        if "NK2D_PC_TWO_ENDED" in os.environ:
            self.set_option("pc_two_ended", float(os.environ["NK2D_PC_TWO_ENDED"]))
        if "NK2D_PC_PIVOT_WAVE" in os.environ:
            self.set_option("pc_pivot_wave", float(os.environ["NK2D_PC_PIVOT_WAVE"]))
        self.set_option("jac_fresh", float(os.environ.get("NK2D_JAC_FRESH", DEFAULT_JAC_FRESH)))
        self.set_option("growth_cap", float(os.environ.get("NK2D_GROWTH_CAP", DEFAULT_GROWTH_CAP)))
        self.set_option("jac_stage", float(os.environ.get("NK2D_JAC_STAGE", DEFAULT_JAC_STAGE)))

    @property
    def _ctx(self):
        if self._handle is None:
            raise Nk2dError("this engine is closed (ModelState.reset_class / ModuleEngine.close)")
        return self._handle

    def close(self):
        if self._handle is not None:
            from . import trail

            trail.drain()
            self._lib.nk2d_destroy(self._handle)
            self._handle = None

    def __del__(self):
        try:
            self.close()
        except Exception:
            pass

    def _chk(self, rc):
        if rc == -7:
            raise Nk2dFrozenMismatch(f"nk2d call failed ({rc}): {self._lib.nk2d_last_error(self._ctx).decode()}")
        if rc == -8:
            raise Nk2dScheduleMismatch(f"nk2d call failed ({rc}): {self._lib.nk2d_last_error(self._ctx).decode()}")
        if rc != 0:
            raise Nk2dError(f"nk2d call failed ({rc}): {self._lib.nk2d_last_error(self._ctx).decode()}")

    def set_region(self, mask, weight):
        mask = np.ascontiguousarray(mask, dtype=np.int32)
        weight = np.ascontiguousarray(weight, dtype=np.float64)
        if mask.shape != (self.nz, self.ny) or weight.shape != (self.nz, self.ny):
            raise ValueError("region mask / weight must have shape (nz, ny)")
        nreg = int(mask.max())
        self._chk(self._lib.nk2d_set_region(
            self._ctx, mask.ctypes.data_as(_lib.c_int32_p), _dp(weight), nreg))
        self.nreg = nreg
        self._region = (mask, weight)
        self._ones_vec = None

    def new_vec(self):
        ptr = ctypes.c_void_p()
        self._chk(self._lib.nk2d_vec_alloc(self._ctx, ctypes.byref(ptr)))
        return DevVec(self, ptr)

    def upload(self, host, out=None):
        host = np.ascontiguousarray(host, dtype=np.float64).reshape(self.shape)
        out = self.new_vec() if out is None else out
        self._chk(self._lib.nk2d_vec_upload(self._ctx, out.ptr, _dp(host)))
        return out

    def download(self, vec):
        host = np.empty(self.shape)
        self._chk(self._lib.nk2d_vec_download(self._ctx, vec.ptr, _dp(host)))
        return host

    def download_begin(self, vec):
        ticket = ctypes.c_void_p()
        self._chk(self._lib.nk2d_vec_download_begin(self._ctx, vec.ptr, ctypes.byref(ticket)))
        return PendingDownload(self, ticket)

    def vec_tensor(self, vec):
        import torch

        nv = self.tc * self.ny * ((self.nz + 63) // 64) * 64

        class _Holder:
            pass

        holder = _Holder()
        holder.__cuda_array_interface__ = {"shape": (nv,), "typestr": "<f8", "data": (int(vec.ptr.value), False),
                                           "version": 2, "strides": None}
        holder._keep = vec
        return torch.as_tensor(holder, device=torch.device("cuda", self._device_id))

    def set_option(self, name, value):
        self._chk(self._lib.nk2d_set_option(self._ctx, name.encode(), float(value)))
        if name == "device_ctl":
            self.device_ctl = int(value)

    def sync(self):
        self._chk(self._lib.nk2d_sync(self._ctx))

    def tend(self, t, y, out=None):
        out = self.new_vec() if out is None else out
        self._chk(self._lib.nk2d_tend(self._ctx, float(t), y.ptr, out.ptr))
        return out

    def vmix_coeff(self, t):
        host = np.empty((self.nz - 1, self.ny))
        self._chk(self._lib.nk2d_vmix_coeff(self._ctx, float(t), _dp(host)))
        return host

    def jacobian_diags(self, t):
        host = np.empty((5, self.tc, self.nz, self.ny))
        self._chk(self._lib.nk2d_jacobian_diags(self._ctx, float(t), _dp(host)))
        return host

    def set_lin_state(self, y):
        self._chk(self._lib.nk2d_set_lin_state(self._ctx, y.ptr))

    def jacobian_apply(self, t, v):
        out = self.new_vec()
        self._chk(self._lib.nk2d_jacobian_apply(self._ctx, float(t), v.ptr, out.ptr))
        return out

    def shifted_solve(self, t_jac, h, mu, b_re, b_im=None):
        mu = complex(mu)
        x_re = self.new_vec()
        x_im = self.new_vec() if mu.imag != 0.0 else None
        sweeps = ctypes.c_int32()
        self._chk(self._lib.nk2d_shifted_solve(
            self._ctx, float(t_jac), float(h), mu.real, mu.imag, b_re.ptr,
            b_im.ptr if b_im is not None else None, x_re.ptr,
            x_im.ptr if x_im is not None else None, ctypes.byref(sweeps)))
        return x_re, x_im, sweeps.value

    def comp_fcn(self, x, out=None, replay=None, record=False, record_cap=65536):
        out = self.new_vec() if out is None else out
        stats = _lib.Stats()
        rp, rn = None, 0
        if replay is not None:
            replay = sched_rows(replay)
            rp, rn = _dp(replay), replay.shape[0]
        rec, recn = None, ctypes.c_int64(0)
        if record:
            rec = np.zeros((record_cap, _lib.SCHED_WIDTH))
        self._chk(self._lib.nk2d_comp_fcn(
            self._ctx, x.ptr, out.ptr, ctypes.byref(stats), rp, rn,
            _dp(rec) if rec is not None else None, record_cap if record else 0,
            ctypes.byref(recn)))
        sched = rec[: recn.value].copy() if record else None
        return out, stats.as_dict(), sched

    def comp_fcn_frozen(self, x, sched, out=None):
        out = self.new_vec() if out is None else out
        stats = _lib.Stats()
        sched = sched_rows(sched)
        self._chk(self._lib.nk2d_comp_fcn_frozen(self._ctx, x.ptr, out.ptr, ctypes.byref(stats), _dp(sched),
                                                 sched.shape[0]))
        return out, stats.as_dict()

    def last_schedule(self):
        n = ctypes.c_int64(0)
        self._chk(self._lib.nk2d_last_schedule(self._ctx, None, 0, ctypes.byref(n)))
# ... 329 lines not shown
```

Measured before the change: 8.458.

## Exchange precomputed stage values y+z between neighbour columns in frozen persistent kernel

Adds a stage-value exchange mode for the persistent frozen-year kernel. Each column now publishes u = y + z for its three stages into a double-buffered area appended to the sync buffer. Neighbours then read the one pre-added value per stage instead of loading y and z separately and adding them. This is meant to cut the global loads on the critical path after each neighbour-flag poll. In exchange it writes an extra 6*nv doubles per step, and z itself is stored only when the error estimate or the last row needs it. It is enabled by default for E 5..7 own-state configurations, and also adds optional clock instrumentation.

Result: faster. 8.790, median of 6 (+3.9%).

```diff
diff --git a/newton-krylov_ooc_amd/csrc/nk2d_api.hip b/newton-krylov_ooc_amd/csrc/nk2d_api.hip
--- a/newton-krylov_ooc_amd/csrc/nk2d_api.hip
+++ b/newton-krylov_ooc_amd/csrc/nk2d_api.hip
@@ -174,6 +174,7 @@
     if (key == "frozen_coef_lds") { c->frozen_coef_lds = (int)value & 63; return 0; }
     if (key == "frozen_sums_poison") { c->frozen_sums_poison = (int)value != 0 ? 1 : 0; return 0; }
     if (key == "frozen_early") { c->frozen_early = (int)value != 0 ? 1 : 0; return 0; }
+    if (key == "frozen_stage_exchange") { c->frozen_stage_exchange = (int)value != 0 ? 1 : 0; return 0; }
     if (key == "frozen_by_column") { c->frozen_by_column = (int)value; return 0; }
     if (key == "frozen_cache_after") { c->frozen_cache_after = (int)value; return 0; }
     if (key == "spec_bias") { c->spec_bias = value > 0.0 ? value : 1.0; return 0; }
@@ -601,6 +602,8 @@
     c->frozen_lds_bits = 0;
     c->frozen_early = NK2D_FROZEN_EARLY_DEFAULT;
     c->frozen_early_bits = 0;
+    c->frozen_stage_exchange = NK2D_FROZEN_STAGE_EXCHANGE_DEFAULT;
+    c->frozen_stage_exchange_bits = 0;
     c->frozen_by_column = 1;
     c->strm = nullptr;
     c->spec_bias = 1.0;
@@ -1113,6 +1116,7 @@
     else if (key == "frozen_cache_lean") v = nk2d_frozen_cache_is_lean(c);
     else if (key == "frozen_lds_bits") v = c->frozen_lds_bits;
     else if (key == "frozen_early_bits") v = c->frozen_early_bits;
+    else if (key == "frozen_stage_exchange_bits") v = c->frozen_stage_exchange_bits;
     else if (key == "frozen_step_sums_hash") v = c->frozen_step_sums_hash;
     else if (key == "frozen_lean_years") v = c->frozen_lean_years;
     else if (key == "frozen_forced_years") v = c->frozen_forced_years;
diff --git a/newton-krylov_ooc_amd/csrc/nk2d_bodies.h b/newton-krylov_ooc_amd/csrc/nk2d_bodies.h
--- a/newton-krylov_ooc_amd/csrc/nk2d_bodies.h
+++ b/newton-krylov_ooc_amd/csrc/nk2d_bodies.h
@@ -785,6 +785,14 @@
     double acc;
     double* part;
     int defer, pending;
+#ifdef NK2D_FROZEN_CLOCKS
+    long long ck_match = 0, ck_fetch = 0;
+#endif
+};
+struct StageXchg {
+    const double* u;
+    double* uout;
+    int keep_z;
 };
 template <int E>
 __device__ __forceinline__ double norm_partial_sum(const DevP& P, const double (&yy)[E], const double (&d0v)[E],
@@ -802,7 +810,9 @@
 template <int E, int KIND, int FACTOR, int STAGE, int MP = 0, int FINAL = 0, int CL = 0>
 __device__ __forceinline__ void newton_fused_body(const DevP& P, const FusedArgs& A, int task, int lane,
                                                   const FinalArgs* fin = nullptr, const LdsSrc* lds = nullptr,
-                                                  OwnState<E>* own = nullptr, LateNorm* late = nullptr) {
+                                                  OwnState<E>* own = nullptr, LateNorm* late = nullptr,
+                                                  const StageXchg* xc = nullptr) {
+    static_assert(!(CL & 256) || (CL & 48) == 48, "the stage-value exchange needs the column's whole own state");
     const double* coef_lds = (CL & 1) ? lds->coef : nullptr;
     double* w_lds = (CL & 2) ? lds->w : nullptr;
     (void)coef_lds; (void)w_lds;
@@ -814,6 +824,12 @@
         if constexpr (CL & 1) load_coef_lds<E>(coef_lds, lane, cf);
         else load_coef<E>(P, j, lane, cf);
         double y0[E], ys[E], yn[E];
+        if constexpr (CL & 256) {
+            if (!own->valid) {
+                load_col<E, MP>(A.st.y, task, lane, y0);
+                w_lds_put<E>(lds->y, 0, lane, y0);
+            }
+        } else {
         if constexpr (CL & 16) {
             if (!own->valid) {
                 load_col<E, MP>(A.st.y, task, lane, y0);
@@ -826,11 +842,26 @@
         }
         load_col<E, MP>(A.st.y, cs_col, lane, ys);
         load_col<E, MP>(A.st.y, cn_col, lane, yn);
+        }
 #pragma unroll
         for (int e = 0; e < E; ++e) { fr[e] = 0.0; fcr[e] = 0.0; fci[e] = 0.0; }
 #pragma unroll
         for (int i = 0; i < 3; ++i) {
             double c[E], cs[E], cn[E], kv[E], f[E];
+#ifdef NK2D_FROZEN_CLOCKS
+            long long ck_t0 = 0;
+            if constexpr (CL & 128) ck_t0 = (i == 0) ? late->ck_match : (long long)__builtin_amdgcn_s_memrealtime();
+#endif
+            if constexpr (CL & 256) {
+                if (own->valid) {
+#pragma unroll
+                    for (int e = 0; e < E; ++e) c[e] = own->z[i][e];
+                } else {
+                    load_col<E, 1>(xc->u + i * A.st.nv, task, lane, c);
+                }
+                load_col<E, 1>(xc->u + i * A.st.nv, cs_col, lane, cs);
+                load_col<E, 1>(xc->u + i * A.st.nv, cn_col, lane, cn);
+            } else {
             if constexpr (CL & 32) {
                 if (own->valid) {
 #pragma unroll
@@ -843,10 +874,19 @@
             }
             load_col<E, MP>(A.st.z + i * A.st.nv, cs_col, lane, cs);
             load_col<E, MP>(A.st.z + i * A.st.nv, cn_col, lane, cn);
+            }
+#ifdef NK2D_FROZEN_CLOCKS
+            if constexpr (CL & 128) {
+                asm volatile("s_waitcnt vmcnt(0)" ::: "memory");
+                late->ck_fetch += (long long)__builtin_amdgcn_s_memrealtime() - ck_t0;
+            }
+#endif
             if constexpr (CL & 4) col_lds_get<E>(lds->step, i, lane, kv);
             else load_col<E, MP>(A.st.kv[i], j, lane, kv);
+            if constexpr (!(CL & 256)) {
 #pragma unroll
             for (int e = 0; e < E; ++e) { c[e] = y0[e] + c[e]; cs[e] = ys[e] + cs[e]; cn[e] = yn[e] + cn[e]; }
+            }
             tend_col<E, KIND>(P, cf, c, cs, cn, kv, tr, lane, f);
             if constexpr (KIND == 2) forced_sources<E>(P, A.st.kv[i], j, lane, c, f);
             if constexpr (KIND == 1) {
@@ -1032,7 +1072,7 @@
     }
     const bool norm = A.part != nullptr;
     double yy[E], w0[E], w1[E], w2[E];
-    if (FINAL || norm) {
+    if (FINAL || norm || (CL & 256) != 0) {
         if constexpr (CL & 16) col_lds_get<E>(lds->y, 0, lane, yy);
         else load_col<E, MP>(A.st.y, task, lane, yy);
     }
@@ -1089,8 +1129,20 @@
                 o[i][e] = v - yn[e];
             }
         }
+        if constexpr (CL & 256) {
+#pragma unroll
+            for (int i = 0; i < 3; ++i) {
+                double uu[E];
+#pragma unroll
+                for (int e = 0; e < E; ++e) uu[e] = yn[e] + o[i][e];
+                store_col<E, 1>(xc->uout + i * A.st.nv, task, lane, uu);
+#pragma unroll
+                for (int e = 0; e < E; ++e) own->z[i][e] = uu[e];
+            }
+        } else {
 #pragma unroll
         for (int i = 0; i < 3; ++i) store_col<E, MP>(fin->znext + i * A.st.nv, task, lane, o[i]);
+        }
         double wv[E];
 #pragma unroll
         for (int r = 0; r < 3; ++r) {
@@ -1099,7 +1151,7 @@
             if constexpr (CL & 2) w_lds_put<E>(w_lds, r, lane, wv);
             else store_col<E>(wout + r * A.st.nv, task, lane, wv);
         }
-        if constexpr (CL & 32) {
+        if constexpr ((CL & 32) != 0 && (CL & 256) == 0) {
 #pragma unroll
             for (int i = 0; i < 3; ++i) {
 #pragma unroll
@@ -1125,8 +1177,18 @@
     for (int r = 0; r < 3; ++r) {
 #pragma unroll
         for (int e = 0; e < E; ++e) zz[e] = (cT[r][0] * w0[e] + cT[r][1] * w1[e]) + cT[r][2] * w2[e];
+        if constexpr (CL & 256) {
+            double uu[E];
+#pragma unroll
+            for (int e = 0; e < E; ++e) uu[e] = yy[e] + zz[e];
+            store_col<E, 1>(xc->uout + r * A.st.nv, task, lane, uu);
+            if (xc->keep_z) store_col<E, MP>(zout + r * A.st.nv, task, lane, zz);
+#pragma unroll
+            for (int e = 0; e < E; ++e) own->z[r][e] = uu[e];
+        } else {
         store_col<E, MP>(zout + r * A.st.nv, task, lane, zz);
-        if constexpr (CL & 32) {
+        }
+        if constexpr ((CL & 32) != 0 && (CL & 256) == 0) {
 #pragma unroll
             for (int e = 0; e < E; ++e) own->z[r][e] = zz[e];
         }
@@ -1815,6 +1877,8 @@
 #define NK2D_SPIN_LIMIT 4000000
 
 static inline size_t yr_sync_bytes(const nk2d_ctx* c) { return 8192 + (size_t)c->ncol * 128; }
+__host__ __device__ static inline size_t yr_xchg_offset(int ncol) { return 8192 + (size_t)ncol * 128; }
+static inline size_t yr_xchg_bytes(const nk2d_ctx* c) { return sizeof(double) * 6 * c->nv; }
 
 struct NeighbourSync {
     unsigned* flags;
@@ -1826,6 +1890,7 @@
     int fences;
 #ifdef NK2D_FROZEN_CLOCKS
     long long ck_drain = 0, ck_wait = 0, ck_flag = 0;
+    long long ck_match = 0;
 #endif
     __device__ __forceinline__ void publish() {
 #ifdef NK2D_FROZEN_CLOCKS
@@ -1871,6 +1936,9 @@
 #endif
         }
         __syncthreads();
+#ifdef NK2D_FROZEN_CLOCKS
+        ck_match = (long long)__builtin_amdgcn_s_memrealtime();
+#endif
         if (fences) __builtin_amdgcn_fence(__ATOMIC_ACQUIRE, "agent");
         return *lds_ok != 0;
     }
@@ -1904,6 +1972,9 @@
             if (lane == 0) *lds_ok = good;
         }
         __syncthreads();
+#ifdef NK2D_FROZEN_CLOCKS
+        ck_match = (long long)__builtin_amdgcn_s_memrealtime();
+#endif
         if (fences) __builtin_amdgcn_fence(__ATOMIC_ACQUIRE, "agent");
         return *lds_ok != 0;
     }
@@ -2128,6 +2199,7 @@
     int fences;
     int coef_lds;
 #define NK2D_FROZEN_EARLY_OF(coef_lds) (((coef_lds) >> 8) & 1)
+#define NK2D_FROZEN_XCHG_OF(coef_lds) (((coef_lds) >> 9) & 1)
     int by_column;
     const double* SRC;
     int upr_on;
@@ -2161,9 +2233,10 @@
     store_col<E, MP>(f, task, lane, ff);
 }
 
-template <int E, int MP>
+template <int E, int MP, int XU = 0>
 __device__ __forceinline__ void step_tail_body(const double* __restrict__ y, const double* __restrict__ z, size_t nv,
-                                               const FinalArgs& fin, double* __restrict__ wout, int task, int lane) {
+                                               const FinalArgs& fin, double* __restrict__ wout, int task, int lane,
+                                               double* __restrict__ unext = nullptr) {
     double yy[E], z0[E], z1[E], z2[E], yn[E];
     load_col<E, MP>(y, task, lane, yy);
     load_col<E, MP>(z, task, lane, z0);
@@ -2189,6 +2262,15 @@
     }
 #pragma unroll
     for (int i = 0; i < 3; ++i) store_col<E, MP>(fin.znext + i * nv, task, lane, o[i]);
+    if constexpr (XU) {
+#pragma unroll
+        for (int i = 0; i < 3; ++i) {
+            double uu[E];
+#pragma unroll
+            for (int e = 0; e < E; ++e) uu[e] = yn[e] + o[i][e];
+            store_col<E, 1>(unext + i * nv, task, lane, uu);
+        }
+    }
     double wv[E];
 #pragma unroll
     for (int r = 0; r < 3; ++r) {
diff --git a/newton-krylov_ooc_amd/csrc/nk2d_common.h b/newton-krylov_ooc_amd/csrc/nk2d_common.h
--- a/newton-krylov_ooc_amd/csrc/nk2d_common.h
+++ b/newton-krylov_ooc_amd/csrc/nk2d_common.h
@@ -17,6 +17,7 @@
 
 
 #define NK2D_FROZEN_EARLY_DEFAULT 1
+#define NK2D_FROZEN_STAGE_EXCHANGE_DEFAULT 1
 struct nk2d_ctx {
     nk2d_desc d;
     int nz, ny, tc, E, nzp, ncol, nreg;
@@ -99,6 +100,8 @@
     int frozen_lds_bits;
     int frozen_early;
     int frozen_early_bits;
+    int frozen_stage_exchange;
+    int frozen_stage_exchange_bits;
     int frozen_by_column;
     int frozen_alloc_async;
     int frozen_cache_after;
diff --git a/newton-krylov_ooc_amd/csrc/nk2d_frozen.hip b/newton-krylov_ooc_amd/csrc/nk2d_frozen.hip
--- a/newton-krylov_ooc_amd/csrc/nk2d_frozen.hip
+++ b/newton-krylov_ooc_amd/csrc/nk2d_frozen.hip
@@ -581,7 +581,7 @@
     if (c->YR_OUT) return 0;
     NK2D_CHECK(c, hipMalloc((void**)&c->YR_PART, sizeof(double) * 2 * c->ncol));
     NK2D_CHECK(c, hipMalloc((void**)&c->YR_OUT, sizeof(double) * 32));
-    NK2D_CHECK(c, hipMalloc((void**)&c->YR_SYNC, yr_sync_bytes(c)));
+    NK2D_CHECK(c, hipMalloc((void**)&c->YR_SYNC, yr_sync_bytes(c) + yr_xchg_bytes(c)));
     NK2D_CHECK(c, hipMalloc((void**)&c->YR_MTAB, sizeof(int) * std::max<size_t>(c->rho_tab.size(), 1)));
     NK2D_CHECK(c, hipHostMalloc((void**)&c->hYR_OUT, sizeof(double) * 32));
     NK2D_CHECK(c, hipEventCreate(&c->yr_ev[0]));
@@ -617,6 +617,10 @@
     c->frozen_lds_bits = A.coef_lds;
     c->frozen_early_bits = (A.coef_lds & 48) == 48 ? c->frozen_early : 0;
     A.coef_lds |= c->frozen_early_bits << 8;
+    const bool team_year = c->frozen_team && c->E <= 2 && !pl.phos;
+    c->frozen_stage_exchange_bits =
+        ((A.coef_lds & 48) == 48 && NK2D_FROZEN_XCHG(c->E, c->kind, team_year, pl.pieces, pl.lean)) ? c->frozen_stage_exchange : 0;
+    A.coef_lds |= c->frozen_stage_exchange_bits << 9;
     return 0;
 }
 
@@ -647,8 +651,10 @@
     const double* o = c->hYR_OUT;
     if ((int)o[0] != 0 || (int64_t)o[1] != n) return 2;
 #ifdef NK2D_FROZEN_CLOCKS
-    std::fprintf(stderr, "frozen clocks (early %d): %.0f phases, per phase drain %.3f us, flag store to poll match %.3f us, rest %.3f us; kernel %.3f ms\n",
-                 c->frozen_early_bits, o[11], 0.01 * o[8] / o[11], 0.01 * o[9] / o[11], 0.01 * (o[10] - o[8] - o[9]) / o[11], 1.0e-5 * o[10]);
+    std::fprintf(stderr, "frozen clocks (early %d, stage exchange %d): %.0f phases, per phase drain %.3f us, flag store to poll match %.3f us, "
+                 "poll match to neighbours loaded %.3f us, rest %.3f us; kernel %.3f ms\n",
+                 c->frozen_early_bits, c->frozen_stage_exchange_bits, o[11], 0.01 * o[8] / o[11], 0.01 * o[9] / o[11], 0.01 * o[12] / o[11],
+                 0.01 * (o[10] - o[8] - o[9] - o[12]) / o[11], 1.0e-5 * o[10]);
 #endif
     if (team) c->frozen_team_years++;
     float ms = 0.f;
diff --git a/newton-krylov_ooc_amd/csrc/nk2d_frozen_body.inc b/newton-krylov_ooc_amd/csrc/nk2d_frozen_body.inc
--- a/newton-krylov_ooc_amd/csrc/nk2d_frozen_body.inc
+++ b/newton-krylov_ooc_amd/csrc/nk2d_frozen_body.inc
@@ -90,10 +90,26 @@
     (void)lds_step;
     LateNorm late = {0.0, nullptr, (OWN && by_col && own_bits == 48) ? uni_i(NK2D_FROZEN_EARLY_OF(A.coef_lds)) : 0, 0};
     (void)late;
+    constexpr bool XCHG = OWN && NK2D_FROZEN_XCHG(E, KIND, TEAM, PIECES, LEAN);
+    const int xchg = (XCHG && by_col && own_bits == 48) ? uni_i(NK2D_FROZEN_XCHG_OF(A.coef_lds)) : 0;
+    double* const xu0 = XCHG ? (double*)((char*)A.arrive + yr_xchg_offset(P.ncol)) : nullptr;
+    (void)xchg; (void)xu0;
+#define FZ_U (swapZ ? xu0 + 3 * nv : xu0)
+#define FZ_UN (swapZ ? xu0 : xu0 + 3 * nv)
     if (col_wave && (!TEAM || tw == 0)) {
         double zero[E];
 #pragma unroll
         for (int e = 0; e < E; ++e) zero[e] = 0.0;
+        if constexpr (XCHG) {
+            if (xchg) {
+                double y0[E];
+                load_col<E, MPX>(FZ_Y, wave, lane, y0);
+#pragma unroll
+                for (int e = 0; e < E; ++e) y0[e] = y0[e] + zero[e];
+#pragma unroll
+                for (int i = 0; i < 3; ++i) store_col<E, 1>(FZ_U + i * nv, wave, lane, y0);
+            }
+        }
 #pragma unroll
         for (int i = 0; i < 3; ++i) {
             store_col<E, MPX>(FZ_Z + i * nv, wave, lane, zero);
@@ -201,6 +217,9 @@
                         __syncthreads();
                     }
                 }
+#ifdef NK2D_FROZEN_CLOCKS
+                late.ck_match = nbs.ck_match;
+#endif
                 if (is_final) {
                     FinalArgs Fin;
                     Fin.ynew = FZ_YOLD;
@@ -223,7 +242,14 @@
                             if (m == 1) { newton_single_body<E, MPX, 1>(P, FA, wave, lane, &Fin); taken = true; }
                         }
                         if constexpr (OWN) {
-                            if (own_bits == 48) { newton_fused_body<E, KIND, 0, 1, MPX, 1, 191>(P, FA, wave, lane, &Fin, &L, &own, &late); taken = true; }
+                            if constexpr (XCHG) {
+                            if (own_bits == 48 && xchg) {
+                                const StageXchg XC = {FZ_U, do_stage ? FZ_UN : FZ_U, 0};
+                                newton_fused_body<E, KIND, 0, 1, MPX, 1, 447>(P, FA, wave, lane, &Fin, &L, &own, &late, &XC); taken = true;
+                            }
+                            }
+                            if (taken) {}
+                            else if (own_bits == 48) { newton_fused_body<E, KIND, 0, 1, MPX, 1, 191>(P, FA, wave, lane, &Fin, &L, &own, &late); taken = true; }
                             else if (!PIECES && own_bits == 32) { newton_fused_body<E, KIND, 0, 1, MPX, 1, 47>(P, FA, wave, lane, &Fin, &L, &own); taken = true; }
                             else if (own_bits == 16) { newton_fused_body<E, KIND, 0, 1, MPX, 1, 31>(P, FA, wave, lane, &Fin, &L, &own); FZ_OWN_DEAD() taken = true; }
                         }
@@ -255,7 +281,14 @@
                             if (m == 1) { newton_single_body<E, MPX, 0>(P, FA, wave, lane); taken = true; }
                         }
                         if constexpr (OWN) {
-                            if (own_bits == 48) { newton_fused_body<E, KIND, 0, 1, MPX, 0, 191>(P, FA, wave, lane, nullptr, &L, &own, &late); taken = true; }
+                            if constexpr (XCHG) {
+                            if (own_bits == 48 && xchg) {
+                                const StageXchg XC = {FZ_U, (do_stage && do_update) ? FZ_UN : FZ_U, (with_err || last_row) ? 1 : 0};
+                                newton_fused_body<E, KIND, 0, 1, MPX, 0, 447>(P, FA, wave, lane, nullptr, &L, &own, &late, &XC); taken = true;
+                            }
+                            }
+                            if (taken) {}
+                            else if (own_bits == 48) { newton_fused_body<E, KIND, 0, 1, MPX, 0, 191>(P, FA, wave, lane, nullptr, &L, &own, &late); taken = true; }
                             else if (!PIECES && own_bits == 32) { newton_fused_body<E, KIND, 0, 1, MPX, 0, 47>(P, FA, wave, lane, nullptr, &L, &own); taken = true; }
                             else if (own_bits == 16) { newton_fused_body<E, KIND, 0, 1, MPX, 0, 31>(P, FA, wave, lane, nullptr, &L, &own); FZ_OWN_DEAD() taken = true; }
                         }
@@ -302,7 +335,11 @@
                 Fin.znext = FZ_ZN;
                 Fin.x0 = R.x0; Fin.x1 = R.x1; Fin.x2 = R.x2;
                 Fin.nblk_cols = 0;
-                step_tail_body<E, MPX>(FZ_Y, FZ_Z, nv, Fin, A.W, wave, lane);
+                bool tail_done = false;
+                if constexpr (XCHG) {
+                    if (xchg) { step_tail_body<E, MPX, 1>(FZ_Y, FZ_Z, nv, Fin, A.W, wave, lane, FZ_UN); tail_done = true; }
+                }
+                if (!tail_done) step_tail_body<E, MPX>(FZ_Y, FZ_Z, nv, Fin, A.W, wave, lane);
                 own.valid = 0;
                 if constexpr (COEF_LDS) {
                     if (w_in_lds) {
@@ -338,6 +375,7 @@
     if (wg == (int)(gridDim.x / 2) && threadIdx.x == 0) {
         A.out[8] = (double)nbs.ck_drain; A.out[9] = (double)nbs.ck_wait;
         A.out[10] = (double)((long long)__builtin_amdgcn_s_memrealtime() - ck_begin); A.out[11] = (double)nbs.phase;
+        A.out[12] = (double)late.ck_fetch;
     }
 #endif
     if (wg == 0 && threadIdx.x == 0) {
@@ -349,3 +387,5 @@
 #undef FZ_YOLD
 #undef FZ_Z
 #undef FZ_ZN
+#undef FZ_U
+#undef FZ_UN
diff --git a/newton-krylov_ooc_amd/csrc/nk2d_frozen_plan.h b/newton-krylov_ooc_amd/csrc/nk2d_frozen_plan.h
--- a/newton-krylov_ooc_amd/csrc/nk2d_frozen_plan.h
+++ b/newton-krylov_ooc_amd/csrc/nk2d_frozen_plan.h
@@ -12,6 +12,7 @@
 #define NK2D_COEF_LDS_DOUBLES(E) ((7 * (E) + 1) * 64)
 
 #define NK2D_FROZEN_OWN(E, KIND, TEAM, LEAN) ((E) >= 5 && (E) <= 7 && ((KIND) == 0 || (KIND) == 2) && !(TEAM) && !(LEAN))
+#define NK2D_FROZEN_XCHG(E, KIND, TEAM, PIECES, LEAN) (NK2D_FROZEN_OWN(E, KIND, TEAM, LEAN) && !((E) == 7 && (KIND) == 0 && (PIECES)))
 
 struct FrozenPlanIn {
     int E, kind, tc, ny, ncol;
diff --git a/newton-krylov_ooc_amd/engine.py b/newton-krylov_ooc_amd/engine.py
--- a/newton-krylov_ooc_amd/engine.py
+++ b/newton-krylov_ooc_amd/engine.py
@@ -191,6 +191,8 @@
             self.set_option("frozen_phosphorus_shallow", float(os.environ["NK2D_FROZEN_PHOSPHORUS_SHALLOW"]))
         if "NK2D_FROZEN_EARLY" in os.environ:
             self.set_option("frozen_early", float(os.environ["NK2D_FROZEN_EARLY"]))
+        if "NK2D_FROZEN_STAGE_EXCHANGE" in os.environ:
+            self.set_option("frozen_stage_exchange", float(os.environ["NK2D_FROZEN_STAGE_EXCHANGE"]))
         if "NK2D_PC_TWO_ENDED" in os.environ:
             self.set_option("pc_two_ended", float(os.environ["NK2D_PC_TWO_ENDED"]))
         if "NK2D_PC_PIVOT_WAVE" in os.environ:
```
